# rodrigo-paganini/kalman-vae

Measured on AMD Instinct MI355X. Metric: sequences/sec (ELBO training step, 32x32xT bouncing-ball), higher is better.
Workload: dtype f32; 1 GPU; BASELINE configs[1] (configs[2] per-GPU shard): bouncing-ball 32x32, T=50, batch=256/GPU, dynamics=lstm K=3, z=4, u=4, a=2, full train step (fwd incl. sigmoid(x_logits) + loss incl. active-unit stats + bwd + clip + Adam); both the GPU leg and the cpu_baseline leg do this work; preset=c2, global_batch=256, seq_len=50, parallelism=dp1, capture=hipgraph, loss_finite=True, dist_backend=none

## Files before the change

### include/kvae_lgssm.h

```cpp
#ifndef KVAE_LGSSM_H
#define KVAE_LGSSM_H

#include <stdint.h>

#ifdef __cplusplus
extern "C" {
#endif

#define KVAE_MAX_DIM 16
#define KVAE_ABI_VERSION 12

typedef enum {
  KVAE_OK = 0,
  KVAE_ERR_DIMS = 1,
  KVAE_ERR_NULL = 2,
  KVAE_ERR_LAUNCH = 3,
  KVAE_ERR_ARG = 4
} kvae_status;

typedef struct {
  const float *ptr;
  int64_t sb, st;
} kvae_stack;

typedef struct {
  int32_t B, T, n, m, p;
  kvae_stack A;
  kvae_stack Bm;
  kvae_stack C;
  kvae_stack Q;
  const float *R;
  const float *mu0;
  int64_t mu0_sb;
  const float *Sigma0;
  int64_t Sigma0_sb;
  const float *Y;
  const float *U;
  const float *mask;
} kvae_lgssm_problem;

typedef struct {
  float *mus_filt;
  float *Sigmas_filt;
  float *mus_pred;
  float *Sigmas_pred;
  float *mus_smooth;
  float *Sigmas_smooth;
  float *aux;
} kvae_lgssm_states;
#define KVAE_AUX(n, p) ((n) * (p) + (p) * (p) + (n) * (n))

typedef struct {
  float *ptr;
  int64_t sb, st;
} kvae_gstack;

typedef struct {
  kvae_gstack gA, gB, gC, gQ;
  float *gY, *gU;
  float *g_mu0, *g_Sigma0;
} kvae_lgssm_input_grads;


int kvae_lgssm_filter_fwd(const kvae_lgssm_problem *prob, const kvae_lgssm_states *out, void *stream);

int kvae_lgssm_rts_fwd(const kvae_lgssm_problem *prob, const kvae_lgssm_states *io, void *stream);

int kvae_lgssm_smooth_fwd(const kvae_lgssm_problem *prob, const kvae_lgssm_states *out, void *stream);

int kvae_lgssm_filter_alpha_lstm(const kvae_lgssm_problem *prob, const kvae_lgssm_states *out, const float *w_ih,
                                 const float *w_hh, const float *b_ih, const float *b_hh, const float *head_w,
                                 const float *head_b, const float *A, const float *Bm, const float *C, int32_t K, int32_t H,
                                 float *record, float *alpha, float *gates, float *c_seq, float *h_seq, float *x_seq,
                                 void *stream);


int kvae_lgssm_smooth_bwd(const kvae_lgssm_problem *prob, const kvae_lgssm_states *saved,
                          const kvae_lgssm_states *up, const kvae_lgssm_input_grads *out,
                          float *ws, int with_rts, void *stream);

int kvae_lgssm_alpha_lstm_bwd(const kvae_lgssm_problem *prob, const kvae_lgssm_states *saved, const kvae_lgssm_states *up,
                              const kvae_lgssm_input_grads *out, float *ws, int with_rts, const float *w_ih,
                              const float *w_hh, const float *head_w, const float *A, const float *Bm, const float *C,
                              int32_t K, int32_t H, const float *alpha, const float *gates, const float *c_seq,
                              const float *g_record_up, const float *g_alpha_up, float *g_record, float *d_pre,
                              float *g_logit, void *stream);


int kvae_lgssm_elbo(const kvae_lgssm_problem *prob, const float *mus_smooth, const float *Sigmas_smooth,
                    const float *eps, float *terms, int32_t *chol_levels, float *ws_lz, float *g_mus,
                    float *g_Sigmas, const kvae_lgssm_input_grads *g, void *stream);


int kvae_mix_fwd(const float *alpha, const float *base, float *out, int64_t rows, int32_t K, int32_t E,
                 void *stream);

int kvae_mix_bwd(const float *alpha, const float *base, const float *g_out, float *g_alpha, float *g_base,
                 float *partials, int64_t rows, int32_t K, int32_t E, int32_t accumulate_alpha, void *stream);
int64_t kvae_mix_bwd_partials(int64_t rows);


int kvae_lstm_fwd(const float *x, const float *w_ih, const float *w_hh, const float *b_ih, const float *b_hh,
                  float *h_seq, float *gates, float *c_seq, int32_t B, int32_t T, int32_t I, int32_t H, void *stream);

int kvae_lstm_bwd(const float *g_h, const float *gates, const float *c_seq, const float *w_ih, const float *w_hh,
                  float *d_pre, float *dx, int32_t B, int32_t T, int32_t I, int32_t H, void *stream);


int kvae_regime_fwd(const float *logits, const float *init_logits, const float *gumbel, const float *P, float *y_seq,
                    float *log_q, float *log_p, int32_t B, int32_t T, int32_t K, float tau, const float *tau_dev,
                    int32_t hard, void *stream);
int kvae_regime_bwd(const float *logits, const float *init_logits, const float *gumbel, const float *P,
                    const float *y_seq, const float *g_y, const float *g_log_q, const float *g_log_p, float *g_logits,
                    float *g_init, int32_t B, int32_t T, int32_t K, float tau, const float *tau_dev, void *stream);


int kvae_bigru_fwd(const float *x, const float *const w_ih[2], const float *const w_hh[2], const float *const b_ih[2],
                   const float *const b_hh[2], float *h_seq, float *gates, int32_t B, int32_t T, int32_t I, int32_t H,
                   void *stream);
int kvae_bigru_bwd(const float *g_h, const float *gates, const float *h_seq, const float *const w_ih[2],
                   const float *const w_hh[2], float *d_pre_i, float *d_pre_h, float *dx, int32_t B, int32_t T,
                   int32_t I, int32_t H, void *stream);


int kvae_bias_shuffle_act_fwd(const float *in, const float *bias, float *out, int64_t N, int32_t C, int32_t H,
                              int32_t W, int32_t r, int32_t relu, void *stream);
int kvae_bias_shuffle_act_bwd(const float *g_out, const float *out, float *g_in, float *bias_partials, int64_t N,
                              int32_t C, int32_t H, int32_t W, int32_t r, int32_t relu, void *stream);
int64_t kvae_bias_partial_rows(int64_t N);
int kvae_colsum(const float *partials, float *out, int64_t rows, int64_t cols, void *stream);
int kvae_colsum2(const float *partials_a, float *out_a, int64_t rows_a, int64_t cols_a, const float *partials_b, float *out_b,
                 int64_t rows_b, int64_t cols_b, void *stream);


int kvae_clip_adam(float *params, const float *grads, float *exp_avg, float *exp_avg_sq, int64_t n, const int32_t *seg_of,
                   int32_t n_seg, const float *seg_active, float *seg_steps, const float *lr_dev, float lr, float beta1, float beta2,
                   float eps, float weight_decay, float clip, const float *div_dev, float *norm_out, float *ws, void *stream);


int kvae_lgssm_emission_means(const kvae_lgssm_problem *prob, const float *mus_smooth, const float *mus_filt, float *a_imputed,
                              float *a_filtered, void *stream);


typedef struct kvae_wgrad_problem {
  const float *d;
  const float *h;
  const float *x;
  float *g_wh, *g_wx, *g_b;
  int64_t d_stride, h_stride, x_stride, N;
  int32_t R, H, I, bias, T, shift;
} kvae_wgrad_problem;
int64_t kvae_rnn_wgrad_ws_floats(const kvae_wgrad_problem *probs, int32_t n);
int kvae_rnn_wgrad(const kvae_wgrad_problem *probs, int32_t n, float *ws, void *stream);

int kvae_linear_fwd(const float *x, int64_t x_stride, int64_t N, int32_t F, const float *W, const float *b, int32_t O,
                    int32_t softmax, float *y, void *stream);
int kvae_linear_bwd_input(const float *g, const float *y, int64_t N, int32_t F, const float *W, int32_t O, float *g_logit,
                          float *dx, int64_t dx_stride, void *stream);


int kvae_bce_frames_fwd(const float *logits, const float *x, float *frame_ll, int64_t frames, int32_t pixels, void *stream);
int kvae_bce_frames_bwd(const float *logits, const float *x, const float *g_frame, float *g_logits, int64_t frames,
                        int32_t pixels, void *stream);


#define KVAE_DEC_HEAD_SCRATCH_FLOATS 2304
int kvae_dec_head_fwd(const float *in, const float *W, const float *bias, float *logits, float *w_scratch, int64_t N,
                      int32_t Cin, int32_t side, void *stream);
int kvae_dec_head_bwd(const float *in, const float *W, const float *g_logits, float *g_in, float *w_partials,
                      float *b_partials, float *w_scratch, int64_t N, int32_t Cin, int32_t side, void *stream);
int kvae_enc_stem_fwd(const float *x, const float *W, const float *bias, float *out, uint32_t *relu_bits, int64_t N, int32_t Cout,
                      int32_t side, void *stream);
int kvae_enc_stem_bwd(const float *x, const float *out, const uint32_t *relu_bits, const float *g_out, float *w_partials,
                      float *b_partials, int64_t N, int32_t Cout, int32_t side, void *stream);
int64_t kvae_conv_edge_partial_rows(int64_t N);

int kvae_enc_mid_fwd(const float *in, const float *W, const float *bias, float *out, int64_t N, int32_t C, int32_t side,
                     void *stream);
int kvae_enc_mid_bwd(const float *in, const float *W, const float *out, const float *g_out, float *g_in,
                     float *w_partials, float *b_partials, int64_t N, int32_t C, int32_t side, void *stream);
int64_t kvae_enc_mid_partial_rows(int64_t N, int32_t side);

int kvae_dec_up_fwd(const float *x, const float *W, const float *bias, float *out, int64_t N, int32_t Cin, int32_t side,
                    void *stream);
int kvae_dec_up_bwd(const float *x, const float *W, const float *out, const float *g_out, float *g_x, float *w_partials,
                    float *b_partials, int64_t N, int32_t Cin, int32_t side, void *stream);
int64_t kvae_dec_up_partial_rows(int64_t N, int32_t side);
int32_t kvae_dec_up_set_workgroups(int32_t n);


int kvae_enc_head_fwd(const float *feat, const float *Wmu, const float *bmu, const float *Wvar, const float *bvar,
                      const float *eps, float *mu, float *var, float *a, int64_t N, int32_t F, int32_t A,
                      float noise_emission, void *stream);
int kvae_enc_head_bwd(const float *feat, const float *Wmu, const float *Wvar, const float *var, const float *eps,
                      const float *g_a, const float *g_mu, const float *g_var, float *g_feat, float *w_partials,
                      float *b_partials, int64_t N, int32_t F, int32_t A, float noise_emission, void *stream);
int kvae_dec_fc_fwd(const float *a, const float *W, const float *b, float *h, int64_t N, int32_t F, int32_t A, void *stream);
int kvae_dec_fc_bwd(const float *g_h, const float *a, const float *W, float *g_a, float *w_partials, float *b_partials,
                    int64_t N, int32_t F, int32_t A, void *stream);
int64_t kvae_head_partial_rows(void);
int kvae_latent_reg_fwd(const float *a, const float *mu, const float *var, float *reg, int64_t N, int32_t A, void *stream);
int kvae_latent_reg_bwd(const float *a, const float *mu, const float *var, const float *g, float *g_a, float *g_mu,
                        float *g_var, int64_t N, int32_t A, void *stream);

int kvae_loss_head_fwd(const float *lpx, const float *regf, const float *mask, const float *elbo_kf, const float *beta,
                       float scale_reconstruction, float vae_weight, float kf_weight, const float *weights_dev, float *out6,
                       float *coef3, int64_t n, void *stream);
int kvae_loss_head_bwd(const float *g_loss, const float *coef3, const float *mask, float *g_lpx, float *g_regf,
                       float *g_elbo_kf, int64_t n, void *stream);

typedef struct {
  int32_t B, S, H;
  int32_t n, m, p, K;
  int32_t kind;
  int32_t hidden;
  const float *A;
  const float *Bm;
  const float *C;
  const float *LQ;
  const float *LR;
  const float *mu;
  const float *L0;
  const float *U;
  const float *w_ih;
  const float *w_hh;
  const float *b_ih;
  const float *b_hh;
  const float *head_w;
  const float *head_b;
  const float *h0;
  const float *c0;
  const float *y0;
  const float *P;
  const float *s0;
  const float *eps0;
  const float *eps_z;
  const float *eps_a;
  const float *gumbel;
  float *a_out;
  float *z_out;
  float *w_out;
} kvae_gen_problem;
int kvae_lgssm_generate(const kvae_gen_problem *prob, void *stream);

#define KVAE_PSAMPLE_GAINS 1
#define KVAE_PSAMPLE_PATHS 2
typedef struct {
  int32_t B, S, T;
  int32_t n, p;
  int32_t stages;
  const float *mus_filt;
  const float *Sigmas_filt;
  const float *mus_pred;
  const float *Sigmas_pred;
  kvae_stack A;
  kvae_stack C;
  kvae_stack Q;
  const float *LR;
  const float *eps;
  const float *eta;
  float *z_out;
  float *a_out;
  int32_t *levels_out;
  float *ws;
} kvae_psample_problem;
int kvae_lgssm_posterior_sample(const kvae_psample_problem *prob, void *stream);
int64_t kvae_lgssm_posterior_sample_ws_floats(const kvae_psample_problem *prob);

int kvae_abi_version(void);
const char *kvae_last_error(void);
const char *kvae_build_info(void);

#ifdef __cplusplus
}
#endif
#endif
```

### kalman-vae_amd/csrc/kvae_vae.hip

```cpp
#include <hip/hip_runtime.h>

#include <stdint.h>
#include <stdio.h>
#include <stdlib.h>
#include <string.h>

#include "../../include/kvae_lgssm.h"

namespace kvae {}
using namespace kvae;

extern "C" int kvae_launch_status(const char *what);
static int launch_status(const char *what) { return kvae_launch_status(what); }

#include "vae_epilogue.h"

__device__ __forceinline__ void colsum_v4_body(const float *__restrict__ partials, float *__restrict__ out, int64_t rows, int64_t cols,
                                               unsigned block) {
  __shared__ float4 red[8][64];
  const int lane = threadIdx.x & 63, wv = threadIdx.x >> 6;
  const int64_t c = ((int64_t)block * 64 + lane) * 4;
  float4 s0 = make_float4(0.f, 0.f, 0.f, 0.f), s1 = s0, s2 = s0, s3 = s0;
  if (c < cols) {
    const float *p = partials + c;
    int64_t r = wv;
    for (; r + 24 < rows; r += 32) {
      const float4 a = *reinterpret_cast<const float4 *>(p + r * cols), b = *reinterpret_cast<const float4 *>(p + (r + 8) * cols),
                   d = *reinterpret_cast<const float4 *>(p + (r + 16) * cols), e = *reinterpret_cast<const float4 *>(p + (r + 24) * cols);
      s0.x += a.x; s0.y += a.y; s0.z += a.z; s0.w += a.w;
      s1.x += b.x; s1.y += b.y; s1.z += b.z; s1.w += b.w;
      s2.x += d.x; s2.y += d.y; s2.z += d.z; s2.w += d.w;
      s3.x += e.x; s3.y += e.y; s3.z += e.z; s3.w += e.w;
    }
    for (; r < rows; r += 8) {
      const float4 a = *reinterpret_cast<const float4 *>(p + r * cols);
      s0.x += a.x; s0.y += a.y; s0.z += a.z; s0.w += a.w;
    }
  }
  red[wv][lane] = make_float4((s0.x + s1.x) + (s2.x + s3.x), (s0.y + s1.y) + (s2.y + s3.y), (s0.z + s1.z) + (s2.z + s3.z),
                              (s0.w + s1.w) + (s2.w + s3.w));
  __syncthreads();
  if (wv == 0 && c < cols) {
    float4 t = red[0][lane];
#pragma unroll
    for (int w = 1; w < 8; ++w) { const float4 u = red[w][lane]; t.x += u.x; t.y += u.y; t.z += u.z; t.w += u.w; }
    *reinterpret_cast<float4 *>(out + c) = t;
  }
}
__global__ __launch_bounds__(512) void k_colsum_v4(const float *__restrict__ partials, float *__restrict__ out, int64_t rows,
                                                   int64_t cols) {
  colsum_v4_body(partials, out, rows, cols, blockIdx.x);
}
__global__ __launch_bounds__(512) void k_colsum_v4_pair(const float *__restrict__ pa, float *__restrict__ oa, int64_t rows_a, int64_t cols_a,
                                                        unsigned nb_a, const float *__restrict__ pb, float *__restrict__ ob,
                                                        int64_t rows_b, int64_t cols_b) {
  if (blockIdx.x < nb_a) colsum_v4_body(pa, oa, rows_a, cols_a, blockIdx.x);
  else colsum_v4_body(pb, ob, rows_b, cols_b, blockIdx.x - nb_a);
}
__global__ __launch_bounds__(256) void k_colsum(const float *__restrict__ partials, float *__restrict__ out, int64_t rows,
                                                int64_t cols) {
  __shared__ float red[256];
  const int cx = threadIdx.x & 63, ry = threadIdx.x >> 6;
  const int64_t c = (int64_t)blockIdx.x * 64 + cx;
  float s0 = 0.f, s1 = 0.f;
  if (c < cols) {
    int64_t r = ry;
    for (; r + 4 < rows; r += 8) {
      s0 += partials[r * cols + c];
      s1 += partials[(r + 4) * cols + c];
    }
    if (r < rows) s0 += partials[r * cols + c];
  }
  red[threadIdx.x] = s0 + s1;
  __syncthreads();
  if (ry == 0 && c < cols) out[c] = (red[cx] + red[64 + cx]) + (red[128 + cx] + red[192 + cx]);
}

template <int R>
__global__ __launch_bounds__(256) void k_vae_epilogue_fwd_v4(const float *__restrict__ in, const float *__restrict__ bias,
                                                             float *__restrict__ out, int C, int H, int W, int64_t quads,
                                                             int relu) {
  const int OW = W * R, OH = H * R, QW = OW / 4;
  for (int64_t qd = (int64_t)blockIdx.x * 256 + threadIdx.x; qd < quads; qd += (int64_t)gridDim.x * 256) {
    const int qw = (int)(qd % QW);
    const int64_t t1 = qd / QW;
    const int oh = (int)(t1 % OH);
    const int64_t t2 = t1 / OH;
    const int c = (int)(t2 % C);
    const int64_t n = t2 / C;
    float4 v;
    if (R == 1) {
      const float b = bias[c];
      const float4 x = *reinterpret_cast<const float4 *>(in + ((n * C + c) * H + oh) * W + 4 * qw);
      v = make_float4(x.x + b, x.y + b, x.z + b, x.w + b);
    } else {
      const int ch0 = c * 4 + (oh & 1) * 2;
      const int64_t base = ((n * (C * 4) + ch0) * H + (oh >> 1)) * W + 2 * qw;
      const float2 a = *reinterpret_cast<const float2 *>(in + base);
      const float2 d = *reinterpret_cast<const float2 *>(in + base + (int64_t)H * W);
      const float b0 = bias[ch0], b1 = bias[ch0 + 1];
      v = make_float4(a.x + b0, d.x + b1, a.y + b0, d.y + b1);
    }
    if (relu) v = make_float4(fmaxf(v.x, 0.f), fmaxf(v.y, 0.f), fmaxf(v.z, 0.f), fmaxf(v.w, 0.f));
    *reinterpret_cast<float4 *>(out + qd * 4) = v;
  }
}

__global__ __launch_bounds__(256) void k_vae_epilogue_fwd(const float *in, const float *bias, float *out, EpiShape s,
                                                          int64_t total, int relu) {
  for (int64_t o = (int64_t)blockIdx.x * 256 + threadIdx.x; o < total; o += (int64_t)gridDim.x * 256)
    epi_fwd_elem(s, in, bias, out, o, relu);
}

__global__ __launch_bounds__(256) void k_vae_epilogue_bwd_bias(const float *__restrict__ g_out, const float *__restrict__ out,
                                                               float *__restrict__ g_in, float *__restrict__ bias_partials,
                                                               EpiShape s, int n_per_chunk, int relu) {
  extern __shared__ float bins[];
  const int Cin = s.C * s.r * s.r;
  const int OW = s.W * s.r, OH = s.H * s.r;
  const int64_t vol = (int64_t)s.C * OH * OW;
  for (int i = threadIdx.x; i < Cin; i += 256) bins[i] = 0.f;
  __syncthreads();
  const int64_t pos = (int64_t)blockIdx.x * 256 + threadIdx.x;
  if (pos < vol) {
    const int ow = (int)(pos % OW);
    const int oh = (int)((pos / OW) % OH);
    const int c = (int)(pos / ((int64_t)OW * OH));
    const int ch = c * s.r * s.r + (oh % s.r) * s.r + (ow % s.r);
    const int64_t in_off = ((int64_t)ch * s.H + oh / s.r) * s.W + ow / s.r;
    const int64_t in_vol = (int64_t)Cin * s.H * s.W;
    const int64_t n0 = (int64_t)blockIdx.y * n_per_chunk;
    const int64_t n1 = n0 + n_per_chunk < s.N ? n0 + n_per_chunk : s.N;
    float acc = 0.f;
    for (int64_t n = n0; n < n1; ++n) {
      float g = g_out[n * vol + pos];
      if (relu && !(out[n * vol + pos] > 0.f)) g = 0.f;
      g_in[n * in_vol + in_off] = g;
      acc += g;
    }
    atomicAdd(&bins[ch], acc);
  }
  __syncthreads();
  for (int i = threadIdx.x; i < Cin; i += 256) {
    if (bins[i] != 0.f) atomicAdd(&bias_partials[(int64_t)blockIdx.y * Cin + i], bins[i]);
  }
}

__global__ __launch_bounds__(256) void k_vae_epilogue_bwd(const float *g_out, const float *out, float *g_in, EpiShape s,
                                                          int64_t total, int relu) {
  for (int64_t o = (int64_t)blockIdx.x * 256 + threadIdx.x; o < total; o += (int64_t)gridDim.x * 256)
    epi_bwd_elem(s, g_out, out, g_in, o, relu);
}

#define KVAE_EPI_SAMPLES_PER_CHUNK 32
extern "C" int64_t kvae_bias_partial_rows(int64_t N);
static unsigned epi_grid(int64_t total) {
  const int64_t blocks = (total + 255) / 256;
  return (unsigned)(blocks < 256 * 32 ? blocks : 256 * 32);
}

extern "C" {
int kvae_bias_shuffle_act_fwd(const float *in, const float *bias, float *out, int64_t N, int32_t C, int32_t H, int32_t W,
                              int32_t r, int32_t relu, void *stream) {
  if (!in || !bias || !out) return KVAE_ERR_NULL;
  if (N < 1 || C < 1 || H < 1 || W < 1 || r < 1) return KVAE_ERR_ARG;
  const EpiShape s{N, C, H, W, r};
  const int64_t total = N * C * H * W * r * r;
  const bool aligned = ((uintptr_t)in % 16 == 0) && ((uintptr_t)out % 16 == 0);
  if (aligned && r == 1 && W % 4 == 0)
    k_vae_epilogue_fwd_v4<1><<<dim3(epi_grid(total / 4)), dim3(256), 0, (hipStream_t)stream>>>(in, bias, out, C, H, W, total / 4, relu);
  else if (aligned && r == 2 && W % 2 == 0)
    k_vae_epilogue_fwd_v4<2><<<dim3(epi_grid(total / 4)), dim3(256), 0, (hipStream_t)stream>>>(in, bias, out, C, H, W, total / 4, relu);
  else
    k_vae_epilogue_fwd<<<dim3(epi_grid(total)), dim3(256), 0, (hipStream_t)stream>>>(in, bias, out, s, total, relu);
  return launch_status("k_vae_epilogue_fwd");
}
int kvae_bias_shuffle_act_bwd(const float *g_out, const float *out, float *g_in, float *bias_partials, int64_t N, int32_t C,
                              int32_t H, int32_t W, int32_t r, int32_t relu, void *stream) {
  if (!g_out || !g_in || (relu && !out)) return KVAE_ERR_NULL;
  if (N < 1 || C < 1 || H < 1 || W < 1 || r < 1) return KVAE_ERR_ARG;
  const EpiShape s{N, C, H, W, r};
  const int64_t total = N * C * H * W * r * r;
  hipStream_t st = (hipStream_t)stream;
  if (bias_partials) {
    const int Cin = C * r * r;
    const int64_t chunks = kvae_bias_partial_rows(N);
    if (hipMemsetAsync(bias_partials, 0, sizeof(float) * chunks * Cin, st) != hipSuccess) return launch_status("memset bias_partials");
    const int64_t vol = (int64_t)C * H * W * r * r;
    k_vae_epilogue_bwd_bias<<<dim3((unsigned)((vol + 255) / 256), (unsigned)chunks), dim3(256), sizeof(float) * Cin, st>>>(
        g_out, out, g_in, bias_partials, s, KVAE_EPI_SAMPLES_PER_CHUNK, relu);
    return launch_status("k_vae_epilogue_bwd_bias");
  }
  k_vae_epilogue_bwd<<<dim3(epi_grid(total)), dim3(256), 0, st>>>(g_out, out, g_in, s, total, relu);
  return launch_status("k_vae_epilogue_bwd");
}
int kvae_colsum(const float *partials, float *out, int64_t rows, int64_t cols, void *stream) {
  if (!partials || !out) return KVAE_ERR_NULL;
  if (rows < 1 || cols < 1) return KVAE_ERR_ARG;
  if ((cols & 3) == 0 && ((((uintptr_t)partials | (uintptr_t)out) & 15) == 0))
    k_colsum_v4<<<dim3((unsigned)((cols + 255) / 256)), dim3(512), 0, (hipStream_t)stream>>>(partials, out, rows, cols);
  else
    k_colsum<<<dim3((unsigned)((cols + 63) / 64)), dim3(256), 0, (hipStream_t)stream>>>(partials, out, rows, cols);
  return launch_status("k_colsum");
}
int kvae_colsum2(const float *pa, float *oa, int64_t rows_a, int64_t cols_a, const float *pb, float *ob, int64_t rows_b,
                 int64_t cols_b, void *stream) {
  if (!pa || !oa || !pb || !ob) return KVAE_ERR_NULL;
  if (rows_a < 1 || cols_a < 1 || rows_b < 1 || cols_b < 1) return KVAE_ERR_ARG;
  if (((cols_a | cols_b) & 3) == 0 && ((((uintptr_t)pa | (uintptr_t)oa | (uintptr_t)pb | (uintptr_t)ob) & 15) == 0)) {
    const unsigned nb_a = (unsigned)((cols_a + 255) / 256), nb_b = (unsigned)((cols_b + 255) / 256);
    k_colsum_v4_pair<<<dim3(nb_a + nb_b), dim3(512), 0, (hipStream_t)stream>>>(pa, oa, rows_a, cols_a, nb_a, pb, ob, rows_b, cols_b);
    return launch_status("k_colsum_v4_pair");
  }
  const int rc = kvae_colsum(pa, oa, rows_a, cols_a, stream);
  return rc ? rc : kvae_colsum(pb, ob, rows_b, cols_b, stream);
}
int64_t kvae_bias_partial_rows(int64_t N) { return (N + KVAE_EPI_SAMPLES_PER_CHUNK - 1) / KVAE_EPI_SAMPLES_PER_CHUNK; }
}

constexpr int CA_BLOCKS = 512;
constexpr int CA_MAX_SEG = 1024;
__global__ __launch_bounds__(256) void k_grad_sumsq(const float *__restrict__ g, int64_t n, const int32_t *__restrict__ seg_of,
                                                    int n_seg, const float *__restrict__ seg_active,
                                                    const float *__restrict__ div_dev, float *__restrict__ seg_steps,
                                                    float *__restrict__ ws) {
  __shared__ float red[256];
  const float inv = div_dev ? 1.0f / fmaxf(*div_dev, 1.0f) : 1.0f;
  const bool gated = seg_of && seg_active;
  float s = 0.f;
  for (int64_t i = (int64_t)blockIdx.x * 256 + threadIdx.x; i < n; i += (int64_t)gridDim.x * 256) {
    float v = g[i] * inv;
    if (gated && seg_active[seg_of[i]] == 0.f) v = 0.f;
    s = fmaf(v, v, s);
  }
  red[threadIdx.x] = s;
  __syncthreads();
  for (int o = 128; o > 0; o >>= 1) {
    if ((int)threadIdx.x < o) red[threadIdx.x] += red[threadIdx.x + o];
    __syncthreads();
  }
  if (threadIdx.x == 0) ws[blockIdx.x] = red[0];
  if (blockIdx.x == 0)
    for (int sg = threadIdx.x; sg < n_seg; sg += 256)
      if (!seg_active || seg_active[sg] != 0.f) seg_steps[sg] += 1.0f;
}
__global__ __launch_bounds__(256) void k_clip_adam(float *__restrict__ p, const float *__restrict__ g, float *__restrict__ m,
                                                   float *__restrict__ v, int64_t n, const int32_t *__restrict__ seg_of, int n_seg,
                                                   const float *__restrict__ seg_active, const float *__restrict__ seg_steps,
                                                   const float *__restrict__ lr_dev, float lr, float beta1, float beta2, float eps,
                                                   float wd, float clip, const float *__restrict__ div_dev,
                                                   float *__restrict__ norm_out, const float *__restrict__ ws, int nparts) {
  __shared__ float red[256];
  __shared__ float s_step_size[CA_MAX_SEG], s_bc2s[CA_MAX_SEG];
  float s = 0.f;
  for (int i = threadIdx.x; i < nparts; i += 256) s += ws[i];
  red[threadIdx.x] = s;
  const float lrv = lr_dev ? *lr_dev : lr;
  for (int sg = threadIdx.x; sg < n_seg; sg += 256) {
    const float step = seg_steps[sg];
    const bool on = !seg_active || seg_active[sg] != 0.f;
    s_step_size[sg] = on ? lrv / (1.0f - powf(beta1, step)) : -1.0f;
    s_bc2s[sg] = on ? sqrtf(1.0f - powf(beta2, step)) : 1.0f;
  }
  __syncthreads();
  for (int o = 128; o > 0; o >>= 1) {
    if ((int)threadIdx.x < o) red[threadIdx.x] += red[threadIdx.x + o];
    __syncthreads();
  }
  const float total = sqrtf(red[0]);
  if (norm_out && blockIdx.x == 0 && threadIdx.x == 0) *norm_out = total;
  const float inv = div_dev ? 1.0f / fmaxf(*div_dev, 1.0f) : 1.0f;
  const float scale = inv * (clip > 0.f ? fminf(clip / (total + 1e-6f), 1.0f) : 1.0f);
  for (int64_t i = (int64_t)blockIdx.x * 256 + threadIdx.x; i < n; i += (int64_t)gridDim.x * 256) {
    const int sg = seg_of ? seg_of[i] : 0;
    const float step_size = s_step_size[sg], bc2s = s_bc2s[sg];
    if (step_size < 0.f) continue;
    float gi = g[i] * scale;
    const float pi = p[i];
    if (wd != 0.f) gi = fmaf(wd, pi, gi);
    const float mi = m[i] + (gi - m[i]) * (1.0f - beta1);
    const float vi = beta2 * v[i] + (1.0f - beta2) * gi * gi;
    m[i] = mi, v[i] = vi;
    p[i] = pi - step_size * mi / (sqrtf(vi) / bc2s + eps);
  }
}
extern "C" int kvae_clip_adam(float *params, const float *grads, float *exp_avg, float *exp_avg_sq, int64_t n,
                              const int32_t *seg_of, int32_t n_seg, const float *seg_active, float *seg_steps, const float *lr_dev,
                              float lr, float beta1, float beta2, float eps, float weight_decay, float clip, const float *div_dev,
                              float *norm_out, float *ws, void *stream) {
  if (!params || !grads || !exp_avg || !exp_avg_sq || !seg_steps || !ws) return KVAE_ERR_NULL;
  if (n < 1 || n_seg < 1 || n_seg > CA_MAX_SEG || (!seg_of && n_seg != 1)) return KVAE_ERR_ARG;
  const int64_t want = (n + 1023) / 1024;
  const unsigned parts = (unsigned)(want < CA_BLOCKS ? want : CA_BLOCKS);
  k_grad_sumsq<<<dim3(parts), dim3(256), 0, (hipStream_t)stream>>>(grads, n, seg_of, n_seg, seg_active, div_dev, seg_steps, ws);
  int rc = launch_status("k_grad_sumsq");
  if (rc) return rc;
  const unsigned blocks = (unsigned)((n + 255) / 256 < 2048 ? (n + 255) / 256 : 2048);
  k_clip_adam<<<dim3(blocks), dim3(256), 0, (hipStream_t)stream>>>(params, grads, exp_avg, exp_avg_sq, n, seg_of, n_seg, seg_active,
                                                                   seg_steps, lr_dev, lr, beta1, beta2, eps, weight_decay, clip,
                                                                   div_dev, norm_out, ws, (int)parts);
  return launch_status("k_clip_adam");
}

#include "vae_loss.h"

__global__ __launch_bounds__(256) void k_vae_bce_fwd(const float *__restrict__ logits, const float *__restrict__ x,
                                                     float *__restrict__ frame_ll, int64_t frames, int pixels) {
  const int64_t f = (int64_t)blockIdx.x * 4 + (threadIdx.x >> 6);
  const int lane = threadIdx.x & 63;
  if (f >= frames) return;
  const float *l = logits + f * pixels, *t = x + f * pixels;
  float acc = 0.f;
  if ((pixels & 3) == 0 && (((uintptr_t)l | (uintptr_t)t) & 15) == 0) {
    for (int i = lane * 4; i < pixels; i += 256) {
      const float4 a = *reinterpret_cast<const float4 *>(l + i), b = *reinterpret_cast<const float4 *>(t + i);
      acc += bce_logit(a.x, b.x) + bce_logit(a.y, b.y) + bce_logit(a.z, b.z) + bce_logit(a.w, b.w);
    }
  } else {
    for (int i = lane; i < pixels; i += 64) acc += bce_logit(l[i], t[i]);
  }
  for (int off = 32; off > 0; off >>= 1) acc += __shfl_down(acc, off, 64);
  if (lane == 0) frame_ll[f] = -acc;
}

__global__ __launch_bounds__(256) void k_vae_bce_bwd(const float *__restrict__ logits, const float *__restrict__ x,
                                                     const float *__restrict__ g_frame, float *__restrict__ g_logits,
                                                     int64_t total, int pixels) {
  for (int64_t i = ((int64_t)blockIdx.x * 256 + threadIdx.x) * 4; i < total; i += (int64_t)gridDim.x * 1024) {
    const float g = -g_frame[i / pixels];
    const float4 a = *reinterpret_cast<const float4 *>(logits + i), b = *reinterpret_cast<const float4 *>(x + i);
    *reinterpret_cast<float4 *>(g_logits + i) = make_float4(g * (sigmoid_stable(a.x) - b.x), g * (sigmoid_stable(a.y) - b.y),
                                                            g * (sigmoid_stable(a.z) - b.z), g * (sigmoid_stable(a.w) - b.w));
  }
}
__global__ __launch_bounds__(256) void k_vae_bce_bwd_scalar(const float *logits, const float *x, const float *g_frame,
                                                            float *g_logits, int64_t total, int pixels) {
  for (int64_t i = (int64_t)blockIdx.x * 256 + threadIdx.x; i < total; i += (int64_t)gridDim.x * 256)
    g_logits[i] = -g_frame[i / pixels] * (sigmoid_stable(logits[i]) - x[i]);
}

extern "C" {
int kvae_bce_frames_fwd(const float *logits, const float *x, float *frame_ll, int64_t frames, int32_t pixels, void *stream) {
  if (!logits || !x || !frame_ll) return KVAE_ERR_NULL;
  if (frames < 1 || pixels < 1) return KVAE_ERR_ARG;
  k_vae_bce_fwd<<<dim3((unsigned)((frames + 3) / 4)), dim3(256), 0, (hipStream_t)stream>>>(logits, x, frame_ll, frames, pixels);
  return launch_status("k_vae_bce_fwd");
}
int kvae_bce_frames_bwd(const float *logits, const float *x, const float *g_frame, float *g_logits, int64_t frames,
                        int32_t pixels, void *stream) {
  if (!logits || !x || !g_frame || !g_logits) return KVAE_ERR_NULL;
  if (frames < 1 || pixels < 1) return KVAE_ERR_ARG;
  const int64_t total = frames * pixels;
  const bool v4 = (pixels & 3) == 0 && ((((uintptr_t)logits | (uintptr_t)x | (uintptr_t)g_logits) & 15) == 0);
  if (v4)
    k_vae_bce_bwd<<<dim3(epi_grid(total / 4)), dim3(256), 0, (hipStream_t)stream>>>(logits, x, g_frame, g_logits, total, pixels);
  else
    k_vae_bce_bwd_scalar<<<dim3(epi_grid(total)), dim3(256), 0, (hipStream_t)stream>>>(logits, x, g_frame, g_logits, total, pixels);
  return launch_status("k_vae_bce_bwd");
}
}

#include "vae_conv_edge.h"
extern "C" {
int64_t kvae_conv_edge_partial_rows(int64_t N) { return N < 1024 ? (N < 1 ? 1 : N) : 1024; }

int kvae_dec_head_fwd(const float *in, const float *W, const float *bias, float *logits, float *w_scratch, int64_t N,
                      int32_t Cin, int32_t side, void *stream) {
  if (!in || !W || !bias || !logits || !w_scratch) return KVAE_ERR_NULL;
  if (N < 1) return KVAE_ERR_ARG;
  if (Cin != DH_CI || side != DH_S) return KVAE_ERR_DIMS;
  k_dec_head_prep<<<dim3(1), dim3(256), 0, (hipStream_t)stream>>>(W, w_scratch);
  k_dec_head_fwd<<<dim3((unsigned)N), dim3(256), 0, (hipStream_t)stream>>>(in, w_scratch, bias, logits);
  return launch_status("k_dec_head_fwd");
}
int kvae_dec_head_bwd(const float *in, const float *W, const float *g_logits, float *g_in, float *w_partials,
                      float *b_partials, float *w_scratch, int64_t N, int32_t Cin, int32_t side, void *stream) {
  if (!in || !W || !g_logits || !w_partials || !b_partials || !w_scratch) return KVAE_ERR_NULL;
  if (N < 1) return KVAE_ERR_ARG;
  if (Cin != DH_CI || side != DH_S) return KVAE_ERR_DIMS;
  if (g_in) {
    k_dec_head_prep<<<dim3(1), dim3(256), 0, (hipStream_t)stream>>>(W, w_scratch);
    k_dec_head_bwd_data<<<dim3((unsigned)N), dim3(256), 0, (hipStream_t)stream>>>(g_logits, w_scratch, g_in);
    const int rc = launch_status("k_dec_head_bwd_data");
    if (rc) return rc;
  }
  k_dec_head_wrw<<<dim3((unsigned)kvae_conv_edge_partial_rows(N)), dim3(256), 0, (hipStream_t)stream>>>(in, g_logits, w_partials,
                                                                                                     b_partials, N);
  return launch_status("k_dec_head_wrw");
}
int kvae_enc_stem_fwd(const float *x, const float *W, const float *bias, float *out, uint32_t *relu_bits, int64_t N, int32_t Cout,
                      int32_t side, void *stream) {
  if (!x || !W || !bias || !out) return KVAE_ERR_NULL;
  if (N < 1) return KVAE_ERR_ARG;
  if (Cout != ES_CO || side != ES_IN) return KVAE_ERR_DIMS;
  k_enc_stem_fwd<<<dim3((unsigned)N), dim3(256), 0, (hipStream_t)stream>>>(x, W, bias, out, relu_bits);
  return launch_status("k_enc_stem_fwd");
}
int kvae_enc_stem_bwd(const float *x, const float *out, const uint32_t *relu_bits, const float *g_out, float *w_partials,
                      float *b_partials, int64_t N, int32_t Cout, int32_t side, void *stream) {
  if (!x || (!out && !relu_bits) || !g_out || !w_partials || !b_partials) return KVAE_ERR_NULL;
  if (N < 1) return KVAE_ERR_ARG;
  if (Cout != ES_CO || side != ES_IN) return KVAE_ERR_DIMS;
  static const int mfma = getenv("KVAE_STEM_MFMA") ? atoi(getenv("KVAE_STEM_MFMA")) : 1;
  const dim3 grid((unsigned)kvae_conv_edge_partial_rows(N));
  if (mfma == 1 && relu_bits) k_enc_stem_wrw_mfma<true><<<grid, dim3(256), 0, (hipStream_t)stream>>>(x, out, relu_bits, g_out, w_partials, b_partials, N);
  else if (!out) return KVAE_ERR_NULL;
  else if (mfma) k_enc_stem_wrw_mfma<false><<<grid, dim3(256), 0, (hipStream_t)stream>>>(x, out, relu_bits, g_out, w_partials, b_partials, N);
  else k_enc_stem_wrw<<<grid, dim3(256), 0, (hipStream_t)stream>>>(x, out, g_out, w_partials, b_partials, N);
  return launch_status("k_enc_stem_wrw");
}
}

#include "vae_conv_mid.h"
static inline int64_t enc_mid_grid(int64_t N, int32_t side) {
  const int64_t fpi = side == 16 ? 2 : 8, iters = (N + fpi - 1) / fpi;
  return iters < 256 ? (iters < 1 ? 1 : iters) : 256;
}
extern "C" {
int64_t kvae_enc_mid_partial_rows(int64_t N, int32_t side) { return enc_mid_grid(N, side); }

int kvae_enc_mid_fwd(const float *in, const float *W, const float *bias, float *out, int64_t N, int32_t C, int32_t side,
                     void *stream) {
  if (!in || !W || !bias || !out) return KVAE_ERR_NULL;
  if (N < 1 || (N + 256 * 8) * EM_C * side * side * 4 >= EM_MAX_BYTES) return KVAE_ERR_ARG;
  if (C != EM_C || (side != 16 && side != 8)) return KVAE_ERR_DIMS;
  const dim3 grid((unsigned)enc_mid_grid(N, side));
  if (side == 16) k_enc_mid_fwd<16><<<grid, dim3(256), 0, (hipStream_t)stream>>>(in, W, bias, out, N);
  else k_enc_mid_fwd<8><<<grid, dim3(256), 0, (hipStream_t)stream>>>(in, W, bias, out, N);
  return launch_status("k_enc_mid_fwd");
}
int kvae_enc_mid_bwd(const float *in, const float *W, const float *out, const float *g_out, float *g_in,
                     float *w_partials, float *b_partials, int64_t N, int32_t C, int32_t side, void *stream) {
  if (!in || !W || !out || !g_out || !w_partials || !b_partials) return KVAE_ERR_NULL;
  if (N < 1 || (N + 256 * 8) * EM_C * side * side * 4 >= EM_MAX_BYTES) return KVAE_ERR_ARG;
  if (C != EM_C || (side != 16 && side != 8)) return KVAE_ERR_DIMS;
  const dim3 grid((unsigned)enc_mid_grid(N, side));
  if (g_in) {
    if (side == 16) k_enc_mid_bwd_data<16><<<grid, dim3(256), 0, (hipStream_t)stream>>>(W, out, g_out, g_in, N);
    else k_enc_mid_bwd_data<8><<<grid, dim3(256), 0, (hipStream_t)stream>>>(W, out, g_out, g_in, N);
    const int rc = launch_status("k_enc_mid_bwd_data");
    if (rc) return rc;
  }
  if (side == 16) k_enc_mid_wrw<16><<<grid, dim3(256), 0, (hipStream_t)stream>>>(in, out, g_out, w_partials, b_partials, N);
  else k_enc_mid_wrw<8><<<grid, dim3(256), 0, (hipStream_t)stream>>>(in, out, g_out, w_partials, b_partials, N);
  return launch_status("k_enc_mid_wrw");
}
}

#include "vae_conv_up_wino.h"
static bool dec_up_wino() {
  static const int env = getenv("KVAE_WINO") ? atoi(getenv("KVAE_WINO")) : 1;
  return env != 0;
}
static int g_dec_up_wgs = 0;
static inline int64_t dec_up_cap() {
  static const int env = getenv("KVAE_UP_WGS") ? atoi(getenv("KVAE_UP_WGS")) : 0;
  const int v = env >= 1 && env <= 256 ? env : __atomic_load_n(&g_dec_up_wgs, __ATOMIC_RELAXED);
  return v >= 1 && v <= 256 ? v : 256;
}
static inline int64_t dec_up_grid(int64_t N, int32_t side) {
  const int64_t fpi = side == 8 ? 2 : 8, iters = (N + fpi - 1) / fpi, cap = dec_up_cap();
  return iters < cap ? (iters < 1 ? 1 : iters) : cap;
}
extern "C" {
int64_t kvae_dec_up_partial_rows(int64_t N, int32_t side) { return dec_up_grid(N, side); }
int32_t kvae_dec_up_set_workgroups(int32_t n) {
  const int32_t prev = (int32_t)dec_up_cap();
  __atomic_store_n(&g_dec_up_wgs, n >= 1 && n <= 256 ? n : 0, __ATOMIC_RELAXED);
  return prev;
}

int kvae_dec_up_fwd(const float *x, const float *W, const float *bias, float *out, int64_t N, int32_t Cin, int32_t side,
                    void *stream) {
  if (!x || !W || !bias || !out) return KVAE_ERR_NULL;
  if (N < 1 || (N + 256 * 8) * UP_CO * side * side * 4 >= EM_MAX_BYTES) return KVAE_ERR_ARG;
  if (Cin != UP_CI || (side != 8 && side != 4)) return KVAE_ERR_DIMS;
  const dim3 grid((unsigned)dec_up_grid(N, side));
  if (dec_up_wino()) {
    const int64_t sets = side == 8 ? N : (N + 3) / 4;
    const dim3 wgrid((unsigned)(sets < dec_up_cap() ? sets : dec_up_cap()));
    if (side == 8) k_dec_up_fwd_wino<8><<<wgrid, dim3(512), 0, (hipStream_t)stream>>>(x, W, bias, out, N);
    else k_dec_up_fwd_wino<4><<<wgrid, dim3(512), 0, (hipStream_t)stream>>>(x, W, bias, out, N);
    return launch_status("k_dec_up_fwd_wino");
  }
  if (side == 8) k_dec_up_fwd<8><<<grid, dim3(256), 0, (hipStream_t)stream>>>(x, W, bias, out, N);
  else k_dec_up_fwd<4><<<grid, dim3(256), 0, (hipStream_t)stream>>>(x, W, bias, out, N);
  return launch_status("k_dec_up_fwd");
}
int kvae_dec_up_bwd(const float *x, const float *W, const float *out, const float *g_out, float *g_x, float *w_partials,
                    float *b_partials, int64_t N, int32_t Cin, int32_t side, void *stream) {
  if (!x || !W || !out || !g_out || !w_partials || !b_partials) return KVAE_ERR_NULL;
  if (N < 1 || (N + 256 * 8) * UP_CO * side * side * 4 >= EM_MAX_BYTES) return KVAE_ERR_ARG;
  if (Cin != UP_CI || (side != 8 && side != 4)) return KVAE_ERR_DIMS;
  const dim3 grid((unsigned)dec_up_grid(N, side));
  if (g_x) {
    const int64_t sets = side == 8 ? N : (N + 3) / 4;
    const dim3 wgrid((unsigned)(sets < dec_up_cap() ? sets : dec_up_cap()));
    if (dec_up_wino() && side == 8) k_dec_up_bwd_data_wino<8><<<wgrid, dim3(512), 0, (hipStream_t)stream>>>(W, out, g_out, g_x, N);
    else if (dec_up_wino()) k_dec_up_bwd_data_wino<4><<<wgrid, dim3(512), 0, (hipStream_t)stream>>>(W, out, g_out, g_x, N);
    else if (side == 8) k_dec_up_bwd_data<8><<<grid, dim3(256), 0, (hipStream_t)stream>>>(W, out, g_out, g_x, N);
    else k_dec_up_bwd_data<4><<<grid, dim3(256), 0, (hipStream_t)stream>>>(W, out, g_out, g_x, N);
    const int rc = launch_status("k_dec_up_bwd_data");
    if (rc) return rc;
  }
  if (dec_up_wino()) {
    if (side == 8) k_dec_up_wrw_wino<8><<<grid, dim3(512), 0, (hipStream_t)stream>>>(x, out, g_out, w_partials, b_partials, N);
    else k_dec_up_wrw_wino<4><<<grid, dim3(512), 0, (hipStream_t)stream>>>(x, out, g_out, w_partials, b_partials, N);
    return launch_status("k_dec_up_wrw_wino");
  }
  if (side == 8) k_dec_up_wrw<8><<<grid, dim3(256), 0, (hipStream_t)stream>>>(x, out, g_out, w_partials, b_partials, N);
  else k_dec_up_wrw<4><<<grid, dim3(256), 0, (hipStream_t)stream>>>(x, out, g_out, w_partials, b_partials, N);
  return launch_status("k_dec_up_wrw");
}
}

#include "vae_heads.h"
extern "C" {
int64_t kvae_head_partial_rows(void) { return HD_WAVES; }

int kvae_enc_head_fwd(const float *feat, const float *Wmu, const float *bmu, const float *Wvar, const float *bvar,
                      const float *eps, float *mu, float *var, float *a, int64_t N, int32_t F, int32_t A,
                      float noise_emission, void *stream) {
  if (!feat || !Wmu || !bmu || !Wvar || !bvar || !mu || !var || !a) return KVAE_ERR_NULL;
  if (N < 1) return KVAE_ERR_ARG;
  if (F != HD_F || A != HD_A) return KVAE_ERR_DIMS;
  const unsigned grid = (unsigned)(N < 4 * 512 ? (N + 3) / 4 : 512);
  k_enc_head_fwd<<<dim3(grid), dim3(256), 0, (hipStream_t)stream>>>(feat, Wmu, bmu, Wvar, bvar, eps, noise_emission, mu, var, a, N);
  return launch_status("k_enc_head_fwd");
}
int kvae_enc_head_bwd(const float *feat, const float *Wmu, const float *Wvar, const float *var, const float *eps,
                      const float *g_a, const float *g_mu, const float *g_var, float *g_feat, float *w_partials,
                      float *b_partials, int64_t N, int32_t F, int32_t A, float noise_emission, void *stream) {
  if (!feat || !Wmu || !Wvar || !var || !g_feat || !w_partials || !b_partials) return KVAE_ERR_NULL;
  if (N < 1) return KVAE_ERR_ARG;
  if (F != HD_F || A != HD_A) return KVAE_ERR_DIMS;
  k_enc_head_bwd<<<dim3(HD_WAVES / 4), dim3(256), 0, (hipStream_t)stream>>>(feat, Wmu, Wvar, var, eps, g_a, g_mu, g_var,
                                                                             noise_emission, g_feat, w_partials, b_partials, N);
  return launch_status("k_enc_head_bwd");
}
int kvae_dec_fc_fwd(const float *a, const float *W, const float *b, float *h, int64_t N, int32_t F, int32_t A, void *stream) {
  if (!a || !W || !b || !h) return KVAE_ERR_NULL;
  if (N < 1) return KVAE_ERR_ARG;
  if (F != HD_F || A != HD_A) return KVAE_ERR_DIMS;
  k_dec_fc_fwd<<<dim3(epi_grid(N * (HD_F / 4))), dim3(256), 0, (hipStream_t)stream>>>(a, W, b, h, N * (HD_F / 4));
  return launch_status("k_dec_fc_fwd");
}
int kvae_dec_fc_bwd(const float *g_h, const float *a, const float *W, float *g_a, float *w_partials, float *b_partials,
                    int64_t N, int32_t F, int32_t A, void *stream) {
  if (!g_h || !a || !W || !g_a || !w_partials || !b_partials) return KVAE_ERR_NULL;
  if (N < 1) return KVAE_ERR_ARG;
  if (F != HD_F || A != HD_A) return KVAE_ERR_DIMS;
  k_dec_fc_bwd<<<dim3(HD_WAVES / 4), dim3(256), 0, (hipStream_t)stream>>>(g_h, a, W, g_a, w_partials, b_partials, N);
  return launch_status("k_dec_fc_bwd");
}
int kvae_latent_reg_fwd(const float *a, const float *mu, const float *var, float *reg, int64_t N, int32_t A, void *stream) {
  if (!a || !mu || !var || !reg) return KVAE_ERR_NULL;
  if (N < 1 || A < 1) return KVAE_ERR_ARG;
  k_latent_reg_fwd<<<dim3(epi_grid(N)), dim3(256), 0, (hipStream_t)stream>>>(a, mu, var, reg, N, A);
  return launch_status("k_latent_reg_fwd");
}
int kvae_latent_reg_bwd(const float *a, const float *mu, const float *var, const float *g, float *g_a, float *g_mu,
                        float *g_var, int64_t N, int32_t A, void *stream) {
  if (!a || !mu || !var || !g || !g_a || !g_mu || !g_var) return KVAE_ERR_NULL;
  if (N < 1 || A < 1) return KVAE_ERR_ARG;
  k_latent_reg_bwd<<<dim3(epi_grid(N * A)), dim3(256), 0, (hipStream_t)stream>>>(a, mu, var, g, g_a, g_mu, g_var, N, A);
  return launch_status("k_latent_reg_bwd");
}
int kvae_loss_head_fwd(const float *lpx, const float *regf, const float *mask, const float *elbo_kf, const float *beta,
                       float scale_reconstruction, float vae_weight, float kf_weight, const float *weights_dev, float *out6,
                       float *coef3, int64_t n, void *stream) {
  if (!lpx || !regf || !elbo_kf || !beta || !out6 || !coef3) return KVAE_ERR_NULL;
  if (n < 1) return KVAE_ERR_ARG;
  k_loss_head_fwd<<<dim3(1), dim3(1024), 0, (hipStream_t)stream>>>(lpx, regf, mask, elbo_kf, beta, scale_reconstruction, vae_weight,
                                                                  kf_weight, weights_dev, out6, coef3, n);
  return launch_status("k_loss_head_fwd");
}
int kvae_loss_head_bwd(const float *g_loss, const float *coef3, const float *mask, float *g_lpx, float *g_regf,
                       float *g_elbo_kf, int64_t n, void *stream) {
  if (!g_loss || !coef3 || !g_lpx || !g_regf || !g_elbo_kf) return KVAE_ERR_NULL;
  if (n < 1) return KVAE_ERR_ARG;
  k_loss_head_bwd<<<dim3(epi_grid(n)), dim3(256), 0, (hipStream_t)stream>>>(g_loss, coef3, mask, g_lpx, g_regf,
                                                                            g_elbo_kf, n);
  return launch_status("k_loss_head_bwd");
}
}
```

### kalman-vae_amd/csrc/vae_conv_edge.h

```cpp
#pragma once
#include <hip/hip_runtime.h>
#include <stdint.h>

namespace kvae {

constexpr int DH_CI = 32, DH_CO = 4, DH_S = 16, DH_TS = 18, DH_CS = 325;
constexpr int DH_W = DH_CO * DH_CI * 9;
typedef float kv_f2 __attribute__((ext_vector_type(2)));
typedef float kv_f4 __attribute__((ext_vector_type(4)));

__global__ __launch_bounds__(256) void k_dec_head_prep(const float *__restrict__ W, float *__restrict__ scratch) {
  for (int i = threadIdx.x; i < DH_W; i += 256) {
    const int co = i / (DH_CI * 9), r = i - co * DH_CI * 9, ci = r / 9, k = r - ci * 9;
    const float w = W[i];
    scratch[(ci * 9 + k) * DH_CO + co] = w;
    scratch[DH_W + (co * 9 + k) * DH_CI + ci] = w;
  }
}

__device__ __forceinline__ void dh_zero_halo(float *tile, int channels) {
  for (int i = threadIdx.x; i < channels * 68; i += 256) {
    const int c = i / 68, j = i - c * 68;
    int r, q;
    if (j < 18) { r = 0; q = j; }
    else if (j < 36) { r = 17; q = j - 18; }
    else if (j < 52) { r = j - 35; q = 0; }
    else { r = j - 51; q = 17; }
    tile[c * DH_CS + r * DH_TS + q] = 0.f;
  }
}
__device__ __forceinline__ void dh_store_interior(float *tile, int i, const float4 v) {
  const int e = i * 4, ci = e >> 8, hw = e & 255, h = hw >> 4, w = hw & 15;
  float *d = tile + ci * DH_CS + (h + 1) * DH_TS + (w + 1);
  d[0] = v.x; d[1] = v.y; d[2] = v.z; d[3] = v.w;
}

__global__ __launch_bounds__(256) void k_dec_head_fwd(const float *__restrict__ in, const float *__restrict__ scratch,
                                                      const float *__restrict__ bias, float *__restrict__ logits) {
  __shared__ float tile[DH_CI * 256];
  const int64_t n = blockIdx.x;
  const float4 *src = reinterpret_cast<const float4 *>(in + n * DH_CI * 256);
  float4 pre[8];
#pragma unroll
  for (int j = 0; j < 8; ++j) pre[j] = src[threadIdx.x + 256 * j];
#pragma unroll
  for (int j = 0; j < 8; ++j) reinterpret_cast<float4 *>(tile)[threadIdx.x + 256 * j] = pre[j];
  __syncthreads();
  const int h = threadIdx.x >> 4, w = threadIdx.x & 15;
  constexpr int OOB = 1 << 24;
  const int tb = (h - 1) * 16 + (w - 1);
  int base[9];
#pragma unroll
  for (int tap = 0; tap < 9; ++tap) {
    const int ky = tap / 3, kx = tap % 3;
    const bool z = (ky == 0 && h == 0) || (ky == 2 && h == 15) || (kx == 0 && w == 0) || (kx == 2 && w == 15);
    base[tap] = (z ? OOB : tb) + ky * 16 + kx;
  }
  kv_f2 a01 = {bias[0], bias[1]}, a23 = {bias[2], bias[3]};
  const kv_f4 *Wf = reinterpret_cast<const kv_f4 *>(scratch);
#pragma unroll 4
  for (int ci = 0; ci < DH_CI; ++ci) {
#pragma unroll
    for (int tap = 0; tap < 9; ++tap) {
      const float v = tile[base[tap] + ci * 256];
      const kv_f4 wv = Wf[ci * 9 + tap];
      a01 += wv.xy * v;
      a23 += wv.zw * v;
    }
  }
  float *o = logits + n * 1024 + (2 * h) * 32 + 2 * w;
  *reinterpret_cast<float2 *>(o) = make_float2(a01.x, a01.y);
  *reinterpret_cast<float2 *>(o + 32) = make_float2(a23.x, a23.y);
}

__global__ __launch_bounds__(256) void k_dec_head_bwd_data(const float *__restrict__ g_logits,
                                                           const float *__restrict__ scratch, float *__restrict__ g_in) {
  __shared__ float gt[DH_CO * DH_CS];
  const int64_t n = blockIdx.x;
  float gp[4];
#pragma unroll
  for (int j = 0; j < 4; ++j) gp[j] = g_logits[n * 1024 + threadIdx.x + 256 * j];
  dh_zero_halo(gt, DH_CO);
#pragma unroll
  for (int j = 0; j < 4; ++j) {
    const int i = threadIdx.x + 256 * j, oh = i >> 5, ow = i & 31, co = (oh & 1) * 2 + (ow & 1);
    gt[co * DH_CS + ((oh >> 1) + 1) * DH_TS + (ow >> 1) + 1] = gp[j];
  }
  __syncthreads();
  const int h = threadIdx.x >> 4, w = threadIdx.x & 15;
  kv_f2 acc[DH_CI / 2];
#pragma unroll
  for (int j = 0; j < DH_CI / 2; ++j) acc[j] = kv_f2{0.f, 0.f};
  const kv_f2 *Wb = reinterpret_cast<const kv_f2 *>(scratch + DH_W);
#pragma unroll
  for (int co = 0; co < DH_CO; ++co)
#pragma unroll
    for (int ky = 0; ky < 3; ++ky)
#pragma unroll
      for (int kx = 0; kx < 3; ++kx) {
        const float v = gt[co * DH_CS + (h + 2 - ky) * DH_TS + (w + 2 - kx)];
        const kv_f2 *wr = Wb + (co * 9 + ky * 3 + kx) * (DH_CI / 2);
#pragma unroll
        for (int j = 0; j < DH_CI / 2; ++j) acc[j] += wr[j] * v;
      }
  float *o = g_in + n * DH_CI * 256 + threadIdx.x;
#pragma unroll
  for (int j = 0; j < DH_CI / 2; ++j) {
    o[(2 * j) * 256] = acc[j].x;
    o[(2 * j + 1) * 256] = acc[j].y;
  }
}

__global__ __launch_bounds__(256) void k_dec_head_wrw(const float *__restrict__ in, const float *__restrict__ g_logits,
                                                      float *__restrict__ partial, float *__restrict__ partial_b, int64_t N) {
  constexpr int CS = 257, OOB = 1 << 24;
  __shared__ float lds[DH_CI * CS + DH_CO * 256];
  __shared__ float redb[8 * DH_CO];
  float *tile = lds, *gt = lds + DH_CI * CS;
  const int ci = threadIdx.x & 31, grp = threadIdx.x >> 5;
  const int tin = (((threadIdx.x & 63) >> 4) << 6) | ((threadIdx.x >> 6) << 4) | (threadIdx.x & 15);
  kv_f2 acc[DH_CO / 2][9];
  float accb[DH_CO];
#pragma unroll
  for (int c = 0; c < DH_CO / 2; ++c)
#pragma unroll
    for (int k = 0; k < 9; ++k) acc[c][k] = kv_f2{0.f, 0.f};
#pragma unroll
  for (int co = 0; co < DH_CO; ++co) accb[co] = 0.f;
  float4 pre[8];
  float gp[4];
  int64_t n = blockIdx.x;
  if (n < N) {
    const float4 *src = reinterpret_cast<const float4 *>(in + n * DH_CI * 256);
#pragma unroll
    for (int j = 0; j < 8; ++j) pre[j] = src[tin + 256 * j];
#pragma unroll
    for (int j = 0; j < 4; ++j) gp[j] = g_logits[n * 1024 + threadIdx.x + 256 * j];
  }
  for (; n < N; n += gridDim.x) {
    __syncthreads();
#pragma unroll
    for (int j = 0; j < 8; ++j) {
      const int e = (tin + 256 * j) * 4;
      float *d = tile + (e >> 8) * CS + (e & 255);
      d[0] = pre[j].x; d[1] = pre[j].y; d[2] = pre[j].z; d[3] = pre[j].w;
    }
#pragma unroll
    for (int j = 0; j < 4; ++j) {
      const int i = threadIdx.x + 256 * j, oh = i >> 5, ow = i & 31, co = (oh & 1) * 2 + (ow & 1);
      gt[co * 256 + (oh >> 1) * 16 + (ow >> 1)] = gp[j];
    }
    __syncthreads();
    const int64_t nn = n + gridDim.x;
    if (nn < N) {
      const float4 *src = reinterpret_cast<const float4 *>(in + nn * DH_CI * 256);
#pragma unroll
      for (int j = 0; j < 8; ++j) pre[j] = src[tin + 256 * j];
#pragma unroll
      for (int j = 0; j < 4; ++j) gp[j] = g_logits[nn * 1024 + threadIdx.x + 256 * j];
    }
#pragma unroll
    for (int rr = 0; rr < 2; ++rr) {
      const int h = 2 * grp + rr;
      int rb[3];
#pragma unroll
      for (int ky = 0; ky < 3; ++ky) {
        const bool off = (ky == 0 && rr == 0 && grp == 0) || (ky == 2 && rr == 1 && grp == 7);
        rb[ky] = (off ? OOB : ci * CS) + (h + ky - 1) * 16;
      }
      float c0[3] = {0.f, 0.f, 0.f}, c1[3], c2[3];
#pragma unroll
      for (int ky = 0; ky < 3; ++ky) c1[ky] = tile[rb[ky]];
#pragma unroll
      for (int w = 0; w < 16; ++w) {
#pragma unroll
        for (int ky = 0; ky < 3; ++ky) c2[ky] = w + 1 < 16 ? tile[rb[ky] + w + 1] : 0.f;
        const int hw = h * 16 + w;
        const kv_f2 g01 = {gt[hw], gt[256 + hw]}, g23 = {gt[512 + hw], gt[768 + hw]};
        accb[0] += g01.x; accb[1] += g01.y; accb[2] += g23.x; accb[3] += g23.y;
#pragma unroll
        for (int ky = 0; ky < 3; ++ky) {
          acc[0][ky * 3 + 0] += g01 * c0[ky]; acc[1][ky * 3 + 0] += g23 * c0[ky];
          acc[0][ky * 3 + 1] += g01 * c1[ky]; acc[1][ky * 3 + 1] += g23 * c1[ky];
          acc[0][ky * 3 + 2] += g01 * c2[ky]; acc[1][ky * 3 + 2] += g23 * c2[ky];
          c0[ky] = c1[ky];
          c1[ky] = c2[ky];
        }
      }
    }
  }
  __syncthreads();
  float *red = lds;
#pragma unroll
  for (int k = 0; k < 9; ++k) {
    float *r = red + (grp * 32 + ci) * 36 + k;
    r[0] = acc[0][k].x; r[9] = acc[0][k].y; r[18] = acc[1][k].x; r[27] = acc[1][k].y;
  }
  if (ci == 0) {
#pragma unroll
    for (int co = 0; co < DH_CO; ++co) redb[grp * 4 + co] = accb[co];
  }
  __syncthreads();
  for (int o = threadIdx.x; o < DH_W; o += 256) {
    const int co = o / (DH_CI * 9), r = o - co * DH_CI * 9, c2 = r / 9, k = r - c2 * 9;
    float s = 0.f;
    for (int gq = 0; gq < 8; ++gq) s += red[(gq * 32 + c2) * 36 + co * 9 + k];
    partial[(int64_t)blockIdx.x * DH_W + o] = s;
  }
  if (threadIdx.x < DH_CO) {
    float s = 0.f;
    for (int gq = 0; gq < 8; ++gq) s += redb[gq * 4 + threadIdx.x];
    partial_b[(int64_t)blockIdx.x * DH_CO + threadIdx.x] = s;
  }
}


constexpr int ES_CO = 32, ES_IN = 32, ES_OUT = 16, ES_TS = 35;

__device__ __forceinline__ void es_load_tile(float *tile, const float *__restrict__ x) {
  for (int i = threadIdx.x; i < 34 * ES_TS; i += 256) tile[i] = 0.f;
  __syncthreads();
  const float4 v = reinterpret_cast<const float4 *>(x)[threadIdx.x];
  const int e = threadIdx.x * 4, h = e >> 5, w = e & 31;
  float *d = tile + (h + 1) * ES_TS + (w + 1);
  d[0] = v.x; d[1] = v.y; d[2] = v.z; d[3] = v.w;
}

__global__ __launch_bounds__(256) void k_enc_stem_fwd(const float *__restrict__ x, const float *__restrict__ W,
                                                      const float *__restrict__ bias, float *__restrict__ out,
                                                      uint32_t *__restrict__ relu_bits) {
  __shared__ float tile[34 * ES_TS];
  const int64_t n = blockIdx.x;
  es_load_tile(tile, x + n * 1024);
  __syncthreads();
  const int oh = threadIdx.x >> 4, ow = threadIdx.x & 15;
  float v[9];
#pragma unroll
  for (int ky = 0; ky < 3; ++ky)
#pragma unroll
    for (int kx = 0; kx < 3; ++kx) v[ky * 3 + kx] = tile[(2 * oh + ky) * ES_TS + 2 * ow + kx];
  float *o = out + n * ES_CO * 256 + threadIdx.x;
  uint32_t bits = 0;
#pragma unroll 8
  for (int co = 0; co < ES_CO; ++co) {
    float acc = bias[co];
#pragma unroll
    for (int k = 0; k < 9; ++k) acc = fmaf(W[co * 9 + k], v[k], acc);
    o[co * 256] = fmaxf(acc, 0.f);
    bits |= (acc > 0.f ? 1u : 0u) << co;
  }
  if (relu_bits) relu_bits[n * 256 + threadIdx.x] = bits;
}

__global__ __launch_bounds__(256) void k_enc_stem_wrw(const float *__restrict__ x, const float *__restrict__ out,
                                                      const float *__restrict__ g_out, float *__restrict__ partial,
                                                      float *__restrict__ partial_b, int64_t N) {
  __shared__ float tile[34 * ES_TS];
  __shared__ float gt[ES_CO * 257];
  const int co = threadIdx.x & 31, grp = threadIdx.x >> 5;
  float acc[9], accb = 0.f;
#pragma unroll
  for (int k = 0; k < 9; ++k) acc[k] = 0.f;
  for (int64_t n = blockIdx.x; n < N; n += gridDim.x) {
    __syncthreads();
    es_load_tile(tile, x + n * 1024);
    const float4 *g4 = reinterpret_cast<const float4 *>(g_out + n * ES_CO * 256);
    const float4 *o4 = reinterpret_cast<const float4 *>(out + n * ES_CO * 256);
    for (int i = threadIdx.x; i < ES_CO * 64; i += 256) {
      const float4 gv = g4[i], ov = o4[i];
      const int e = i * 4, c = e >> 8, hw = e & 255;
      float *d = gt + c * 257 + hw;
      d[0] = ov.x > 0.f ? gv.x : 0.f; d[1] = ov.y > 0.f ? gv.y : 0.f;
      d[2] = ov.z > 0.f ? gv.z : 0.f; d[3] = ov.w > 0.f ? gv.w : 0.f;
    }
    __syncthreads();
    for (int i = 0; i < 32; ++i) {
      const int hw = grp * 32 + i, oh = hw >> 4, ow = hw & 15;
      const float gv = gt[co * 257 + hw];
      accb += gv;
      const float *t = tile + (2 * oh) * ES_TS + 2 * ow;
#pragma unroll
      for (int ky = 0; ky < 3; ++ky)
#pragma unroll
        for (int kx = 0; kx < 3; ++kx) acc[ky * 3 + kx] = fmaf(gv, t[ky * ES_TS + kx], acc[ky * 3 + kx]);
    }
  }
  __syncthreads();
  float *red = gt;
#pragma unroll
  for (int k = 0; k < 9; ++k) red[(grp * 32 + co) * 10 + k] = acc[k];
  red[(grp * 32 + co) * 10 + 9] = accb;
  __syncthreads();
  for (int o = threadIdx.x; o < ES_CO * 10; o += 256) {
    const int c = o / 10, k = o - c * 10;
    float s = 0.f;
    for (int gq = 0; gq < 8; ++gq) s += red[(gq * 32 + c) * 10 + k];
    if (k < 9) partial[(int64_t)blockIdx.x * (ES_CO * 9) + c * 9 + k] = s;
    else partial_b[(int64_t)blockIdx.x * ES_CO + c] = s;
  }
}

typedef float es_f4 __attribute__((ext_vector_type(4)));
template <bool BITS>
__global__ __launch_bounds__(256) void k_enc_stem_wrw_mfma(const float *__restrict__ x, const float *__restrict__ out,
                                                           const uint32_t *__restrict__ relu_bits, const float *__restrict__ g_out,
                                                           float *__restrict__ partial,
                                                           float *__restrict__ partial_b, int64_t N) {
  __shared__ float tile[34 * ES_TS];
  constexpr int GS = 260;
  __shared__ __attribute__((aligned(16))) float gt[ES_CO * GS];
  __shared__ __attribute__((aligned(16))) uint32_t mw[256];
  const int lane = threadIdx.x & 63, wv = threadIdx.x >> 6, j = lane & 15, g = lane >> 4;
  const int tap = j < 9 ? j : 8;
  const float *tb = tile + (8 * wv) * ES_TS + 2 * g + (tap / 3) * ES_TS + tap % 3;
  const float *ga = gt + j * GS + 64 * wv + g;
  es_f4 acc0 = {0.f, 0.f, 0.f, 0.f}, acc1 = acc0;
  float4 gv[8], ov[8], xv;
  uint32_t mv = 0;
  auto fetch = [&](int64_t n) {
    const bool ok = n < N;
    const float4 *g4 = reinterpret_cast<const float4 *>(g_out + (ok ? n : 0) * ES_CO * 256);
    const float4 *o4 = reinterpret_cast<const float4 *>(out + (ok ? n : 0) * ES_CO * 256);
#pragma unroll
    for (int q = 0; q < 8; ++q) {
      gv[q] = g4[threadIdx.x + 256 * q];
      if constexpr (!BITS) ov[q] = o4[threadIdx.x + 256 * q];
    }
    xv = reinterpret_cast<const float4 *>(x + (ok ? n : 0) * 1024)[threadIdx.x];
    if constexpr (BITS) mv = relu_bits[(ok ? n : 0) * 256 + threadIdx.x];
  };
  fetch(blockIdx.x);
  for (int i = threadIdx.x; i < 34 * ES_TS; i += 256) tile[i] = 0.f;
  for (int64_t n = blockIdx.x; n < N; n += gridDim.x) {
    __syncthreads();
    {
      float *d = tile + ((threadIdx.x >> 3) + 1) * ES_TS + 4 * (threadIdx.x & 7) + 1;
      d[0] = xv.x; d[1] = xv.y; d[2] = xv.z; d[3] = xv.w;
    }
    if constexpr (BITS) {
      mw[threadIdx.x] = mv;
      __syncthreads();
    }
#pragma unroll
    for (int q = 0; q < 8; ++q) {
      const int e = (threadIdx.x + 256 * q) * 4, c = e >> 8, hw = e & 255;
      float4 md;
      if constexpr (BITS) {
        const uint4 m = *reinterpret_cast<const uint4 *>(mw + hw);
        md = make_float4((m.x >> c) & 1u ? gv[q].x : 0.f, (m.y >> c) & 1u ? gv[q].y : 0.f, (m.z >> c) & 1u ? gv[q].z : 0.f,
                         (m.w >> c) & 1u ? gv[q].w : 0.f);
      } else {
        md = make_float4(ov[q].x > 0.f ? gv[q].x : 0.f, ov[q].y > 0.f ? gv[q].y : 0.f, ov[q].z > 0.f ? gv[q].z : 0.f,
                         ov[q].w > 0.f ? gv[q].w : 0.f);
      }
      *reinterpret_cast<float4 *>(gt + c * GS + hw) = md;
    }
    __syncthreads();
    fetch(n + gridDim.x);
#pragma unroll
    for (int s = 0; s < 16; ++s) {
      const float xb = tb[2 * (s >> 2) * ES_TS + 8 * (s & 3)];
      const float b = j == 9 ? 1.0f : xb;
      acc0 = __builtin_amdgcn_mfma_f32_16x16x4f32(ga[4 * s], b, acc0, 0, 0, 0);
      acc1 = __builtin_amdgcn_mfma_f32_16x16x4f32(ga[16 * GS + 4 * s], b, acc1, 0, 0, 0);
    }
  }
  __syncthreads();
  float *red = gt;
#pragma unroll
  for (int r = 0; r < 4; ++r) {
    red[(wv * 32 + 4 * g + r) * 16 + j] = acc0[r];
    red[(wv * 32 + 16 + 4 * g + r) * 16 + j] = acc1[r];
  }
  __syncthreads();
  for (int o = threadIdx.x; o < ES_CO * 10; o += 256) {
    const int c = o / 10, k = o - c * 10;
    const float s = (red[c * 16 + k] + red[(32 + c) * 16 + k]) + (red[(64 + c) * 16 + k] + red[(96 + c) * 16 + k]);
    if (k < 9) partial[(int64_t)blockIdx.x * (ES_CO * 9) + c * 9 + k] = s;
    else partial_b[(int64_t)blockIdx.x * ES_CO + c] = s;
  }
}

}
```

### kalman-vae_amd/csrc/vae_conv_mid.h

```cpp
#pragma once
#include <hip/hip_runtime.h>
#include <stdint.h>

namespace kvae {

typedef float em_f16 __attribute__((ext_vector_type(16)));
constexpr int EM_C = 32, EM_W = EM_C * EM_C * 9;

template <int S>
struct EmDims {
  static constexpr int OS = S / 2, PF = OS * OS;
  static constexpr int FPI = 128 / PF;
  static constexpr int PLANE = S * S, FRAME = EM_C * PLANE;
  static constexpr int IT_IN = FPI * FRAME;
  static constexpr int IT_OUT = FPI * EM_C * PF;
};

__device__ __forceinline__ void em_load_weights(float *Wl, const float *__restrict__ W, bool m_is_co) {
  for (int i = threadIdx.x; i < EM_W; i += 256) {
    const int tap = i >> 10, k = (i >> 5) & 31, m = i & 31;
    const int co = m_is_co ? m : k, ci = m_is_co ? k : m;
    Wl[i] = W[(co * EM_C + ci) * 9 + tap];
  }
}

constexpr int EM_OOB = 1 << 24;
constexpr int64_t EM_MAX_BYTES = (int64_t)1 << 31;

typedef unsigned int em_u4 __attribute__((ext_vector_type(4)));
__device__ __forceinline__ __amdgpu_buffer_rsrc_t em_rsrc(const void *p, int64_t bytes) {
  return __builtin_amdgcn_make_buffer_rsrc(const_cast<void *>(p), 0, (int)bytes, 0x00020000);
}
__device__ __forceinline__ float4 em_ld4(__amdgpu_buffer_rsrc_t r, uint32_t byte_off) {
  const em_u4 v = __builtin_amdgcn_raw_buffer_load_b128(r, byte_off, 0, 0);
  return make_float4(__uint_as_float(v.x), __uint_as_float(v.y), __uint_as_float(v.z), __uint_as_float(v.w));
}
__device__ __forceinline__ void em_st4(__amdgpu_buffer_rsrc_t r, uint32_t byte_off, const float4 v) {
  const em_u4 u = {__float_as_uint(v.x), __float_as_uint(v.y), __float_as_uint(v.z), __float_as_uint(v.w)};
  __builtin_amdgcn_raw_buffer_store_b128(u, r, byte_off, 0, 0);
}
__device__ __forceinline__ void em_st1(__amdgpu_buffer_rsrc_t r, uint32_t byte_off, float v) {
  __builtin_amdgcn_raw_buffer_store_b32(__float_as_uint(v), r, byte_off, 0, 0);
}
#ifdef KVAE_EM_STAMPS
__device__ unsigned long long em_stamps[4096];
#define EM_STAMP(slot, k) do { if (blockIdx.x == 0 && threadIdx.x == 0 && (slot) < 500) em_stamps[(slot) * 8 + (k)] = __builtin_amdgcn_s_memtime(); } while (0)
#else
#define EM_STAMP(slot, k) do {} while (0)
#endif
#define KV_MFMA_F32(a, b, c) __builtin_amdgcn_mfma_f32_32x32x2f32((a), (b), (c), 0, 0, 0)
#define KV_ACC_ROW(r, half) (((r) & 3) + 8 * ((r) >> 2) + 4 * (half))

template <int S>
__global__ __launch_bounds__(256) void k_enc_mid_fwd(const float *__restrict__ in, const float *__restrict__ W,
                                                     const float *__restrict__ bias, float *__restrict__ out, int64_t N) {
  using D = EmDims<S>;
  __shared__ float lds[EM_W + D::IT_IN + D::IT_OUT];
  float *Wl = lds, *fr = lds + EM_W, *ot = fr + D::IT_IN;
  const int tid = threadIdx.x, lane = tid & 63, wv = tid >> 6, q = lane & 31, half = lane >> 5;
  em_load_weights(Wl, W, true);
  const int64_t iters = (N + D::FPI - 1) / D::FPI, total = N * D::FRAME;
  const int gp = 32 * wv + q, fl = gp / D::PF, pix = gp % D::PF, oh = pix / D::OS, ow = pix % D::OS;
  const bool top = oh == 0, left = ow == 0;
  const int bbase = fl * D::FRAME + half * D::PLANE + (2 * oh - 1) * S + (2 * ow - 1);
  const int b_t = top ? EM_OOB : bbase, b_l = left ? EM_OOB : bbase, b_tl = (top || left) ? EM_OOB : bbase;
  const int abase = half * 32 + q;
  float bv[16];
#pragma unroll
  for (int r = 0; r < 16; ++r) bv[r] = bias[KV_ACC_ROW(r, half)];

  const int rot = blockIdx.x & 15;
  const __amdgpu_buffer_rsrc_t rin = em_rsrc(in, total * 4), rout = em_rsrc(out, N * EM_C * D::PF * 4);
  float4 pre[16];
  int64_t it = blockIdx.x;
  auto fetch1 = [&](int64_t i, int j) {
    pre[j] = em_ld4(rin, (uint32_t)(i * D::IT_IN + (tid + 256 * ((j + rot) & 15)) * 4) * 4u);
  };
  uint32_t done_base = 0x80000000u;
  auto flush1 = [&](int j) {
    em_st4(rout, done_base + (uint32_t)(tid + 256 * j) * 16u, reinterpret_cast<const float4 *>(ot)[tid + 256 * j]);
  };
#pragma unroll
  for (int j = 0; j < 16; ++j) fetch1(it, j);
  for (int slot = 0; it < iters; it += gridDim.x, ++slot) {
    EM_STAMP(slot, 0);
    __syncthreads();
    EM_STAMP(slot, 1);
#pragma unroll
    for (int j = 0; j < 16; ++j) reinterpret_cast<float4 *>(fr)[tid + 256 * ((j + rot) & 15)] = pre[j];
    EM_STAMP(slot, 2);
    __syncthreads();
    EM_STAMP(slot, 3);
    EM_STAMP(slot, 4);
    em_f16 acc;
#pragma unroll
    for (int r = 0; r < 16; ++r) acc[r] = 0.f;
    float av[36][4], bw[36][4];
    auto rd = [&](int g) {
#pragma unroll
      for (int u = 0; u < 4; ++u) {
        const int k = g * 4 + u, tap = k / 16, jj = k % 16, ky = tap / 3, kx = tap % 3;
        av[g][u] = Wl[abase + (tap * 32 + 2 * jj) * 32];
        bw[g][u] = fr[(ky == 0 ? (kx == 0 ? b_tl : b_t) : (kx == 0 ? b_l : bbase)) + ky * S + kx + 2 * jj * D::PLANE];
      }
    };
    rd(0);
    rd(1);
#pragma unroll
    for (int g = 0; g < 36; ++g) {
      if (g + 2 < 36) rd(g + 2);
      if (g < 4) flush1(g);
      else if (g < 20) fetch1(it + gridDim.x, g - 4);
      __builtin_amdgcn_sched_barrier(0);
#pragma unroll
      for (int u = 0; u < 4; ++u) acc = KV_MFMA_F32(av[g][u], bw[g][u], acc);
      __builtin_amdgcn_sched_barrier(0);
    }
    EM_STAMP(slot, 5);
    __syncthreads();
    EM_STAMP(slot, 6);
#pragma unroll
    for (int r = 0; r < 16; ++r) ot[(fl * EM_C + KV_ACC_ROW(r, half)) * D::PF + pix] = fmaxf(acc[r] + bv[r], 0.f);
    EM_STAMP(slot, 7);
    done_base = (uint32_t)(it * D::IT_OUT) * 4u;
  }
  __syncthreads();
#pragma unroll
  for (int j = 0; j < 4; ++j) flush1(j);
}

template <int S>
__global__ __launch_bounds__(256) void k_enc_mid_bwd_data(const float *__restrict__ W, const float *__restrict__ out,
                                                          const float *__restrict__ g_out, float *__restrict__ g_in, int64_t N) {
  using D = EmDims<S>;
  __shared__ float lds[EM_W + D::IT_OUT + D::IT_IN];
  float *Wl = lds, *gm = lds + EM_W, *ot = gm + D::IT_OUT;
  const int tid = threadIdx.x, lane = tid & 63, wv = tid >> 6, q = lane & 31, half = lane >> 5;
  em_load_weights(Wl, W, false);
  const int64_t iters = (N + D::FPI - 1) / D::FPI, total_in = N * D::FRAME, total_out = N * EM_C * D::PF;
  const int cp = 32 * wv + q, fl = cp / D::PF, idx = cp % D::PF, a_ = idx / D::OS, b_ = idx % D::OS;
  const bool bottom = a_ == D::OS - 1, right = b_ == D::OS - 1;
  const int gbase = fl * EM_C * D::PF + half * D::PF + a_ * D::OS + b_;
  const int g_b = bottom ? EM_OOB : gbase, g_r = right ? EM_OOB : gbase, g_br = (bottom || right) ? EM_OOB : gbase;
  const int abase = half * 32 + q;
  const int obase = fl * D::FRAME + (2 * a_) * S + 2 * b_;

  const int rot = blockIdx.x & 15;
  const __amdgpu_buffer_rsrc_t rg = em_rsrc(g_out, total_out * 4), ro = em_rsrc(out, total_out * 4),
                               rgi = em_rsrc(g_in, total_in * 4);
  float4 pg[4], po[4];
  int64_t it = blockIdx.x;
  auto fetch1 = [&](int64_t i, int j) {
    const uint32_t e = (uint32_t)(i * D::IT_OUT + (tid + 256 * (((j & 3) + rot) & 3)) * 4) * 4u;
    if (j < 4) pg[j] = em_ld4(rg, e);
    else po[j - 4] = em_ld4(ro, e);
  };
  uint32_t done_base = 0x80000000u;
  auto flush1 = [&](int j) {
    const int c = (j + rot) & 15;
    em_st4(rgi, done_base + (uint32_t)(tid + 256 * c) * 16u, reinterpret_cast<const float4 *>(ot)[tid + 256 * c]);
  };
#pragma unroll
  for (int j = 0; j < 8; ++j) fetch1(it, j);
  for (; it < iters; it += gridDim.x) {
    __syncthreads();
#pragma unroll
    for (int j = 0; j < 4; ++j)
      reinterpret_cast<float4 *>(gm)[tid + 256 * ((j + rot) & 3)] =
          make_float4(po[j].x > 0.f ? pg[j].x : 0.f, po[j].y > 0.f ? pg[j].y : 0.f, po[j].z > 0.f ? pg[j].z : 0.f,
                      po[j].w > 0.f ? pg[j].w : 0.f);
    __syncthreads();
    constexpr int E_CLS[9] = {3, 3, 3, 3, 1, 1, 2, 2, 0};
    constexpr int E_KY[9] = {0, 0, 2, 2, 1, 1, 0, 2, 1};
    constexpr int E_KX[9] = {0, 2, 0, 2, 0, 2, 1, 1, 1};
    float av[36][4], bw[36][4];
    auto rd = [&](int g) {
#pragma unroll
      for (int u = 0; u < 4; ++u) {
        const int en = g / 4, jj = (g % 4) * 4 + u, ph = E_CLS[en] >> 1, pw = E_CLS[en] & 1;
        const int dy = (ph == 1 && E_KY[en] == 0) ? 1 : 0, dx = (pw == 1 && E_KX[en] == 0) ? 1 : 0;
        av[g][u] = Wl[abase + ((E_KY[en] * 3 + E_KX[en]) * 32 + 2 * jj) * 32];
        bw[g][u] = gm[(dy ? (dx ? g_br : g_b) : (dx ? g_r : gbase)) + 2 * jj * D::PF + dy * D::OS + dx];
      }
    };
    rd(0);
    rd(1);
    em_f16 acc;
#pragma unroll
    for (int g = 0; g < 36; ++g) {
      const int en = g / 4, cls = E_CLS[en], ph = cls >> 1, pw = cls & 1;
      if (g % 4 == 0 && (en == 0 || E_CLS[en - 1] != cls)) {
#pragma unroll
        for (int r = 0; r < 16; ++r) acc[r] = 0.f;
      }
      if (g + 2 < 36) rd(g + 2);
      if (g < 16) flush1(g);
      else if (g < 24) fetch1(it + gridDim.x, g - 16);
      __builtin_amdgcn_sched_barrier(0);
#pragma unroll
      for (int u = 0; u < 4; ++u) acc = KV_MFMA_F32(av[g][u], bw[g][u], acc);
      __builtin_amdgcn_sched_barrier(0);
      if (g % 4 == 3 && (en == 8 || E_CLS[en + 1] != cls)) {
        if (g == 15) __syncthreads();
#pragma unroll
        for (int r = 0; r < 16; ++r) ot[obase + KV_ACC_ROW(r, half) * D::PLANE + ph * S + pw] = acc[r];
      }
    }
    done_base = (uint32_t)(it * D::IT_IN) * 4u;
  }
  __syncthreads();
#pragma unroll
  for (int j = 0; j < 16; ++j) flush1(j);
}

template <int S>
__global__ __launch_bounds__(256) void k_enc_mid_wrw(const float *__restrict__ in, const float *__restrict__ out,
                                                     const float *__restrict__ g_out, float *__restrict__ w_partials,
                                                     float *__restrict__ b_partials, int64_t N) {
  using D = EmDims<S>;
  constexpr int CSP = D::PLANE + 1, GSP = D::PF + 1;
  __shared__ float lds[D::FPI * EM_C * GSP + D::FPI * EM_C * CSP];
  float *gm = lds, *xin = lds + D::FPI * EM_C * GSP;
  const int tid = threadIdx.x, lane = tid & 63, wv = tid >> 6, q = lane & 31, half = lane >> 5;
  const int64_t iters = (N + D::FPI - 1) / D::FPI, total_in = N * D::FRAME, total_out = N * EM_C * D::PF;
  const int wframe = S == 16 ? (wv >> 1) : 2 * wv, wpix0 = S == 16 ? 32 * (wv & 1) : 0;
  const int oh0 = wpix0 / D::OS;
  const int abase = wframe * EM_C * GSP + q * GSP + wpix0 + half;
  const int bbase = wframe * EM_C * CSP + q * CSP + (2 * oh0 - 1) * S - 1 + 2 * half;
  const bool wtop = oh0 == 0, wleft = half == 0;
  const int x_t = wtop ? EM_OOB : bbase, x_l = wleft ? EM_OOB : bbase, x_tl = (wtop || wleft) ? EM_OOB : bbase;

  em_f16 acc[9];
#pragma unroll
  for (int t = 0; t < 9; ++t)
#pragma unroll
    for (int r = 0; r < 16; ++r) acc[t][r] = 0.f;
  float bsum = 0.f;

  const int rot = blockIdx.x & 15;
  const __amdgpu_buffer_rsrc_t rin = em_rsrc(in, total_in * 4), rg = em_rsrc(g_out, total_out * 4),
                               ro = em_rsrc(out, total_out * 4);
  float4 px[16], pg[4], po[4];
  int64_t it = blockIdx.x;
  const int tin = S == 16 ? ((lane >> 4) << 6) | (wv << 4) | (lane & 15) : tid;
  auto fetch1 = [&](int64_t i, int j) {
    if (j < 16) {
      px[j] = em_ld4(rin, (uint32_t)(i * D::IT_IN + (tin + 256 * ((j + rot) & 15)) * 4) * 4u);
    } else {
      const uint32_t e = (uint32_t)(i * D::IT_OUT + (tid + 256 * (((j & 3) + rot) & 3)) * 4) * 4u;
      if (j < 20) pg[j - 16] = em_ld4(rg, e);
      else po[j - 20] = em_ld4(ro, e);
    }
  };
#pragma unroll
  for (int j = 0; j < 24; ++j) fetch1(it, j);
  for (; it < iters; it += gridDim.x) {
    __syncthreads();
#pragma unroll
    for (int j = 0; j < 16; ++j) {
      const int e = (tin + 256 * ((j + rot) & 15)) * 4, f = e / D::FRAME, c = (e % D::FRAME) / D::PLANE, p = e % D::PLANE;
      float *d = xin + (f * EM_C + c) * CSP + p;
      d[0] = px[j].x; d[1] = px[j].y; d[2] = px[j].z; d[3] = px[j].w;
    }
#pragma unroll
    for (int j = 0; j < 4; ++j) {
      const int e = (tid + 256 * ((j + rot) & 3)) * 4, f = e / (EM_C * D::PF), c = (e / D::PF) % EM_C, p = e % D::PF;
      float *d = gm + (f * EM_C + c) * GSP + p;
      d[0] = po[j].x > 0.f ? pg[j].x : 0.f; d[1] = po[j].y > 0.f ? pg[j].y : 0.f;
      d[2] = po[j].z > 0.f ? pg[j].z : 0.f; d[3] = po[j].w > 0.f ? pg[j].w : 0.f;
    }
    __syncthreads();
    float av[16], bw[16][9];
    auto rd = [&](int i) {
      const int fi = S == 16 ? 0 : i / 8, p = S == 16 ? 2 * i : 2 * (i % 8);
      const int ohr = p / D::OS, owr = p % D::OS;
      av[i] = gm[abase + fi * EM_C * GSP + p];
#pragma unroll
      for (int tap = 0; tap < 9; ++tap) {
        const bool zt = tap / 3 == 0 && ohr == 0, zl = tap % 3 == 0 && owr == 0;
        bw[i][tap] = xin[(zt ? (zl ? x_tl : x_t) : (zl ? x_l : bbase)) + fi * EM_C * CSP + (2 * ohr + tap / 3) * S + 2 * owr + tap % 3];
      }
    };
    rd(0);
#pragma unroll
    for (int i = 0; i < 16; ++i) {
      if (i + 1 < 16) rd(i + 1);
      if (i < 12) {
        fetch1(it + gridDim.x, 2 * i);
        fetch1(it + gridDim.x, 2 * i + 1);
      }
      __builtin_amdgcn_sched_barrier(0);
      bsum += av[i];
#pragma unroll
      for (int tap = 0; tap < 9; ++tap) acc[tap] = KV_MFMA_F32(av[i], bw[i][tap], acc[tap]);
      __builtin_amdgcn_sched_barrier(0);
    }
  }
  float *red = lds, *redb = lds + EM_W;
  for (int w = 0; w < 4; ++w) {
    __syncthreads();
    if (wv == w) {
#pragma unroll
      for (int tap = 0; tap < 9; ++tap)
#pragma unroll
        for (int r = 0; r < 16; ++r) {
          float *d = red + (KV_ACC_ROW(r, half) * EM_C + q) * 9 + tap;
          *d = w == 0 ? acc[tap][r] : *d + acc[tap][r];
        }
      float *db = redb + half * EM_C + q;
      *db = w == 0 ? bsum : *db + bsum;
    }
  }
  __syncthreads();
  for (int i = tid; i < EM_W; i += 256) w_partials[(int64_t)blockIdx.x * EM_W + i] = red[i];
  if (tid < EM_C) b_partials[(int64_t)blockIdx.x * EM_C + tid] = redb[tid] + redb[EM_C + tid];
}

}
```

### kalman-vae_amd/csrc/vae_loss.h

```cpp
#pragma once
#include "lgssm_vm.h"

namespace kvae {

KV_DEV float bce_logit(float l, float x) { return fmaxf(l, 0.f) - l * x + log1pf(expf(-fabsf(l))); }
KV_DEV float sigmoid_stable(float l) {
  const float e = expf(-fabsf(l));
  return l >= 0.f ? 1.0f / (1.0f + e) : e / (1.0f + e);
}

}
```

### kalman-vae_amd/kvae/_native.py

```python
import ctypes as C
import os
from pathlib import Path

import torch

_HERE = Path(__file__).resolve().parent
LIB_PATH = _HERE / "lib" / "libkvae_lgssm.so"

KVAE_MAX_DIM = 16
KVAE_MAX_K = 16
LSTM_MAX_H, LSTM_MAX_I = 52, 16
ABI_VERSION = 12

_STATUS = {1: "KVAE_ERR_DIMS (n, m, p must be in [1,16]; B, T >= 1)", 2: "KVAE_ERR_NULL", 3: "KVAE_ERR_LAUNCH",
           4: "KVAE_ERR_ARG"}


class Stack(C.Structure):
    _fields_ = [("ptr", C.c_void_p), ("sb", C.c_int64), ("st", C.c_int64)]


class Problem(C.Structure):
    _fields_ = [("B", C.c_int32), ("T", C.c_int32), ("n", C.c_int32), ("m", C.c_int32), ("p", C.c_int32),
                ("A", Stack), ("Bm", Stack), ("C", Stack), ("Q", Stack),
                ("R", C.c_void_p), ("mu0", C.c_void_p), ("mu0_sb", C.c_int64),
                ("Sigma0", C.c_void_p), ("Sigma0_sb", C.c_int64),
                ("Y", C.c_void_p), ("U", C.c_void_p), ("mask", C.c_void_p)]


class States(C.Structure):
    _fields_ = [(k, C.c_void_p) for k in ("mus_filt", "Sigmas_filt", "mus_pred", "Sigmas_pred",
                                          "mus_smooth", "Sigmas_smooth", "aux")]


class WgradProblem(C.Structure):
    _fields_ = [("d", C.c_void_p), ("h", C.c_void_p), ("x", C.c_void_p), ("g_wh", C.c_void_p), ("g_wx", C.c_void_p),
                ("g_b", C.c_void_p), ("d_stride", C.c_int64), ("h_stride", C.c_int64), ("x_stride", C.c_int64), ("N", C.c_int64),
                ("R", C.c_int32), ("H", C.c_int32), ("I", C.c_int32), ("bias", C.c_int32), ("T", C.c_int32), ("shift", C.c_int32)]


class GenProblem(C.Structure):
    _fields_ = ([(k, C.c_int32) for k in ("B", "S", "H", "n", "m", "p", "K", "kind", "hidden")]
                + [(k, C.c_void_p) for k in ("A", "Bm", "C", "LQ", "LR", "mu", "L0", "U", "w_ih", "w_hh", "b_ih", "b_hh",
                                             "head_w", "head_b", "h0", "c0", "y0", "P", "s0", "eps0", "eps_z", "eps_a",
                                             "gumbel", "a_out", "z_out", "w_out")])


class PsampleProblem(C.Structure):
    _fields_ = ([(k, C.c_int32) for k in ("B", "S", "T", "n", "p", "stages")]
                + [(k, C.c_void_p) for k in ("mus_filt", "Sigmas_filt", "mus_pred", "Sigmas_pred")]
                + [("A", Stack), ("C", Stack), ("Q", Stack)]
                + [(k, C.c_void_p) for k in ("LR", "eps", "eta", "z_out", "a_out", "levels_out", "ws")])


class InputGrads(C.Structure):
    _fields_ = [("gA", Stack), ("gB", Stack), ("gC", Stack), ("gQ", Stack),
                ("gY", C.c_void_p), ("gU", C.c_void_p), ("g_mu0", C.c_void_p), ("g_Sigma0", C.c_void_p)]


SYMBOLS = ("kvae_lgssm_filter_alpha_lstm", "kvae_lgssm_alpha_lstm_bwd", "kvae_lgssm_filter_fwd", "kvae_lgssm_rts_fwd", "kvae_lgssm_smooth_fwd", "kvae_lgssm_smooth_bwd",
           "kvae_lgssm_elbo", "kvae_mix_fwd", "kvae_mix_bwd", "kvae_mix_bwd_partials", "kvae_lstm_fwd",
           "kvae_lstm_bwd", "kvae_bias_shuffle_act_fwd", "kvae_bias_shuffle_act_bwd", "kvae_bias_partial_rows", "kvae_colsum", "kvae_colsum2", "kvae_clip_adam", "kvae_regime_fwd", "kvae_regime_bwd", "kvae_bigru_fwd", "kvae_bigru_bwd", "kvae_bce_frames_fwd", "kvae_bce_frames_bwd",
           "kvae_dec_head_fwd", "kvae_dec_head_bwd", "kvae_enc_stem_fwd", "kvae_enc_stem_bwd", "kvae_conv_edge_partial_rows",
           "kvae_enc_mid_fwd", "kvae_enc_mid_bwd", "kvae_enc_mid_partial_rows",
           "kvae_dec_up_fwd", "kvae_dec_up_bwd", "kvae_dec_up_partial_rows", "kvae_dec_up_set_workgroups",
           "kvae_enc_head_fwd", "kvae_enc_head_bwd", "kvae_dec_fc_fwd", "kvae_dec_fc_bwd", "kvae_head_partial_rows",
           "kvae_latent_reg_fwd", "kvae_latent_reg_bwd", "kvae_loss_head_fwd", "kvae_loss_head_bwd",
           "kvae_lgssm_emission_means", "kvae_lgssm_generate", "kvae_lgssm_posterior_sample", "kvae_lgssm_posterior_sample_ws_floats", "kvae_rnn_wgrad", "kvae_rnn_wgrad_ws_floats", "kvae_linear_fwd", "kvae_linear_bwd_input",
           "kvae_abi_version",
           "kvae_last_error", "kvae_build_info")


class LgssmLib:

    def __init__(self, path):
        self.path = str(path)
        self.dll = C.CDLL(self.path)
        missing = [s for s in SYMBOLS if not hasattr(self.dll, s)]
        if missing:
            raise OSError(f"{self.path} does not export {missing}")
        d = self.dll
        P, S, G, vp = C.POINTER(Problem), C.POINTER(States), C.POINTER(InputGrads), C.c_void_p
        for name in ("kvae_lgssm_filter_fwd", "kvae_lgssm_rts_fwd", "kvae_lgssm_smooth_fwd"):
            getattr(d, name).argtypes = [P, S, vp]
            getattr(d, name).restype = C.c_int
        d.kvae_lgssm_filter_alpha_lstm.argtypes = [P, S] + [vp] * 9 + [C.c_int32, C.c_int32] + [vp] * 7
        d.kvae_lgssm_filter_alpha_lstm.restype = C.c_int
        d.kvae_lgssm_alpha_lstm_bwd.argtypes = [P, S, S, G, vp, C.c_int] + [vp] * 6 + [C.c_int32, C.c_int32] + [vp] * 9
        d.kvae_lgssm_alpha_lstm_bwd.restype = C.c_int
        d.kvae_lgssm_generate.argtypes = [C.POINTER(GenProblem), vp]
        d.kvae_lgssm_generate.restype = C.c_int
        d.kvae_lgssm_posterior_sample.argtypes = [C.POINTER(PsampleProblem), vp]
        d.kvae_lgssm_posterior_sample.restype = C.c_int
        d.kvae_lgssm_posterior_sample_ws_floats.argtypes = [C.POINTER(PsampleProblem)]
        d.kvae_lgssm_posterior_sample_ws_floats.restype = C.c_int64
        d.kvae_lgssm_smooth_bwd.argtypes = [P, S, S, G, vp, C.c_int, vp]
        d.kvae_lgssm_smooth_bwd.restype = C.c_int
        d.kvae_lgssm_elbo.argtypes = [P, vp, vp, vp, vp, vp, vp, vp, vp, G, vp]
        d.kvae_lgssm_elbo.restype = C.c_int
        d.kvae_mix_fwd.argtypes = [vp, vp, vp, C.c_int64, C.c_int32, C.c_int32, vp]
        d.kvae_mix_fwd.restype = C.c_int
        d.kvae_mix_bwd.argtypes = [vp, vp, vp, vp, vp, vp, C.c_int64, C.c_int32, C.c_int32, C.c_int32, vp]
        d.kvae_mix_bwd.restype = C.c_int
        d.kvae_mix_bwd_partials.argtypes = [C.c_int64]
        d.kvae_mix_bwd_partials.restype = C.c_int64
        d.kvae_lstm_fwd.argtypes = [vp] * 8 + [C.c_int32] * 4 + [vp]
        d.kvae_lstm_fwd.restype = C.c_int
        d.kvae_lstm_bwd.argtypes = [vp] * 7 + [C.c_int32] * 4 + [vp]
        d.kvae_lstm_bwd.restype = C.c_int
        d.kvae_bias_shuffle_act_fwd.argtypes = [vp, vp, vp, C.c_int64] + [C.c_int32] * 5 + [vp]
        d.kvae_bias_shuffle_act_fwd.restype = C.c_int
        d.kvae_bias_shuffle_act_bwd.argtypes = [vp, vp, vp, vp, C.c_int64] + [C.c_int32] * 5 + [vp]
        d.kvae_bias_shuffle_act_bwd.restype = C.c_int
        d.kvae_regime_fwd.argtypes = [vp] * 7 + [C.c_int32] * 3 + [C.c_float, vp, C.c_int32, vp]
        d.kvae_regime_fwd.restype = C.c_int
        d.kvae_regime_bwd.argtypes = [vp] * 10 + [C.c_int32] * 3 + [C.c_float, vp, vp]
        d.kvae_regime_bwd.restype = C.c_int
        d.kvae_bigru_fwd.argtypes = [vp] * 7 + [C.c_int32] * 4 + [vp]
        d.kvae_bigru_fwd.restype = C.c_int
        d.kvae_bigru_bwd.argtypes = [vp] * 8 + [C.c_int32] * 4 + [vp]
        d.kvae_bigru_bwd.restype = C.c_int
        d.kvae_bce_frames_fwd.argtypes = [vp, vp, vp, C.c_int64, C.c_int32, vp]
        d.kvae_bce_frames_fwd.restype = C.c_int
        d.kvae_bce_frames_bwd.argtypes = [vp, vp, vp, vp, C.c_int64, C.c_int32, vp]
        d.kvae_bce_frames_bwd.restype = C.c_int
        d.kvae_dec_head_fwd.argtypes = [vp, vp, vp, vp, vp, C.c_int64, C.c_int32, C.c_int32, vp]
        d.kvae_dec_head_fwd.restype = C.c_int
        d.kvae_dec_head_bwd.argtypes = [vp] * 7 + [C.c_int64, C.c_int32, C.c_int32, vp]
        d.kvae_dec_head_bwd.restype = C.c_int
        d.kvae_enc_stem_fwd.argtypes = [vp, vp, vp, vp, vp, C.c_int64, C.c_int32, C.c_int32, vp]
        d.kvae_enc_stem_fwd.restype = C.c_int
        d.kvae_enc_stem_bwd.argtypes = [vp] * 6 + [C.c_int64, C.c_int32, C.c_int32, vp]
        d.kvae_enc_stem_bwd.restype = C.c_int
        d.kvae_enc_mid_fwd.argtypes = [vp, vp, vp, vp, C.c_int64, C.c_int32, C.c_int32, vp]
        d.kvae_enc_mid_fwd.restype = C.c_int
        d.kvae_enc_mid_bwd.argtypes = [vp] * 7 + [C.c_int64, C.c_int32, C.c_int32, vp]
        d.kvae_enc_mid_bwd.restype = C.c_int
        d.kvae_enc_mid_partial_rows.argtypes = [C.c_int64, C.c_int32]
        d.kvae_dec_up_fwd.argtypes = [vp, vp, vp, vp, C.c_int64, C.c_int32, C.c_int32, vp]
        d.kvae_dec_up_fwd.restype = C.c_int
        d.kvae_dec_up_bwd.argtypes = [vp] * 7 + [C.c_int64, C.c_int32, C.c_int32, vp]
        d.kvae_dec_up_bwd.restype = C.c_int
        d.kvae_dec_up_partial_rows.argtypes = [C.c_int64, C.c_int32]
        d.kvae_enc_head_fwd.argtypes = [vp] * 9 + [C.c_int64, C.c_int32, C.c_int32, C.c_float, vp]
        d.kvae_enc_head_fwd.restype = C.c_int
        d.kvae_enc_head_bwd.argtypes = [vp] * 11 + [C.c_int64, C.c_int32, C.c_int32, C.c_float, vp]
        d.kvae_enc_head_bwd.restype = C.c_int
        d.kvae_dec_fc_fwd.argtypes = [vp] * 4 + [C.c_int64, C.c_int32, C.c_int32, vp]
        d.kvae_dec_fc_fwd.restype = C.c_int
        d.kvae_dec_fc_bwd.argtypes = [vp] * 6 + [C.c_int64, C.c_int32, C.c_int32, vp]
        d.kvae_dec_fc_bwd.restype = C.c_int
        d.kvae_head_partial_rows.argtypes = []
        d.kvae_head_partial_rows.restype = C.c_int64
        d.kvae_latent_reg_fwd.argtypes = [vp] * 4 + [C.c_int64, C.c_int32, vp]
        d.kvae_latent_reg_fwd.restype = C.c_int
        d.kvae_latent_reg_bwd.argtypes = [vp] * 7 + [C.c_int64, C.c_int32, vp]
        d.kvae_latent_reg_bwd.restype = C.c_int
        d.kvae_loss_head_fwd.argtypes = [vp] * 5 + [C.c_float] * 3 + [vp, vp, vp, C.c_int64, vp]
        d.kvae_loss_head_fwd.restype = C.c_int
        d.kvae_loss_head_bwd.argtypes = [vp, vp, vp, vp, vp, vp, C.c_int64, vp]
        d.kvae_loss_head_bwd.restype = C.c_int
        d.kvae_dec_up_partial_rows.restype = C.c_int64
        d.kvae_dec_up_set_workgroups.argtypes = [C.c_int32]
        d.kvae_dec_up_set_workgroups.restype = C.c_int32
        d.kvae_enc_mid_partial_rows.restype = C.c_int64
        d.kvae_conv_edge_partial_rows.argtypes = [C.c_int64]
        d.kvae_conv_edge_partial_rows.restype = C.c_int64
        d.kvae_colsum.argtypes = [vp, vp, C.c_int64, C.c_int64, vp]
        d.kvae_colsum.restype = C.c_int
        d.kvae_colsum2.argtypes = [vp, vp, C.c_int64, C.c_int64, vp, vp, C.c_int64, C.c_int64, vp]
        d.kvae_colsum2.restype = C.c_int
        d.kvae_lgssm_emission_means.argtypes = [P, vp, vp, vp, vp, vp]
        d.kvae_lgssm_emission_means.restype = C.c_int
        d.kvae_rnn_wgrad_ws_floats.argtypes = [C.POINTER(WgradProblem), C.c_int32]
        d.kvae_rnn_wgrad_ws_floats.restype = C.c_int64
        d.kvae_rnn_wgrad.argtypes = [C.POINTER(WgradProblem), C.c_int32, vp, vp]
        d.kvae_rnn_wgrad.restype = C.c_int
        d.kvae_linear_fwd.argtypes = [vp, C.c_int64, C.c_int64, C.c_int32, vp, vp, C.c_int32, C.c_int32, vp, vp]
        d.kvae_linear_fwd.restype = C.c_int
        d.kvae_linear_bwd_input.argtypes = [vp, vp, C.c_int64, C.c_int32, vp, C.c_int32, vp, vp, C.c_int64, vp]
        d.kvae_linear_bwd_input.restype = C.c_int
        d.kvae_clip_adam.argtypes = [vp, vp, vp, vp, C.c_int64, vp, C.c_int32, vp, vp, vp, C.c_float, C.c_float, C.c_float, C.c_float,
                                     C.c_float, C.c_float, vp, vp, vp, vp]
        d.kvae_clip_adam.restype = C.c_int
        d.kvae_bias_partial_rows.argtypes = [C.c_int64]
        d.kvae_bias_partial_rows.restype = C.c_int64
        d.kvae_abi_version.restype = C.c_int
        d.kvae_last_error.restype = C.c_char_p
        d.kvae_build_info.restype = C.c_char_p
        if d.kvae_abi_version() != ABI_VERSION:
            raise OSError(f"{self.path}: ABI {d.kvae_abi_version()} != expected {ABI_VERSION}")

    def check(self, rc, what):
        if rc != 0:
            detail = self.dll.kvae_last_error().decode() if rc == 3 else ""
            raise RuntimeError(f"{what} failed: {_STATUS.get(rc, rc)} {detail}")

    @property
    def build_info(self):
        return self.dll.kvae_build_info().decode()


_hip_lib = None
_test_backend = None


def hip_lib():
    global _hip_lib
    if _hip_lib is None:
        if not LIB_PATH.exists():
            raise RuntimeError(
                f"HIP library {LIB_PATH} is missing. Build it with `python __graft_entry__.py build` "
                "(hipcc --offload-arch=gfx950). There is no CPU fallback for the LGSSM path.")
        _hip_lib = LgssmLib(LIB_PATH)
    return _hip_lib


def _set_test_backend(lib):
    global _test_backend
    _test_backend = lib


def fused_ok(t: torch.Tensor) -> bool:
    return t.is_cuda or _test_backend is not None


def lib_for(t: torch.Tensor):
    if t.is_cuda:
        return hip_lib()
    if _test_backend is not None:
        return _test_backend
    raise RuntimeError(
        "kvae LGSSM ops run only on a HIP device (MI355X): got a CPU tensor and there is no CPU fallback. "
        "Move the model and inputs to 'cuda'.")


def stream_for(t: torch.Tensor):
    if t.is_cuda:
        return C.c_void_p(torch.cuda.current_stream(t.device).cuda_stream)
    return C.c_void_p(0)


def ptr(t):
    return C.c_void_p(t.data_ptr()) if t is not None else C.c_void_p(0)


_prof = None


def profile_start():
    global _prof
    _prof = {}


def profile_stop():
    global _prof
    rec, _prof = _prof, None
    torch.cuda.synchronize()
    return {k: [s.elapsed_time(e) for s, e in v] for k, v in (rec or {}).items()}


def timed(name, t, thunk):
    if _prof is None or not t.is_cuda:
        return thunk()
    s, e = torch.cuda.Event(enable_timing=True), torch.cuda.Event(enable_timing=True)
    s.record()
    rc = thunk()
    e.record()
    _prof.setdefault(name, []).append((s, e))
    return rc


def _colsum_raw(p2):
    import torch
    out = torch.empty(p2.shape[1], device=p2.device, dtype=torch.float32)
    lib = lib_for(p2)
    lib.check(lib.dll.kvae_colsum(ptr(p2), ptr(out), p2.shape[0], p2.shape[1], stream_for(p2)), "kvae_colsum")
    return out


def colsum_pair(a, b):
    import torch
    a2, b2 = a.reshape(a.shape[0], -1).contiguous(), b.reshape(b.shape[0], -1).contiguous()
    tall = [p.shape[0] >= 1024 and p.shape[1] < 4096 for p in (a2, b2)]
    if a2.device != b2.device or tall[0] != tall[1] or (tall[0] and (a2.shape[0] != b2.shape[0] or a2.shape[0] % 64)):
        return colsum(a), colsum(b)

    def pair(x, y):
        ox = torch.empty(x.shape[1], device=x.device, dtype=torch.float32)
        oy = torch.empty(y.shape[1], device=y.device, dtype=torch.float32)
        lib = lib_for(x)
        lib.check(lib.dll.kvae_colsum2(ptr(x), ptr(ox), x.shape[0], x.shape[1], ptr(y), ptr(oy), y.shape[0], y.shape[1],
                                       stream_for(x)), "kvae_colsum2")
        return ox, oy

    if tall[0]:
        rows = a2.shape[0]
        fa, fb = pair(a2.view(64, (rows // 64) * a2.shape[1]), b2.view(64, (rows // 64) * b2.shape[1]))
        a2, b2 = fa.view(rows // 64, a2.shape[1]), fb.view(rows // 64, b2.shape[1])
    oa, ob = pair(a2, b2)
    return oa.view(a.shape[1:]), ob.view(b.shape[1:])


def colsum(partials):
    p2 = partials.reshape(partials.shape[0], -1).contiguous()
    rows, cols = p2.shape
    if rows >= 1024 and cols < 4096:
        r1 = 64
        while r1 > 1 and rows % r1:
            r1 //= 2
        if r1 > 1:
            p2 = _colsum_raw(p2.view(r1, (rows // r1) * cols)).view(rows // r1, cols)
    return _colsum_raw(p2).view(partials.shape[1:])
```

### kalman-vae_amd/kvae/model/model.py

```python
import os

import torch
from torch import nn

from kvae import _native, noise
from kvae.kalman import dyn_param as base_dyn_param
from kvae.kalman import lgssm_ops, switch_dyn_param
from kvae.kalman.kalman_filter import KalmanFilter
from kvae.noise import take as _take_noise
from kvae.vae.losses import LinearScheduler, count_active_units, vae_loss
from kvae.vae.vae import Decoder, Encoder


_FAST_PATH_NOTES = {
    "lgssm_specialised": "(z,u,a) is neither (4,4,2) nor (16,16,2): the LGSSM runs the run-time-dimension kernels",
    "lstm_registers": "alpha-net shape is not (hidden 50, a_dim 2): the LSTM runs the run-time-shape kernel",
    "bigru_registers": "regime posterior shape is not (hidden 50, a_dim 2): the bi-GRU runs on nn.GRU (MIOpen), "
                       "which cannot be captured into a hipGraph",
    "vae_default_shapes": "frame VAE is not the reference's default (32x32x1, channels [32,32,32], a_dim 2): "
                          "convolutions run on MIOpen with fused epilogues",
}


class _SideGradJoin(torch.autograd.Function):

    @staticmethod
    def forward(ctx, a, holder):
        ctx.holder = holder
        return a.view_as(a)

    @staticmethod
    def backward(ctx, g):
        h = ctx.holder
        torch.cuda.current_stream().wait_stream(h["side"])
        ga = h["a_side"].grad
        if ga is None:
            raise RuntimeError("KVAE.early_kf_backward is on but the LGSSM branch has no gradient yet: call "
                               "compute_loss() (which runs that branch's backward) before loss.backward(), or clear the flag")
        return g + ga, None


_LOSS_HEAD = os.environ.get("KVAE_LOSS_HEAD")


class KVAE(nn.Module):
    early_kf_backward = False
    lgssm_stream = None
    kf_value_only = False

    def __init__(self, config):
        super().__init__()
        if hasattr(config, "validate"):
            config.validate()
            slow = [k for k, v in config.fast_path().items() if not v and k in _FAST_PATH_NOTES]
            if slow:
                import warnings
                warnings.warn("KVAE: " + "; ".join(_FAST_PATH_NOTES[k] for k in slow), stacklevel=2)
        self.config = config
        self.encoder = Encoder(config)
        self.decoder = Decoder(config)
        self.scheduler = LinearScheduler(config)
        self.beta = self.scheduler.get_beta(0) if config.scheduled_beta else 1.0
        self.K, self.z_dim, self.a_dim, self.u_dim = config.num_modes, config.z_dim, config.a_dim, config.u_dim

        A0 = torch.eye(self.z_dim).repeat(self.K, 1, 1)
        B0 = torch.randn(self.K, self.z_dim, self.u_dim) * config.init_kf_matrices
        C0 = torch.randn(self.K, self.a_dim, self.z_dim) * config.init_kf_matrices
        kind = config.dynamics_model.lower()
        if kind == "switching":
            prior = switch_dyn_param.StickyRegimePrior(self.K, p_stay=config.sticky_p_stay)
            posterior = switch_dyn_param.MarkovVariationalRegimePosterior(
                self.K, input_dim=self.a_dim, hidden_size=config.dynamics_hidden_dim)
            Q0 = torch.eye(self.z_dim).repeat(self.K, 1, 1) * config.noise_transition
            dynamics = switch_dyn_param.SwitchingDynamicsParameter(
                A0, B0, C0, Q=Q0, prior=prior, hidden_lstm=config.dynamics_hidden_dim,
                markov_regime_posterior=posterior)
            dynamics.tau = config.tau_init
        elif kind == "lstm":
            dynamics = base_dyn_param.DynamicsParameter(A0, B0, C0, hidden_lstm=config.dynamics_hidden_dim)
        else:
            raise ValueError(f"Unknown dynamics model: {config.dynamics_model}")
        self.kalman_filter = KalmanFilter(config.noise_transition ** 0.5, config.noise_emission ** 0.5,
                                          torch.zeros(self.z_dim), torch.eye(self.z_dim) * config.init_cov, dynamics)

    def reparameterize(self, mu, var):
        std = torch.sqrt(var + 1e-6)
        eps = noise.take("eps_a")
        eps = torch.randn_like(std) if eps is None else eps.to(device=std.device, dtype=std.dtype).reshape(std.shape)
        return mu + eps * std

    def encode_sequence(self, x):
        lead = x.shape[:2]
        feat = self.encoder.features(x.flatten(0, 1))
        eps = noise.take("eps_a")
        if eps is None:
            eps = torch.randn(feat.shape[0], self.config.a_dim, device=feat.device, dtype=feat.dtype)
        else:
            eps = eps.to(device=feat.device, dtype=feat.dtype).reshape(feat.shape[0], self.config.a_dim)
        a, mu, var = self.encoder.heads(feat, eps)
        return a.unflatten(0, lead), mu.unflatten(0, lead), var.unflatten(0, lead)

    def decode_sequence(self, a):
        return self.decoder(a.flatten(0, 1)).unflatten(0, a.shape[:2])

    def _to_pixels(self, logits):
        return torch.sigmoid(logits) if self.config.out_distr.lower() == "bernoulli" else logits

    def forward(self, x, u=None, mask=None, with_recon=True):
        a_samples, a_mu, a_var = self.encode_sequence(x)
        if u is None:
            u = torch.zeros(x.shape[0], x.shape[1], self.u_dim, device=x.device, dtype=x.dtype)
        self.kalman_filter.dyn_params.reset_state()
        side = self.lgssm_stream if (self.training and a_samples.is_cuda) else None
        a_side = None
        value_only = self.kf_value_only and self.training
        if side is not None:
            side.wait_stream(torch.cuda.current_stream())
            a_lgssm = a_samples.detach() if value_only else a_samples
            if self.early_kf_backward and not value_only and torch.is_grad_enabled() and a_samples.requires_grad:
                a_side = a_lgssm = a_samples.detach().requires_grad_(True)
                a_samples = _SideGradJoin.apply(a_samples, {"a_side": a_side, "side": side})
            with torch.cuda.stream(side), torch.set_grad_enabled(torch.is_grad_enabled() and not value_only):
                smoothed = self.kalman_filter.smooth(a_lgssm, u, mask=mask)
        elif value_only:
            with torch.no_grad():
                smoothed = self.kalman_filter.smooth(a_samples.detach(), u, mask=mask)
        else:
            smoothed = self.kalman_filter.smooth(a_samples, u, mask=mask)
        (mus_smooth, Sigmas_smooth, mus_filt, Sigmas_filt, mus_pred, Sigmas_pred, A_list, B_list, C_list) = smoothed
        x_logits = self.decode_sequence(a_samples)
        return {
            "x_recon": self._to_pixels(x_logits) if with_recon else None, "x_logits": x_logits,
            "a_samples": a_samples, "a_mu": a_mu, "a_var": a_var, "a_side": a_side,
            "mus_smooth": mus_smooth, "Sigmas_smooth": Sigmas_smooth,
            "mus_filt": mus_filt, "Sigmas_filt": Sigmas_filt,
            "mus_pred": mus_pred, "Sigmas_pred": Sigmas_pred,
            "ABC": (A_list, B_list, C_list), "u": u,
            "state_probs": self.kalman_filter.dyn_params.state_seq,
        }

    def compute_loss(self, x, outputs, kf_weight=1.0, vae_weight=1.0, mask=None, with_metrics=True, weights_dev=None):
        if weights_dev is not None:
            vae_weight, kf_weight = weights_dev[0], weights_dev[1]
        B, T = x.shape[:2]
        a, a_mu, a_var = outputs["a_samples"], outputs["a_mu"], outputs["a_var"]
        A_list, B_list, C_list = outputs["ABC"]
        u = outputs.get("u")
        if u is None:
            u = torch.zeros(B, T, self.u_dim, device=x.device, dtype=x.dtype)
        x_mu = outputs["x_logits"] if outputs.get("x_logits") is not None else outputs["x_recon"]
        side = self.lgssm_stream if (self.training and a.is_cuda) else None

        a_side = outputs.get("a_side")
        stats = None
        if with_metrics == "device":
            variances = a_mu.detach().reshape(-1, a_mu.shape[-1]).var(dim=0)
            stats = ((variances > 1e-2).sum(), variances)

        def kf_elbo():
            if self.kf_value_only and self.training:
                with torch.no_grad():
                    if side is None:
                        return self.kalman_filter.elbo(outputs["mus_smooth"], outputs["Sigmas_smooth"], a.detach(), u, A_list,
                                                       B_list, C_list, mask=mask)
                    with torch.cuda.stream(side):
                        v = self.kalman_filter.elbo(outputs["mus_smooth"], outputs["Sigmas_smooth"], a.detach(), u, A_list,
                                                    B_list, C_list, mask=mask)
                    torch.cuda.current_stream().wait_stream(side)
                    return v
            if a_side is not None:
                with torch.cuda.stream(side):
                    v = self.kalman_filter.elbo(outputs["mus_smooth"], outputs["Sigmas_smooth"], a_side, u, A_list, B_list,
                                                C_list, mask=mask)
                    done = torch.cuda.Event()
                    done.record(side)
                    v.backward((-kf_weight).reshape(v.shape) if torch.is_tensor(kf_weight) else torch.full_like(v, -float(kf_weight)))
                torch.cuda.current_stream().wait_event(done)
                return v.detach()
            if side is None:
                return self.kalman_filter.elbo(outputs["mus_smooth"], outputs["Sigmas_smooth"], a, u, A_list, B_list, C_list,
                                               mask=mask)
            with torch.cuda.stream(side):
                v = self.kalman_filter.elbo(outputs["mus_smooth"], outputs["Sigmas_smooth"], a, u, A_list, B_list, C_list,
                                            mask=mask)
            torch.cuda.current_stream().wait_stream(side)
            return v

        head = _LOSS_HEAD
        if head is None and (a_side is not None or (self.kf_value_only and self.training and side is not None)):
            head = "2"
        if ((head in ("1", "2") or (head is None and side is None)) and self.config.out_distr.lower() == "bernoulli"
                and _native.fused_ok(x_mu) and x_mu.dtype == torch.float32
                and x.dtype == torch.float32 and a.dtype == torch.float32 and not x.requires_grad):
            from kvae.vae.fused import BernoulliFrameLogLik, LatentReg, LossHead
            lpx = BernoulliFrameLogLik.apply(x_mu, x)
            regf = LatentReg.apply(a, a_mu, a_var)
            mk = None if mask is None else mask.to(device=x.device, dtype=torch.float32).reshape(B, T)
            if head == "2":
                z = getattr(self, "_zero_kf", None)
                if z is None or z.device != x.device:
                    z = self._zero_kf = torch.zeros(1, device=x.device, dtype=torch.float32)
                wd = weights_dev
                vae_loss_w, _, _, vae_elbo, recon, reg = LossHead.apply(
                    lpx, regf, z, mk, self.beta, self.config.scale_reconstruction, 0.0 if wd is not None else vae_weight, 0.0, wd)
                elbo_kf = kf_elbo()
                loss = vae_loss_w - kf_weight * elbo_kf
                out = {"loss": loss, "elbo_total": -loss.detach(), "elbo_kf": elbo_kf, "elbo_vae_total": vae_elbo,
                       "recon": recon, "kl": reg}
            else:
                elbo_kf = kf_elbo()
                loss, elbo_total, elbo_kf_v, vae_elbo, recon, reg = LossHead.apply(
                    lpx, regf, elbo_kf, mk, self.beta, self.config.scale_reconstruction,
                    0.0 if weights_dev is not None else vae_weight, 0.0 if weights_dev is not None else kf_weight, weights_dev)
                out = {"loss": loss, "elbo_total": elbo_total, "elbo_kf": elbo_kf_v, "elbo_vae_total": vae_elbo,
                       "recon": recon, "kl": reg}
        else:
            x_var = torch.tensor(self.config.noise_pixel_var, device=x.device, dtype=x_mu.dtype) \
                if self.config.out_distr.lower() != "bernoulli" else None
            vae_elbo, recon, reg = vae_loss(x, x_mu, x_var, a, a_mu, a_var,
                                            scale_reconstruction=self.config.scale_reconstruction, mask=mask,
                                            out_distr=self.config.out_distr, beta=self.beta)
            elbo_kf = kf_elbo()
            elbo_total = vae_weight * vae_elbo + kf_weight * elbo_kf
            out = {"loss": -elbo_total, "elbo_total": elbo_total, "elbo_kf": elbo_kf, "elbo_vae_total": vae_elbo,
                   "recon": recon, "kl": reg}
        if with_metrics == "device":
            out.update(active_units=stats[0], latent_variances=stats[1])
        elif with_metrics:
            active, variances = count_active_units(a_mu)
            out.update(active_units=active, latent_var_0=variances[0].item(), latent_var_1=variances[1].item())
        return out

    @torch.no_grad()
    def impute(self, x, mask, u=None):
        self.eval()
        mask = mask.to(device=x.device, dtype=x.dtype)
        out = self.forward(x, u=u, mask=mask)
        _, _, C_list = out["ABC"]
        a_imputed, a_filtered = self.kalman_filter.emission_means(out["mus_smooth"], out["mus_filt"], C_list)
        x2 = self._to_pixels(self.decode_sequence(torch.cat([a_imputed, a_filtered], 0)))
        x_imputed, x_filtered = x2.chunk(2, 0)
        return {"x_recon": out["x_recon"], "x_imputed": x_imputed, "x_filtered": x_filtered,
                "a_vae": out["a_samples"], "a_imputed": a_imputed, "a_filtered": a_filtered,
                "state_probs": out["state_probs"]}

    @torch.no_grad()
    def sample_imputations(self, x, mask, num_samples=1, u=None, noise=True, emission_noise=False, decode=True):
        num_samples = int(num_samples)
        if num_samples < 1:
            raise ValueError(f"sample_imputations: num_samples must be >= 1, got {num_samples}")
        Bsz, T = x.shape[:2]
        if mask is None or tuple(mask.shape) != (Bsz, T):
            raise ValueError(f"sample_imputations: mask must be [B, T] = [{Bsz}, {T}], got "
                             f"{None if mask is None else list(mask.shape)}")
        if u is not None and (u.dim() != 3 or u.shape[0] != Bsz or u.shape[1] != T or u.shape[2] != self.u_dim):
            raise ValueError(f"sample_imputations: u must be [B, T, m] = [{Bsz}, {T}, {self.u_dim}], got {list(u.shape)}")
        was_training = self.training
        self.eval()
        try:
            a_vae, _, _ = self.encode_sequence(x)
            dev, dt = a_vae.device, a_vae.dtype
            u = torch.zeros(Bsz, T, self.u_dim, device=dev, dtype=dt) if u is None else u.to(device=dev, dtype=dt)
            self.kalman_filter.dyn_params.reset_state()
            post = self.kalman_filter.sample_posterior(a_vae, u, mask.to(device=dev, dtype=dt), num_samples, noise=noise,
                                                       emission_noise=emission_noise)
            a = post["a"]
            x_s = None
            if decode:
                x_s = self._to_pixels(self.decode_sequence(a.reshape(Bsz, num_samples * T, self.a_dim).to(dt))).unflatten(
                    1, (num_samples, T))
            return {"x": x_s, "a": a, "z": post["z"], "a_vae": a_vae, "state_probs": post["state_probs"],
                    "levels": post["levels"]}
        finally:
            self.train(was_training)

    @torch.no_grad()
    def generate(self, x, horizon, num_samples=1, u=None, mask=None, noise=True, decode=True):
        horizon, num_samples = int(horizon), int(num_samples)
        if horizon < 1:
            raise ValueError(f"generate: horizon must be >= 1, got {horizon}")
        if num_samples < 1:
            raise ValueError(f"generate: num_samples must be >= 1, got {num_samples}")
        Bsz, T0 = x.shape[:2]
        H, S = horizon, num_samples
        if u is not None and (u.dim() != 3 or u.shape[0] != Bsz or u.shape[1] != T0 + H or u.shape[2] != self.u_dim):
            raise ValueError(f"generate: u must be [B, T0+H, m] = [{Bsz}, {T0 + H}, {self.u_dim}], got {list(u.shape)}")
        was_training = self.training
        self.eval()
        try:
            kf, dyn = self.kalman_filter, self.kalman_filter.dyn_params
            a_vae, _, _ = self.encode_sequence(x)
            dev, dt = a_vae.device, a_vae.dtype
            if u is None:
                u_cond, u_fut = torch.zeros(Bsz, T0, self.u_dim, device=dev, dtype=dt), None
            else:
                u = u.to(device=dev, dtype=dt)
                u_cond, u_fut = u[:, :T0], u[:, T0:]
            hand = kf.condition(a_vae, u_cond, mask)
            n, p, K = self.z_dim, self.a_dim, self.K
            switching = dyn.is_switching_dynamics
            draws = dict(eps0=None, eps_z=None, eps_a=None, gumbel=None)
            L0 = LQ = LR = None
            if noise:
                def draw(slot, *shape):
                    v = _take_noise(slot)
                    return torch.randn(*shape, device=dev, dtype=dt) if v is None else v.to(device=dev, dtype=dt).reshape(shape)
                draws.update(eps0=draw("gen_z0", Bsz, S, n), eps_z=draw("gen_z", Bsz, S, H, n), eps_a=draw("gen_a", Bsz, S, H, p))
                if switching:
                    g = _take_noise("gen_gumbel")
                    draws["gumbel"] = (-torch.empty(Bsz, S, H, K, device=dev, dtype=dt).exponential_().log() if g is None
                                       else g.to(device=dev, dtype=dt).reshape(Bsz, S, H, K))
                L0 = lgssm_ops.safe_cholesky(hand["Sigma"])
                LQ = lgssm_ops.safe_cholesky(dyn.Q.detach() if switching else kf.Q)
                LR = lgssm_ops.safe_cholesky(kf.R)
            if switching:
                kind, extra = "switching", dict(P=dyn._prior_matrix(dev, dt), s0=hand["s"])
            elif K > 1:
                lstm = dyn.lstm
                kind, extra = "lstm", dict(lstm=tuple(t.detach() for t in (lstm.weight_ih_l0, lstm.weight_hh_l0, lstm.bias_ih_l0,
                                                                         lstm.bias_hh_l0, dyn.head_w.weight, dyn.head_w.bias)),
                                           h0=hand["h"], c0=hand["c"], y0=hand["y"])
            else:
                kind, extra = "lstm", {}
            a, z, w = lgssm_ops.rollout(kind, dyn.A.detach(), dyn.B.detach(), dyn.C.detach(), hand["mu"], L0, u_fut, LQ, LR, S, H,
                                        **extra, **draws)
            x_gen = None
            if decode:
                x_gen = self._to_pixels(self.decode_sequence(a.reshape(Bsz, S * H, p).to(dt))).unflatten(1, (S, H))
            return {"a": a, "z": z, "weights": w, "x": x_gen, "a_vae": a_vae}
        finally:
            self.train(was_training)
```

### kalman-vae_amd/kvae/vae/fused.py

```python
import torch

from .. import _native as N


colsum = N.colsum
colsum_pair = N.colsum_pair


def _chunks(n, size):
    return [(a, min(a + size, n)) for a in range(0, n, size)]


def _acc(total, part):
    return part if total is None else total + part


class BiasShuffleAct(torch.autograd.Function):

    @staticmethod
    def forward(ctx, x, bias, r, relu):
        x = x.contiguous()
        bias = bias.contiguous()
        Nb, Crr, H, W = x.shape
        C = Crr // (r * r)
        out = torch.empty(Nb, C, H * r, W * r, device=x.device, dtype=torch.float32)
        lib = N.lib_for(x)
        lib.check(lib.dll.kvae_bias_shuffle_act_fwd(N.ptr(x), N.ptr(bias), N.ptr(out), Nb, C, H, W, r, int(relu),
                                                    N.stream_for(x)), "kvae_bias_shuffle_act_fwd")
        ctx.r, ctx.relu, ctx.shape = r, relu, (Nb, C, H, W)
        ctx.save_for_backward(out if relu else None)
        return out

    @staticmethod
    def backward(ctx, g):
        (out,) = ctx.saved_tensors
        Nb, C, H, W = ctx.shape
        g = g.contiguous()
        g_in = torch.empty(Nb, C * ctx.r * ctx.r, H, W, device=g.device, dtype=torch.float32)
        lib = N.lib_for(g)
        partials = torch.empty(lib.dll.kvae_bias_partial_rows(Nb), C * ctx.r * ctx.r, device=g.device, dtype=torch.float32)
        lib.check(lib.dll.kvae_bias_shuffle_act_bwd(N.ptr(g), N.ptr(out), N.ptr(g_in), N.ptr(partials), Nb, C, H, W, ctx.r,
                                                    int(ctx.relu), N.stream_for(g)), "kvae_bias_shuffle_act_bwd")
        return g_in, colsum(partials), None, None


def conv_block(x, conv, r=1, relu=True):
    y = torch.nn.functional.conv2d(x, conv.weight, None, conv.stride, conv.padding, conv.dilation, conv.groups)
    return BiasShuffleAct.apply(y, conv.bias, r, relu)


class DecoderHead(torch.autograd.Function):

    SCRATCH = 2304

    @staticmethod
    def supported(h, conv):
        return (h.dim() == 4 and tuple(h.shape[1:]) == (32, 16, 16) and tuple(conv.weight.shape) == (4, 32, 3, 3)
                and conv.stride == (1, 1) and conv.padding == (1, 1) and conv.dilation == (1, 1) and conv.groups == 1
                and conv.bias is not None)

    @staticmethod
    def forward(ctx, h, weight, bias):
        h, weight, bias = h.contiguous(), weight.contiguous(), bias.contiguous()
        Nb, Cin, s, _ = h.shape
        logits = torch.empty(Nb, 1, 2 * s, 2 * s, device=h.device, dtype=torch.float32)
        scratch = torch.empty(DecoderHead.SCRATCH, device=h.device, dtype=torch.float32)
        lib = N.lib_for(h)
        lib.check(lib.dll.kvae_dec_head_fwd(N.ptr(h), N.ptr(weight), N.ptr(bias), N.ptr(logits), N.ptr(scratch), Nb, Cin, s,
                                            N.stream_for(h)), "kvae_dec_head_fwd")
        ctx.save_for_backward(h, weight)
        return logits

    @staticmethod
    def backward(ctx, g):
        h, weight = ctx.saved_tensors
        g = g.contiguous()
        Nb, Cin, s, _ = h.shape
        lib = N.lib_for(h)
        rows = lib.dll.kvae_conv_edge_partial_rows(Nb)
        g_h = torch.empty_like(h) if ctx.needs_input_grad[0] else None
        wp = torch.empty(rows, weight.numel(), device=h.device, dtype=torch.float32)
        bp = torch.empty(rows, 4, device=h.device, dtype=torch.float32)
        scratch = torch.empty(DecoderHead.SCRATCH, device=h.device, dtype=torch.float32)
        lib.check(lib.dll.kvae_dec_head_bwd(N.ptr(h), N.ptr(weight), N.ptr(g), N.ptr(g_h) if g_h is not None else None,
                                            N.ptr(wp), N.ptr(bp), N.ptr(scratch), Nb, Cin, s, N.stream_for(h)),
                  "kvae_dec_head_bwd")
        gw, gb = colsum_pair(wp, bp)
        return g_h, gw.view_as(weight), gb


class EncoderStem(torch.autograd.Function):

    @staticmethod
    def supported(x, conv):
        return (x.dim() == 4 and tuple(x.shape[1:]) == (1, 32, 32) and tuple(conv.weight.shape) == (32, 1, 3, 3)
                and conv.stride == (2, 2) and conv.padding == (1, 1) and conv.dilation == (1, 1) and conv.groups == 1
                and conv.bias is not None and not x.requires_grad)

    @staticmethod
    def forward(ctx, x, weight, bias):
        x, weight, bias = x.contiguous(), weight.contiguous(), bias.contiguous()
        Nb, _, s, _ = x.shape
        Cout = weight.shape[0]
        out = torch.empty(Nb, Cout, s // 2, s // 2, device=x.device, dtype=torch.float32)
        lib = N.lib_for(x)
        bits = torch.empty(Nb, (s // 2) ** 2, device=x.device, dtype=torch.int32) if (x.is_cuda and Cout == 32) else None
        lib.check(lib.dll.kvae_enc_stem_fwd(N.ptr(x), N.ptr(weight), N.ptr(bias), N.ptr(out), N.ptr(bits) if bits is not None else None,
                                            Nb, Cout, s, N.stream_for(x)), "kvae_enc_stem_fwd")
        ctx.save_for_backward(x, out, bits)
        ctx.wshape = weight.shape
        return out

    @staticmethod
    def backward(ctx, g):
        x, out, bits = ctx.saved_tensors
        g = g.contiguous()
        Nb, Cout = out.shape[:2]
        lib = N.lib_for(x)
        rows = lib.dll.kvae_conv_edge_partial_rows(Nb)
        wp = torch.empty(rows, Cout * 9, device=x.device, dtype=torch.float32)
        bp = torch.empty(rows, Cout, device=x.device, dtype=torch.float32)
        lib.check(lib.dll.kvae_enc_stem_bwd(N.ptr(x), N.ptr(out), N.ptr(bits) if bits is not None else None, N.ptr(g), N.ptr(wp),
                                            N.ptr(bp), Nb, Cout, x.shape[2], N.stream_for(x)), "kvae_enc_stem_bwd")
        gw, gb = colsum_pair(wp, bp)
        return None, gw.view(ctx.wshape), gb


class EncoderMid(torch.autograd.Function):

    @staticmethod
    def supported(x, conv):
        return (x.dim() == 4 and x.shape[1] == 32 and x.shape[2] == x.shape[3] and x.shape[2] in (16, 8)
                and tuple(conv.weight.shape) == (32, 32, 3, 3) and conv.stride == (2, 2) and conv.padding == (1, 1)
                and conv.dilation == (1, 1) and conv.groups == 1 and conv.bias is not None)

    CHUNK = 16384

    @staticmethod
    def forward(ctx, x, weight, bias):
        x, weight, bias = x.contiguous(), weight.contiguous(), bias.contiguous()
        Nb, Cc, s, _ = x.shape
        out = torch.empty(Nb, Cc, s // 2, s // 2, device=x.device, dtype=torch.float32)
        lib = N.lib_for(x)
        for a, b in _chunks(Nb, EncoderMid.CHUNK):
            lib.check(N.timed(f"enc_mid_fwd_s{s}", x, lambda: lib.dll.kvae_enc_mid_fwd(
                N.ptr(x[a:b]), N.ptr(weight), N.ptr(bias), N.ptr(out[a:b]), b - a, Cc, s, N.stream_for(x))), "kvae_enc_mid_fwd")
        ctx.save_for_backward(x, weight, out)
        return out

    @staticmethod
    def backward(ctx, g):
        x, weight, out = ctx.saved_tensors
        g = g.contiguous()
        Nb, Cc, s, _ = x.shape
        lib = N.lib_for(x)
        g_x = torch.empty_like(x) if ctx.needs_input_grad[0] else None
        gw = gb = None
        for a, b in _chunks(Nb, EncoderMid.CHUNK):
            rows = lib.dll.kvae_enc_mid_partial_rows(b - a, s)
            wp = torch.empty(rows, weight.numel(), device=x.device, dtype=torch.float32)
            bp = torch.empty(rows, Cc, device=x.device, dtype=torch.float32)
            lib.check(lib.dll.kvae_enc_mid_bwd(N.ptr(x[a:b]), N.ptr(weight), N.ptr(out[a:b]), N.ptr(g[a:b]),
                                               N.ptr(g_x[a:b]) if g_x is not None else None, N.ptr(wp), N.ptr(bp), b - a, Cc, s,
                                               N.stream_for(x)), "kvae_enc_mid_bwd")
            cw, cb = colsum_pair(wp, bp)
            gw, gb = _acc(gw, cw), _acc(gb, cb)
        return g_x, gw.view_as(weight), gb


class DecoderUp(torch.autograd.Function):

    CHUNK = 16384

    @staticmethod
    def supported(x, conv):
        return (x.dim() == 4 and x.shape[1] == 32 and x.shape[2] == x.shape[3] and x.shape[2] in (8, 4)
                and tuple(conv.weight.shape) == (128, 32, 3, 3) and conv.stride == (1, 1) and conv.padding == (1, 1)
                and conv.dilation == (1, 1) and conv.groups == 1 and conv.bias is not None)

    @staticmethod
    def forward(ctx, x, weight, bias):
        x, weight, bias = x.contiguous(), weight.contiguous(), bias.contiguous()
        Nb, Cin, s, _ = x.shape
        out = torch.empty(Nb, 32, 2 * s, 2 * s, device=x.device, dtype=torch.float32)
        lib = N.lib_for(x)
        for a, b in _chunks(Nb, DecoderUp.CHUNK):
            lib.check(N.timed(f"dec_up_fwd_s{s}", x, lambda: lib.dll.kvae_dec_up_fwd(
                N.ptr(x[a:b]), N.ptr(weight), N.ptr(bias), N.ptr(out[a:b]), b - a, Cin, s, N.stream_for(x))), "kvae_dec_up_fwd")
        ctx.save_for_backward(x, weight, out)
        return out

    @staticmethod
    def backward(ctx, g):
        x, weight, out = ctx.saved_tensors
        g = g.contiguous()
        Nb, Cin, s, _ = x.shape
        lib = N.lib_for(x)
        g_x = torch.empty_like(x) if ctx.needs_input_grad[0] else None
        gw = gb = None
        for a, b in _chunks(Nb, DecoderUp.CHUNK):
            rows = lib.dll.kvae_dec_up_partial_rows(b - a, s)
            wp = torch.empty(rows, weight.numel(), device=x.device, dtype=torch.float32)
            bp = torch.empty(rows, 128, device=x.device, dtype=torch.float32)
            lib.check(N.timed(f"dec_up_bwd_s{s}", x, lambda: lib.dll.kvae_dec_up_bwd(
                N.ptr(x[a:b]), N.ptr(weight), N.ptr(out[a:b]), N.ptr(g[a:b]), N.ptr(g_x[a:b]) if g_x is not None else None, N.ptr(wp),
                N.ptr(bp), b - a, Cin, s, N.stream_for(x))), "kvae_dec_up_bwd")
            cw, cb = colsum_pair(wp, bp)
            gw, gb = _acc(gw, cw), _acc(gb, cb)
        return g_x, gw.view_as(weight), gb


def _optr(t):
    return N.ptr(t) if t is not None else None


class EncoderHead(torch.autograd.Function):

    @staticmethod
    def supported(feat, fc_mu, fc_var_lin):
        return (feat.dim() == 2 and feat.shape[1] == 512 and tuple(fc_mu.weight.shape) == (2, 512)
                and tuple(fc_var_lin.weight.shape) == (2, 512) and fc_mu.bias is not None and fc_var_lin.bias is not None)

    @staticmethod
    def forward(ctx, feat, w_mu, b_mu, w_var, b_var, eps, ne):
        feat, w_mu, b_mu, w_var, b_var = (t.contiguous() for t in (feat, w_mu, b_mu, w_var, b_var))
        eps = eps.contiguous() if eps is not None else None
        Nb = feat.shape[0]
        mu, var, a = (torch.empty(Nb, 2, device=feat.device, dtype=torch.float32) for _ in range(3))
        lib = N.lib_for(feat)
        lib.check(lib.dll.kvae_enc_head_fwd(N.ptr(feat), N.ptr(w_mu), N.ptr(b_mu), N.ptr(w_var), N.ptr(b_var), _optr(eps),
                                            N.ptr(mu), N.ptr(var), N.ptr(a), Nb, 512, 2, float(ne), N.stream_for(feat)),
                  "kvae_enc_head_fwd")
        ctx.save_for_backward(feat, w_mu, w_var, var, eps)
        ctx.ne = float(ne)
        return a, mu, var

    @staticmethod
    def backward(ctx, g_a, g_mu, g_var):
        feat, w_mu, w_var, var, eps = ctx.saved_tensors
        g_a, g_mu, g_var = (t.contiguous() if t is not None else None for t in (g_a, g_mu, g_var))
        Nb = feat.shape[0]
        lib = N.lib_for(feat)
        rows = lib.dll.kvae_head_partial_rows()
        g_feat = torch.empty_like(feat)
        wp = torch.empty(rows, 4 * 512, device=feat.device, dtype=torch.float32)
        bp = torch.empty(rows, 4, device=feat.device, dtype=torch.float32)
        lib.check(lib.dll.kvae_enc_head_bwd(N.ptr(feat), N.ptr(w_mu), N.ptr(w_var), N.ptr(var), _optr(eps), _optr(g_a), _optr(g_mu),
                                            _optr(g_var), N.ptr(g_feat), N.ptr(wp), N.ptr(bp), Nb, 512, 2, ctx.ne,
                                            N.stream_for(feat)), "kvae_enc_head_bwd")
        gw, gb = colsum_pair(wp, bp)
        gw, gb = gw.view(2, 2, 512), gb.view(2, 2)
        return g_feat, gw[0], gb[0], gw[1], gb[1], None, None


class DecoderFc(torch.autograd.Function):

    @staticmethod
    def supported(a, fc):
        return a.dim() == 2 and a.shape[1] == 2 and tuple(fc.weight.shape) == (512, 2) and fc.bias is not None

    @staticmethod
    def forward(ctx, a, weight, bias):
        a, weight, bias = a.contiguous(), weight.contiguous(), bias.contiguous()
        Nb = a.shape[0]
        h = torch.empty(Nb, 512, device=a.device, dtype=torch.float32)
        lib = N.lib_for(a)
        lib.check(lib.dll.kvae_dec_fc_fwd(N.ptr(a), N.ptr(weight), N.ptr(bias), N.ptr(h), Nb, 512, 2, N.stream_for(a)),
                  "kvae_dec_fc_fwd")
        ctx.save_for_backward(a, weight)
        return h

    @staticmethod
    def backward(ctx, g):
        a, weight = ctx.saved_tensors
        g = g.contiguous()
        Nb = a.shape[0]
        lib = N.lib_for(a)
        rows = lib.dll.kvae_head_partial_rows()
        g_a = torch.empty_like(a)
        wp = torch.empty(rows, 1024, device=a.device, dtype=torch.float32)
        bp = torch.empty(rows, 512, device=a.device, dtype=torch.float32)
        lib.check(lib.dll.kvae_dec_fc_bwd(N.ptr(g), N.ptr(a), N.ptr(weight), N.ptr(g_a), N.ptr(wp), N.ptr(bp), Nb, 512, 2,
                                          N.stream_for(a)), "kvae_dec_fc_bwd")
        gw, gb = colsum_pair(wp, bp)
        return g_a, gw.view(512, 2), gb


class LatentReg(torch.autograd.Function):

    @staticmethod
    def forward(ctx, a, mu, var):
        a, mu, var = a.contiguous(), mu.contiguous(), var.contiguous()
        A = a.shape[-1]
        Nb = a.numel() // A
        reg = torch.empty(a.shape[:-1], device=a.device, dtype=torch.float32)
        lib = N.lib_for(a)
        lib.check(lib.dll.kvae_latent_reg_fwd(N.ptr(a), N.ptr(mu), N.ptr(var), N.ptr(reg), Nb, A, N.stream_for(a)),
                  "kvae_latent_reg_fwd")
        ctx.save_for_backward(a, mu, var)
        return reg

    @staticmethod
    def backward(ctx, g):
        a, mu, var = ctx.saved_tensors
        g = g.contiguous()
        A = a.shape[-1]
        g_a, g_mu, g_var = torch.empty_like(a), torch.empty_like(a), torch.empty_like(a)
        lib = N.lib_for(a)
        lib.check(lib.dll.kvae_latent_reg_bwd(N.ptr(a), N.ptr(mu), N.ptr(var), N.ptr(g), N.ptr(g_a), N.ptr(g_mu), N.ptr(g_var),
                                              a.numel() // A, A, N.stream_for(a)), "kvae_latent_reg_bwd")
        return g_a, g_mu, g_var


class LossHead(torch.autograd.Function):

    @staticmethod
    def forward(ctx, lpx, regf, elbo_kf, mask, beta, scale, vae_w, kf_w, weights=None):
        lpx, regf = lpx.contiguous(), regf.contiguous()
        mask = mask.contiguous() if mask is not None else None
        kf = elbo_kf.reshape(1).contiguous()
        b = beta.reshape(1).to(device=lpx.device, dtype=torch.float32).contiguous() if torch.is_tensor(beta) else \
            torch.full((1,), float(beta), device=lpx.device, dtype=torch.float32)
        out, coef = torch.empty(6, device=lpx.device, dtype=torch.float32), torch.empty(3, device=lpx.device, dtype=torch.float32)
        lib = N.lib_for(lpx)
        lib.check(lib.dll.kvae_loss_head_fwd(N.ptr(lpx), N.ptr(regf), _optr(mask), N.ptr(kf), N.ptr(b), float(scale), float(vae_w),
                                             float(kf_w), _optr(weights), N.ptr(out), N.ptr(coef), lpx.numel(), N.stream_for(lpx)),
                  "kvae_loss_head_fwd")
        ctx.save_for_backward(coef, mask)
        ctx.set_materialize_grads(False)
        ctx.shape, ctx.kf_shape = lpx.shape, elbo_kf.shape
        vals = out.unbind(0)
        ctx.mark_non_differentiable(*vals[1:])
        return vals

    @staticmethod
    def backward(ctx, g_loss, *_unused):
        if g_loss is None:
            return (None,) * 9
        coef, mask = ctx.saved_tensors
        g = g_loss.reshape(1).contiguous()
        g_lpx = torch.empty(ctx.shape, device=g.device, dtype=torch.float32)
        g_reg = torch.empty(ctx.shape, device=g.device, dtype=torch.float32)
        g_kf = torch.empty(1, device=g.device, dtype=torch.float32)
        lib = N.lib_for(g)
        lib.check(lib.dll.kvae_loss_head_bwd(N.ptr(g), N.ptr(coef), _optr(mask), N.ptr(g_lpx), N.ptr(g_reg), N.ptr(g_kf),
                                             g_lpx.numel(), N.stream_for(g)), "kvae_loss_head_bwd")
        return g_lpx, g_reg, g_kf.reshape(ctx.kf_shape), None, None, None, None, None, None


class BernoulliFrameLogLik(torch.autograd.Function):

    @staticmethod
    def forward(ctx, x_logits, x):
        lg, xx = x_logits.contiguous(), x.contiguous()
        lead = lg.shape[:2]
        frames = lead[0] * lead[1]
        pixels = lg.numel() // frames
        out = torch.empty(lead, device=lg.device, dtype=torch.float32)
        lib = N.lib_for(lg)
        lib.check(lib.dll.kvae_bce_frames_fwd(N.ptr(lg), N.ptr(xx), N.ptr(out), frames, pixels, N.stream_for(lg)),
                  "kvae_bce_frames_fwd")
        ctx.save_for_backward(lg, xx)
        return out

    @staticmethod
    def backward(ctx, g):
        lg, xx = ctx.saved_tensors
        g = g.contiguous()
        frames = g.numel()
        g_logits = torch.empty_like(lg)
        lib = N.lib_for(lg)
        lib.check(lib.dll.kvae_bce_frames_bwd(N.ptr(lg), N.ptr(xx), N.ptr(g), N.ptr(g_logits), frames, lg.numel() // frames,
                                              N.stream_for(lg)), "kvae_bce_frames_bwd")
        return g_logits, None
```

### kalman-vae_amd/kvae/vae/losses.py

```python
import math

import torch
import torch.nn.functional as F

from kvae.utils.config import KVAEConfig

_HALF_LOG_2PI = 0.5 * math.log(2.0 * math.pi)


def log_gaussian(x, mean, var):
    return -_HALF_LOG_2PI - 0.5 * torch.log(var) - (x - mean) ** 2 / (2 * var)


def _frame_mask(mask, x):
    B, T = x.shape[:2]
    if mask is None:
        return torch.ones(B, T, device=x.device, dtype=x.dtype)
    return mask.to(device=x.device, dtype=x.dtype).reshape(B, T)


def log_likelihood(x, x_mu, x_var, a, a_mu, a_var, mask=None):
    mk = _frame_mask(mask, x)
    lpx = log_gaussian(x, x_mu, x_var).sum(dim=(2, 3, 4))
    lqa = log_gaussian(a, a_mu, a_var).sum(dim=-1)
    return (lpx * mk).sum(), (lqa * mk).sum()


def vae_loss(x, x_mu, x_var, a, a_mu, a_var, scale_reconstruction: float = 0.3, beta: float = 1.0,
             mask=None, out_distr: str = "gaussian"):
    mk = _frame_mask(mask, x)
    denom = mk.sum().clamp(min=1.0)
    from kvae import _native
    if out_distr.lower() == "bernoulli" and _native.fused_ok(a) and a.dtype == torch.float32 and a_var.dim() == a.dim():
        from kvae.vae.fused import BernoulliFrameLogLik, LatentReg
        if x_mu.dtype == torch.float32 and x.dtype == torch.float32 and not x.requires_grad:
            lpx = BernoulliFrameLogLik.apply(x_mu, x)
        else:
            lpx = -F.binary_cross_entropy_with_logits(x_mu, x, reduction="none").sum(dim=(2, 3, 4))
        recon = (lpx * mk).sum() / denom
        reg = (LatentReg.apply(a, a_mu, a_var) * mk).sum() / denom
        return scale_reconstruction * recon + beta * reg, recon, reg
    if out_distr.lower() == "bernoulli":
        if _native.fused_ok(x_mu) and x_mu.dtype == torch.float32 and x.dtype == torch.float32 and not x.requires_grad:
            from kvae.vae.fused import BernoulliFrameLogLik
            lpx = BernoulliFrameLogLik.apply(x_mu, x)
        else:
            lpx = -F.binary_cross_entropy_with_logits(x_mu, x, reduction="none").sum(dim=(2, 3, 4))
        log_px = (lpx * mk).sum()
        log_qa = (log_gaussian(a, a_mu, a_var).sum(-1) * mk).sum()
    else:
        log_px, log_qa = log_likelihood(x, x_mu, x_var, a, a_mu, a_var, mask=mask)
    log_pa = ((-_HALF_LOG_2PI - 0.5 * a ** 2).sum(-1) * mk).sum()
    recon = log_px / denom
    reg = (log_pa - log_qa) / denom
    return scale_reconstruction * recon + beta * reg, recon, reg


class LinearScheduler:

    def __init__(self, config: KVAEConfig):
        self.start_epoch, self.end_epoch = config.start_epoch, config.end_epoch
        self.start_val, self.end_val = config.start_val, config.end_val

    def get_beta(self, current_epoch: int) -> float:
        if current_epoch < self.start_epoch:
            return self.start_val
        if current_epoch >= self.end_epoch:
            return self.end_val
        frac = (current_epoch - self.start_epoch) / (self.end_epoch - self.start_epoch)
        return self.start_val + frac * (self.end_val - self.start_val)


def count_active_units(mu_tensor, threshold=1e-2):
    mu = mu_tensor.reshape(-1, mu_tensor.shape[-1]) if mu_tensor.dim() == 3 else mu_tensor
    variances = mu.var(dim=0)
    return int((variances > threshold).sum().item()), variances
```

### kalman-vae_amd/kvae/vae/vae.py

```python
import os
from typing import Tuple

import torch
import torch.nn as nn

from kvae import _native
from kvae.utils.config import KVAEConfig
from kvae.vae.fused import DecoderFc, DecoderHead, DecoderUp, EncoderHead, EncoderMid, EncoderStem, conv_block


def _conv_out(size, k, s, p):
    return (size + 2 * p - k) // s + 1


class Encoder(nn.Module):

    def __init__(self, config: KVAEConfig):
        super().__init__()
        self.config = config
        blocks, c_in, side = [], config.img_channels, config.img_size
        for c_out in config.encoder_channels:
            blocks += [nn.Conv2d(c_in, c_out, config.encoder_kernel_size, config.encoder_stride,
                                 config.encoder_padding), nn.ReLU()]
            side = _conv_out(side, config.encoder_kernel_size, config.encoder_stride, config.encoder_padding)
            c_in = c_out
        self.conv_layers = nn.Sequential(*blocks)
        self.flat_size = c_in * side * side
        self.fc_mu = nn.Linear(self.flat_size, config.a_dim)
        self.fc_var = nn.Sequential(nn.Linear(self.flat_size, config.a_dim), nn.Sigmoid())

    def features(self, x: torch.Tensor) -> torch.Tensor:
        if _native.fused_ok(x) and x.dtype == torch.float32:
            h = x
            for i, layer in enumerate(self.conv_layers):
                if isinstance(layer, nn.Conv2d):
                    if i == 0 and EncoderStem.supported(h, layer):
                        h = EncoderStem.apply(h, layer.weight, layer.bias)
                    elif EncoderMid.supported(h, layer):
                        h = EncoderMid.apply(h, layer.weight, layer.bias)
                    else:
                        h = conv_block(h, layer, r=1, relu=True)
            return h.flatten(1)
        return self.conv_layers(x).flatten(1)

    def heads(self, feat: torch.Tensor, eps=None):
        if _native.fused_ok(feat) and feat.dtype == torch.float32 and EncoderHead.supported(feat, self.fc_mu, self.fc_var[0]):
            return EncoderHead.apply(feat, self.fc_mu.weight, self.fc_mu.bias, self.fc_var[0].weight, self.fc_var[0].bias,
                                     eps, self.config.noise_emission)
        mu, var = self.fc_mu(feat), self.config.noise_emission * self.fc_var(feat)
        return (mu if eps is None else mu + eps * torch.sqrt(var + 1e-6)), mu, var

    def forward(self, x: torch.Tensor) -> Tuple[torch.Tensor, torch.Tensor]:
        _, mu, var = self.heads(self.features(x))
        return mu, var


class Decoder(nn.Module):

    def __init__(self, config: KVAEConfig):
        super().__init__()
        self.config = config
        chans = list(config.decoder_channels)
        self.init_size = config.img_size // (2 ** len(chans))
        self.init_channels = chans[0]
        self.fc = nn.Linear(config.a_dim, self.init_channels * self.init_size ** 2)
        up = []
        for c_in, c_out in zip(chans[:-1], chans[1:]):
            up += [nn.Conv2d(c_in, 4 * c_out, kernel_size=3, padding=1), nn.PixelShuffle(2), nn.ReLU()]
        up += [nn.Conv2d(chans[-1], 4 * config.img_channels, kernel_size=3, padding=1), nn.PixelShuffle(2)]
        self.deconv_layers = nn.Sequential(*up)

    def forward(self, a: torch.Tensor) -> torch.Tensor:
        fused = _native.fused_ok(a) and a.dtype == torch.float32
        h = DecoderFc.apply(a, self.fc.weight, self.fc.bias) if fused and DecoderFc.supported(a, self.fc) else self.fc(a)
        h = h.unflatten(1, (self.init_channels, self.init_size, self.init_size))
        if not fused:
            return self.deconv_layers(h)
        layers = list(self.deconv_layers)
        for i, layer in enumerate(layers):
            if isinstance(layer, nn.Conv2d):
                relu = i + 2 < len(layers) and isinstance(layers[i + 2], nn.ReLU)
                if not relu and DecoderHead.supported(h, layer):
                    h = DecoderHead.apply(h, layer.weight, layer.bias)
                elif relu and DecoderUp.supported(h, layer):
                    h = DecoderUp.apply(h, layer.weight, layer.bias)
                else:
                    h = conv_block(h, layer, r=2, relu=relu)
        return h


class VAE(nn.Module):

    def __init__(self, config: KVAEConfig):
        super().__init__()
        self.config = config
        self.encoder = Encoder(config)
        self.decoder = Decoder(config)

    def encode(self, x):
        return self.encoder(x)

    def decode(self, a):
        return self.decoder(a)

    def reparameterize(self, mu, var):
        return mu + torch.randn_like(var) * var.sqrt()

    def forward(self, x: torch.Tensor) -> dict:
        lead = x.shape[:2]
        mu, var = self.encode(x.flatten(0, 1))
        a = self.reparameterize(mu, var)
        x_mu = self.decode(a)
        x_rec = torch.sigmoid(x_mu) if self.config.out_distr.lower() == "bernoulli" else x_mu
        back = lambda t: t.unflatten(0, lead)
        return {"x_recon": back(x_rec), "x_recon_mu": back(x_mu),
                "x_recon_var": torch.tensor(self.config.noise_pixel_var, device=x.device, dtype=x_mu.dtype),
                "a_vae": back(a), "a_mu": back(mu), "a_var": back(var)}

    def sample_from_prior(self, n: int = 1, device=None) -> torch.Tensor:
        device = device or next(self.parameters()).device
        return self.decode(torch.randn(n, self.config.a_dim, device=device))

    @classmethod
    def load_from_checkpoint(cls, checkpoint_path: str, config: KVAEConfig = None, device: str = "cpu"):
        if not os.path.exists(checkpoint_path):
            raise FileNotFoundError(checkpoint_path)
        vae = cls(config or KVAEConfig())
        payload = torch.load(checkpoint_path, map_location=device, weights_only=True)
        for key in ("state_dict", "model_state"):
            if isinstance(payload, dict) and key in payload:
                payload = payload[key]
        for part in ("encoder", "decoder"):
            sub = {k.split(part + ".", 1)[1]: v for k, v in payload.items() if (part + ".") in k}
            if sub:
                getattr(vae, part).load_state_dict(sub)
        return vae.to(device)
```

Baseline: 91880 sequences/s.

## Fuse decoder head with BCE loss, add ReLU bitmasks to enc mid, GPU active units

Adds a fused decoder-head kernel that computes the logits and, in the same pass, the sigmoid reconstruction, the unscaled gradient (x - sigmoid) and per-frame BCE log-likelihood. The backward pass scales that stored gradient by the per-frame upstream gradient inside the data and weight-gradient kernels, which removes the separate BCE forward and backward kernels and their extra passes over the 32x32 logits. It also adds encoder-mid conv variants that save packed ReLU bitmasks instead of the full float output for backward, and a single-block GPU kernel for the active-unit statistics. The changes add more code paths and gated Python branches, and the active-unit kernel runs in one workgroup.

Result: faster. 93360 sequences/s, median of 6 (+1.6%).

```diff
diff --git a/include/kvae_lgssm.h b/include/kvae_lgssm.h
--- a/include/kvae_lgssm.h
+++ b/include/kvae_lgssm.h
@@ -8,7 +8,7 @@
 #endif
 
 #define KVAE_MAX_DIM 16
-#define KVAE_ABI_VERSION 12
+#define KVAE_ABI_VERSION 13
 
 typedef enum {
   KVAE_OK = 0,
@@ -169,6 +169,12 @@
                       int32_t Cin, int32_t side, void *stream);
 int kvae_dec_head_bwd(const float *in, const float *W, const float *g_logits, float *g_in, float *w_partials,
                       float *b_partials, float *w_scratch, int64_t N, int32_t Cin, int32_t side, void *stream);
+int kvae_dec_head_fwd_loss(const float *in, const float *W, const float *bias, const float *x, float *logits, float *x_recon,
+                           float *g_unscaled, float *frame_ll, float *w_scratch, int64_t N, int32_t Cin, int32_t side,
+                           void *stream);
+int kvae_dec_head_bwd_loss(const float *in, const float *W, const float *g_unscaled, const float *g_frame, float *g_in,
+                           float *w_partials, float *b_partials, float *w_scratch, int64_t N, int32_t Cin, int32_t side,
+                           void *stream);
 int kvae_enc_stem_fwd(const float *x, const float *W, const float *bias, float *out, uint32_t *relu_bits, int64_t N, int32_t Cout,
                       int32_t side, void *stream);
 int kvae_enc_stem_bwd(const float *x, const float *out, const uint32_t *relu_bits, const float *g_out, float *w_partials,
@@ -180,6 +186,12 @@
 int kvae_enc_mid_bwd(const float *in, const float *W, const float *out, const float *g_out, float *g_in,
                      float *w_partials, float *b_partials, int64_t N, int32_t C, int32_t side, void *stream);
 int64_t kvae_enc_mid_partial_rows(int64_t N, int32_t side);
+int kvae_enc_mid_fwd_bits(const float *in, const float *W, const float *bias, float *out, uint32_t *relu_bits, int64_t N, int32_t C,
+                          int32_t side, void *stream);
+int kvae_enc_mid_bwd_bits(const float *in, const float *W, const uint32_t *relu_bits, const float *g_out, float *g_in,
+                          float *w_partials, float *b_partials, int64_t N, int32_t C, int32_t side, void *stream);
+
+int kvae_active_units(const float *mu, int64_t N, int32_t A, float threshold, float *variances, int64_t *count, void *stream);
 
 int kvae_dec_up_fwd(const float *x, const float *W, const float *bias, float *out, int64_t N, int32_t Cin, int32_t side,
                     void *stream);
diff --git a/kalman-vae_amd/csrc/kvae_vae.hip b/kalman-vae_amd/csrc/kvae_vae.hip
--- a/kalman-vae_amd/csrc/kvae_vae.hip
+++ b/kalman-vae_amd/csrc/kvae_vae.hip
@@ -388,6 +388,32 @@
                                                                                                      b_partials, N);
   return launch_status("k_dec_head_wrw");
 }
+int kvae_dec_head_fwd_loss(const float *in, const float *W, const float *bias, const float *x, float *logits, float *x_recon,
+                           float *g_unscaled, float *frame_ll, float *w_scratch, int64_t N, int32_t Cin, int32_t side,
+                           void *stream) {
+  if (!in || !W || !bias || !x || !logits || !g_unscaled || !frame_ll || !w_scratch) return KVAE_ERR_NULL;
+  if (N < 1) return KVAE_ERR_ARG;
+  if (Cin != DH_CI || side != DH_S) return KVAE_ERR_DIMS;
+  k_dec_head_prep<<<dim3(1), dim3(256), 0, (hipStream_t)stream>>>(W, w_scratch);
+  k_dec_head_fwd_loss<<<dim3((unsigned)N), dim3(256), 0, (hipStream_t)stream>>>(in, w_scratch, bias, x, logits, x_recon, g_unscaled,
+                                                                                frame_ll);
+  return launch_status("k_dec_head_fwd_loss");
+}
+int kvae_dec_head_bwd_loss(const float *in, const float *W, const float *g_unscaled, const float *g_frame, float *g_in,
+                           float *w_partials, float *b_partials, float *w_scratch, int64_t N, int32_t Cin, int32_t side,
+                           void *stream) {
+  if (!in || !g_unscaled || !g_frame || !w_partials || !b_partials || !w_scratch) return KVAE_ERR_NULL;
+  if (N < 1) return KVAE_ERR_ARG;
+  if (Cin != DH_CI || side != DH_S) return KVAE_ERR_DIMS;
+  if (g_in) {
+    k_dec_head_bwd_data_scaled<<<dim3((unsigned)N), dim3(256), 0, (hipStream_t)stream>>>(g_unscaled, g_frame, w_scratch, g_in);
+    const int rc = launch_status("k_dec_head_bwd_data_scaled");
+    if (rc) return rc;
+  }
+  k_dec_head_wrw_scaled<<<dim3((unsigned)kvae_conv_edge_partial_rows(N)), dim3(256), 0, (hipStream_t)stream>>>(
+      in, g_unscaled, g_frame, w_partials, b_partials, N);
+  return launch_status("k_dec_head_wrw_scaled");
+}
 int kvae_enc_stem_fwd(const float *x, const float *W, const float *bias, float *out, uint32_t *relu_bits, int64_t N, int32_t Cout,
                       int32_t side, void *stream) {
   if (!x || !W || !bias || !out) return KVAE_ERR_NULL;
@@ -444,6 +470,32 @@
   if (side == 16) k_enc_mid_wrw<16><<<grid, dim3(256), 0, (hipStream_t)stream>>>(in, out, g_out, w_partials, b_partials, N);
   else k_enc_mid_wrw<8><<<grid, dim3(256), 0, (hipStream_t)stream>>>(in, out, g_out, w_partials, b_partials, N);
   return launch_status("k_enc_mid_wrw");
+}
+int kvae_enc_mid_fwd_bits(const float *in, const float *W, const float *bias, float *out, uint32_t *relu_bits, int64_t N, int32_t C,
+                          int32_t side, void *stream) {
+  if (!in || !W || !bias || !out || !relu_bits) return KVAE_ERR_NULL;
+  if (N < 1 || (N + 256 * 8) * EM_C * side * side * 4 >= EM_MAX_BYTES) return KVAE_ERR_ARG;
+  if (C != EM_C || (side != 16 && side != 8)) return KVAE_ERR_DIMS;
+  const dim3 grid((unsigned)enc_mid_grid(N, side));
+  if (side == 16) k_enc_mid_fwd_bits<16><<<grid, dim3(256), 0, (hipStream_t)stream>>>(in, W, bias, out, relu_bits, N);
+  else k_enc_mid_fwd_bits<8><<<grid, dim3(256), 0, (hipStream_t)stream>>>(in, W, bias, out, relu_bits, N);
+  return launch_status("k_enc_mid_fwd_bits");
+}
+int kvae_enc_mid_bwd_bits(const float *in, const float *W, const uint32_t *relu_bits, const float *g_out, float *g_in,
+                          float *w_partials, float *b_partials, int64_t N, int32_t C, int32_t side, void *stream) {
+  if (!in || !W || !relu_bits || !g_out || !w_partials || !b_partials) return KVAE_ERR_NULL;
+  if (N < 1 || (N + 256 * 8) * EM_C * side * side * 4 >= EM_MAX_BYTES) return KVAE_ERR_ARG;
+  if (C != EM_C || (side != 16 && side != 8)) return KVAE_ERR_DIMS;
+  const dim3 grid((unsigned)enc_mid_grid(N, side));
+  if (g_in) {
+    if (side == 16) k_enc_mid_bwd_data_bits<16><<<grid, dim3(256), 0, (hipStream_t)stream>>>(W, relu_bits, g_out, g_in, N);
+    else k_enc_mid_bwd_data_bits<8><<<grid, dim3(256), 0, (hipStream_t)stream>>>(W, relu_bits, g_out, g_in, N);
+    const int rc = launch_status("k_enc_mid_bwd_data_bits");
+    if (rc) return rc;
+  }
+  if (side == 16) k_enc_mid_wrw_bits<16><<<grid, dim3(256), 0, (hipStream_t)stream>>>(in, relu_bits, g_out, w_partials, b_partials, N);
+  else k_enc_mid_wrw_bits<8><<<grid, dim3(256), 0, (hipStream_t)stream>>>(in, relu_bits, g_out, w_partials, b_partials, N);
+  return launch_status("k_enc_mid_wrw_bits");
 }
 }
 
@@ -515,8 +567,16 @@
 }
 
 #include "vae_heads.h"
+#include "vae_stats.h"
 extern "C" {
 int64_t kvae_head_partial_rows(void) { return HD_WAVES; }
+
+int kvae_active_units(const float *mu, int64_t N, int32_t A, float threshold, float *variances, int64_t *count, void *stream) {
+  if (!mu || !variances || !count) return KVAE_ERR_NULL;
+  if (N < 1 || N > AU_MAX_ROWS || A < 1) return KVAE_ERR_ARG;
+  k_active_units<<<dim3(1), dim3(AU_THREADS), 0, (hipStream_t)stream>>>(mu, N, A, threshold, variances, count);
+  return launch_status("k_active_units");
+}
 
 int kvae_enc_head_fwd(const float *feat, const float *Wmu, const float *bmu, const float *Wvar, const float *bvar,
                       const float *eps, float *mu, float *var, float *a, int64_t N, int32_t F, int32_t A,
diff --git a/kalman-vae_amd/csrc/vae_conv_edge.h b/kalman-vae_amd/csrc/vae_conv_edge.h
--- a/kalman-vae_amd/csrc/vae_conv_edge.h
+++ b/kalman-vae_amd/csrc/vae_conv_edge.h
@@ -1,6 +1,8 @@
 #pragma once
 #include <hip/hip_runtime.h>
 #include <stdint.h>
+
+#include "vae_loss.h"
 
 namespace kvae {
 
@@ -35,8 +37,11 @@
   d[0] = v.x; d[1] = v.y; d[2] = v.z; d[3] = v.w;
 }
 
-__global__ __launch_bounds__(256) void k_dec_head_fwd(const float *__restrict__ in, const float *__restrict__ scratch,
-                                                      const float *__restrict__ bias, float *__restrict__ logits) {
+template <bool LOSS>
+__device__ __forceinline__ void dh_fwd_body(const float *__restrict__ in, const float *__restrict__ scratch,
+                                            const float *__restrict__ bias, float *__restrict__ logits,
+                                            const float *__restrict__ x, float *__restrict__ x_recon,
+                                            float *__restrict__ g_unscaled, float *__restrict__ frame_ll) {
   __shared__ float tile[DH_CI * 256];
   const int64_t n = blockIdx.x;
   const float4 *src = reinterpret_cast<const float4 *>(in + n * DH_CI * 256);
@@ -68,18 +73,64 @@
       a23 += wv.zw * v;
     }
   }
-  float *o = logits + n * 1024 + (2 * h) * 32 + 2 * w;
+  const int64_t po = n * 1024 + (2 * h) * 32 + 2 * w;
+  float2 x0, x1;
+  if constexpr (LOSS) {
+    x0 = *reinterpret_cast<const float2 *>(x + po);
+    x1 = *reinterpret_cast<const float2 *>(x + po + 32);
+  }
+  float *o = logits + po;
   *reinterpret_cast<float2 *>(o) = make_float2(a01.x, a01.y);
   *reinterpret_cast<float2 *>(o + 32) = make_float2(a23.x, a23.y);
-}
-
-__global__ __launch_bounds__(256) void k_dec_head_bwd_data(const float *__restrict__ g_logits,
-                                                           const float *__restrict__ scratch, float *__restrict__ g_in) {
+  if constexpr (LOSS) {
+    const float s00 = sigmoid_stable(a01.x), s01 = sigmoid_stable(a01.y), s10 = sigmoid_stable(a23.x), s11 = sigmoid_stable(a23.y);
+    if (x_recon) {
+      *reinterpret_cast<float2 *>(x_recon + po) = make_float2(s00, s01);
+      *reinterpret_cast<float2 *>(x_recon + po + 32) = make_float2(s10, s11);
+    }
+    *reinterpret_cast<float2 *>(g_unscaled + po) = make_float2(x0.x - s00, x0.y - s01);
+    *reinterpret_cast<float2 *>(g_unscaled + po + 32) = make_float2(x1.x - s10, x1.y - s11);
+    const float b00 = bce_logit(a01.x, x0.x), b01 = bce_logit(a01.y, x0.y), b10 = bce_logit(a23.x, x1.x), b11 = bce_logit(a23.y, x1.y);
+    const float n00 = __shfl_down(b00, 1, 64), n01 = __shfl_down(b01, 1, 64), n10 = __shfl_down(b10, 1, 64), n11 = __shfl_down(b11, 1, 64);
+    __syncthreads();
+    if ((w & 1) == 0) {
+      tile[(2 * h) * 8 + (w >> 1)] = b00 + b01 + n00 + n01;
+      tile[(2 * h + 1) * 8 + (w >> 1)] = b10 + b11 + n10 + n11;
+    }
+    __syncthreads();
+    if (threadIdx.x < 64) {
+      float acc = 0.f;
+#pragma unroll
+      for (int k = 0; k < 4; ++k) acc += tile[threadIdx.x + 64 * k];
+      for (int off = 32; off > 0; off >>= 1) acc += __shfl_down(acc, off, 64);
+      if (threadIdx.x == 0) frame_ll[n] = -acc;
+    }
+  }
+}
+__global__ __launch_bounds__(256) void k_dec_head_fwd(const float *__restrict__ in, const float *__restrict__ scratch,
+                                                      const float *__restrict__ bias, float *__restrict__ logits) {
+  dh_fwd_body<false>(in, scratch, bias, logits, nullptr, nullptr, nullptr, nullptr);
+}
+__global__ __launch_bounds__(256) void k_dec_head_fwd_loss(const float *__restrict__ in, const float *__restrict__ scratch,
+                                                           const float *__restrict__ bias, const float *__restrict__ x,
+                                                           float *__restrict__ logits, float *__restrict__ x_recon,
+                                                           float *__restrict__ g_unscaled, float *__restrict__ frame_ll) {
+  dh_fwd_body<true>(in, scratch, bias, logits, x, x_recon, g_unscaled, frame_ll);
+}
+
+template <bool SCALED>
+__device__ __forceinline__ void dh_bwd_data_body(const float *__restrict__ g_logits, const float *__restrict__ g_frame,
+                                                 const float *__restrict__ scratch, float *__restrict__ g_in) {
   __shared__ float gt[DH_CO * DH_CS];
   const int64_t n = blockIdx.x;
   float gp[4];
 #pragma unroll
   for (int j = 0; j < 4; ++j) gp[j] = g_logits[n * 1024 + threadIdx.x + 256 * j];
+  if constexpr (SCALED) {
+    const float gf = g_frame[n];
+#pragma unroll
+    for (int j = 0; j < 4; ++j) gp[j] = gf * gp[j];
+  }
   dh_zero_halo(gt, DH_CO);
 #pragma unroll
   for (int j = 0; j < 4; ++j) {
@@ -110,9 +161,20 @@
     o[(2 * j + 1) * 256] = acc[j].y;
   }
 }
-
-__global__ __launch_bounds__(256) void k_dec_head_wrw(const float *__restrict__ in, const float *__restrict__ g_logits,
-                                                      float *__restrict__ partial, float *__restrict__ partial_b, int64_t N) {
+__global__ __launch_bounds__(256) void k_dec_head_bwd_data(const float *__restrict__ g_logits,
+                                                           const float *__restrict__ scratch, float *__restrict__ g_in) {
+  dh_bwd_data_body<false>(g_logits, nullptr, scratch, g_in);
+}
+__global__ __launch_bounds__(256) void k_dec_head_bwd_data_scaled(const float *__restrict__ g_unscaled,
+                                                                  const float *__restrict__ g_frame,
+                                                                  const float *__restrict__ scratch, float *__restrict__ g_in) {
+  dh_bwd_data_body<true>(g_unscaled, g_frame, scratch, g_in);
+}
+
+template <bool SCALED>
+__device__ __forceinline__ void dh_wrw_body(const float *__restrict__ in, const float *__restrict__ g_logits,
+                                            const float *__restrict__ g_frame, float *__restrict__ partial,
+                                            float *__restrict__ partial_b, int64_t N) {
   constexpr int CS = 257, OOB = 1 << 24;
   __shared__ float lds[DH_CI * CS + DH_CO * 256];
   __shared__ float redb[8 * DH_CO];
@@ -128,7 +190,7 @@
 #pragma unroll
   for (int co = 0; co < DH_CO; ++co) accb[co] = 0.f;
   float4 pre[8];
-  float gp[4];
+  float gp[4], gf = 1.f;
   int64_t n = blockIdx.x;
   if (n < N) {
     const float4 *src = reinterpret_cast<const float4 *>(in + n * DH_CI * 256);
@@ -136,6 +198,7 @@
     for (int j = 0; j < 8; ++j) pre[j] = src[tin + 256 * j];
 #pragma unroll
     for (int j = 0; j < 4; ++j) gp[j] = g_logits[n * 1024 + threadIdx.x + 256 * j];
+    if constexpr (SCALED) gf = g_frame[n];
   }
   for (; n < N; n += gridDim.x) {
     __syncthreads();
@@ -148,7 +211,7 @@
 #pragma unroll
     for (int j = 0; j < 4; ++j) {
       const int i = threadIdx.x + 256 * j, oh = i >> 5, ow = i & 31, co = (oh & 1) * 2 + (ow & 1);
-      gt[co * 256 + (oh >> 1) * 16 + (ow >> 1)] = gp[j];
+      gt[co * 256 + (oh >> 1) * 16 + (ow >> 1)] = SCALED ? gf * gp[j] : gp[j];
     }
     __syncthreads();
     const int64_t nn = n + gridDim.x;
@@ -158,6 +221,7 @@
       for (int j = 0; j < 8; ++j) pre[j] = src[tin + 256 * j];
 #pragma unroll
       for (int j = 0; j < 4; ++j) gp[j] = g_logits[nn * 1024 + threadIdx.x + 256 * j];
+      if constexpr (SCALED) gf = g_frame[nn];
     }
 #pragma unroll
     for (int rr = 0; rr < 2; ++rr) {
@@ -212,6 +276,15 @@
     for (int gq = 0; gq < 8; ++gq) s += redb[gq * 4 + threadIdx.x];
     partial_b[(int64_t)blockIdx.x * DH_CO + threadIdx.x] = s;
   }
+}
+__global__ __launch_bounds__(256) void k_dec_head_wrw(const float *__restrict__ in, const float *__restrict__ g_logits,
+                                                      float *__restrict__ partial, float *__restrict__ partial_b, int64_t N) {
+  dh_wrw_body<false>(in, g_logits, nullptr, partial, partial_b, N);
+}
+__global__ __launch_bounds__(256) void k_dec_head_wrw_scaled(const float *__restrict__ in, const float *__restrict__ g_unscaled,
+                                                             const float *__restrict__ g_frame, float *__restrict__ partial,
+                                                             float *__restrict__ partial_b, int64_t N) {
+  dh_wrw_body<true>(in, g_unscaled, g_frame, partial, partial_b, N);
 }
 
 
diff --git a/kalman-vae_amd/csrc/vae_conv_mid.h b/kalman-vae_amd/csrc/vae_conv_mid.h
--- a/kalman-vae_amd/csrc/vae_conv_mid.h
+++ b/kalman-vae_amd/csrc/vae_conv_mid.h
@@ -38,6 +38,16 @@
 __device__ __forceinline__ void em_st4(__amdgpu_buffer_rsrc_t r, uint32_t byte_off, const float4 v) {
   const em_u4 u = {__float_as_uint(v.x), __float_as_uint(v.y), __float_as_uint(v.z), __float_as_uint(v.w)};
   __builtin_amdgcn_raw_buffer_store_b128(u, r, byte_off, 0, 0);
+}
+__device__ __forceinline__ uint32_t em_ld1u(__amdgpu_buffer_rsrc_t r, uint32_t byte_off) {
+  return __builtin_amdgcn_raw_buffer_load_b32(r, byte_off, 0, 0);
+}
+__device__ __forceinline__ void em_st1u(__amdgpu_buffer_rsrc_t r, uint32_t byte_off, uint32_t v) {
+  __builtin_amdgcn_raw_buffer_store_b32(v, r, byte_off, 0, 0);
+}
+__device__ __forceinline__ float4 em_mask4(const float4 g, const uint4 m, int c) {
+  return make_float4((m.x >> c) & 1u ? g.x : 0.f, (m.y >> c) & 1u ? g.y : 0.f, (m.z >> c) & 1u ? g.z : 0.f,
+                     (m.w >> c) & 1u ? g.w : 0.f);
 }
 __device__ __forceinline__ void em_st1(__amdgpu_buffer_rsrc_t r, uint32_t byte_off, float v) {
   __builtin_amdgcn_raw_buffer_store_b32(__float_as_uint(v), r, byte_off, 0, 0);
@@ -51,9 +61,10 @@
 #define KV_MFMA_F32(a, b, c) __builtin_amdgcn_mfma_f32_32x32x2f32((a), (b), (c), 0, 0, 0)
 #define KV_ACC_ROW(r, half) (((r) & 3) + 8 * ((r) >> 2) + 4 * (half))
 
-template <int S>
-__global__ __launch_bounds__(256) void k_enc_mid_fwd(const float *__restrict__ in, const float *__restrict__ W,
-                                                     const float *__restrict__ bias, float *__restrict__ out, int64_t N) {
+template <int S, bool BITS>
+__device__ __forceinline__ void em_fwd_body(const float *__restrict__ in, const float *__restrict__ W,
+                                            const float *__restrict__ bias, float *__restrict__ out,
+                                            uint32_t *__restrict__ bits, int64_t N) {
   using D = EmDims<S>;
   __shared__ float lds[EM_W + D::IT_IN + D::IT_OUT];
   float *Wl = lds, *fr = lds + EM_W, *ot = fr + D::IT_IN;
@@ -70,7 +81,9 @@
   for (int r = 0; r < 16; ++r) bv[r] = bias[KV_ACC_ROW(r, half)];
 
   const int rot = blockIdx.x & 15;
-  const __amdgpu_buffer_rsrc_t rin = em_rsrc(in, total * 4), rout = em_rsrc(out, N * EM_C * D::PF * 4);
+  const __amdgpu_buffer_rsrc_t rin = em_rsrc(in, total * 4), rout = em_rsrc(out, N * EM_C * D::PF * 4),
+                               rbits = em_rsrc(bits, BITS ? N * D::PF * 4 : 0);
+  uint32_t word = 0, word_off = 0x80000000u;
   float4 pre[16];
   int64_t it = blockIdx.x;
   auto fetch1 = [&](int64_t i, int j) {
@@ -111,6 +124,7 @@
       if (g + 2 < 36) rd(g + 2);
       if (g < 4) flush1(g);
       else if (g < 20) fetch1(it + gridDim.x, g - 4);
+      else if (BITS && g == 20) em_st1u(rbits, word_off, word);
       __builtin_amdgcn_sched_barrier(0);
 #pragma unroll
       for (int u = 0; u < 4; ++u) acc = KV_MFMA_F32(av[g][u], bw[g][u], acc);
@@ -119,22 +133,45 @@
     EM_STAMP(slot, 5);
     __syncthreads();
     EM_STAMP(slot, 6);
-#pragma unroll
-    for (int r = 0; r < 16; ++r) ot[(fl * EM_C + KV_ACC_ROW(r, half)) * D::PF + pix] = fmaxf(acc[r] + bv[r], 0.f);
+    uint32_t wbits = 0;
+#pragma unroll
+    for (int r = 0; r < 16; ++r) {
+      const float v = acc[r] + bv[r];
+      ot[(fl * EM_C + KV_ACC_ROW(r, half)) * D::PF + pix] = fmaxf(v, 0.f);
+      if constexpr (BITS) wbits |= (v > 0.f ? 1u : 0u) << KV_ACC_ROW(r, half);
+    }
     EM_STAMP(slot, 7);
     done_base = (uint32_t)(it * D::IT_OUT) * 4u;
+    if constexpr (BITS) {
+      word = wbits | __shfl_xor(wbits, 32, 64);
+      word_off = half == 0 ? (uint32_t)(it * 128 + gp) * 4u : 0x80000000u;
+    }
   }
   __syncthreads();
 #pragma unroll
   for (int j = 0; j < 4; ++j) flush1(j);
-}
-
-template <int S>
-__global__ __launch_bounds__(256) void k_enc_mid_bwd_data(const float *__restrict__ W, const float *__restrict__ out,
-                                                          const float *__restrict__ g_out, float *__restrict__ g_in, int64_t N) {
+  if constexpr (BITS) em_st1u(rbits, word_off, word);
+}
+template <int S>
+__global__ __launch_bounds__(256) void k_enc_mid_fwd(const float *__restrict__ in, const float *__restrict__ W,
+                                                     const float *__restrict__ bias, float *__restrict__ out, int64_t N) {
+  em_fwd_body<S, false>(in, W, bias, out, nullptr, N);
+}
+template <int S>
+__global__ __launch_bounds__(256) void k_enc_mid_fwd_bits(const float *__restrict__ in, const float *__restrict__ W,
+                                                          const float *__restrict__ bias, float *__restrict__ out,
+                                                          uint32_t *__restrict__ bits, int64_t N) {
+  em_fwd_body<S, true>(in, W, bias, out, bits, N);
+}
+
+template <int S, bool BITS>
+__device__ __forceinline__ void em_bwd_data_body(const float *__restrict__ W, const float *__restrict__ out,
+                                                 const uint32_t *__restrict__ bits, const float *__restrict__ g_out,
+                                                 float *__restrict__ g_in, int64_t N) {
   using D = EmDims<S>;
-  __shared__ float lds[EM_W + D::IT_OUT + D::IT_IN];
+  __shared__ __attribute__((aligned(16))) float lds[EM_W + D::IT_OUT + D::IT_IN + (BITS ? 128 : 0)];
   float *Wl = lds, *gm = lds + EM_W, *ot = gm + D::IT_OUT;
+  uint32_t *mw = reinterpret_cast<uint32_t *>(ot + D::IT_IN);
   const int tid = threadIdx.x, lane = tid & 63, wv = tid >> 6, q = lane & 31, half = lane >> 5;
   em_load_weights(Wl, W, false);
   const int64_t iters = (N + D::FPI - 1) / D::FPI, total_in = N * D::FRAME, total_out = N * EM_C * D::PF;
@@ -146,14 +183,16 @@
   const int obase = fl * D::FRAME + (2 * a_) * S + 2 * b_;
 
   const int rot = blockIdx.x & 15;
-  const __amdgpu_buffer_rsrc_t rg = em_rsrc(g_out, total_out * 4), ro = em_rsrc(out, total_out * 4),
-                               rgi = em_rsrc(g_in, total_in * 4);
+  const __amdgpu_buffer_rsrc_t rg = em_rsrc(g_out, total_out * 4), ro = em_rsrc(BITS ? nullptr : out, BITS ? 0 : total_out * 4),
+                               rb = em_rsrc(bits, BITS ? N * D::PF * 4 : 0), rgi = em_rsrc(g_in, total_in * 4);
   float4 pg[4], po[4];
+  uint32_t pm = 0;
   int64_t it = blockIdx.x;
   auto fetch1 = [&](int64_t i, int j) {
     const uint32_t e = (uint32_t)(i * D::IT_OUT + (tid + 256 * (((j & 3) + rot) & 3)) * 4) * 4u;
     if (j < 4) pg[j] = em_ld4(rg, e);
-    else po[j - 4] = em_ld4(ro, e);
+    else if constexpr (!BITS) po[j - 4] = em_ld4(ro, e);
+    else if (j == 4) pm = em_ld1u(rb, tid < 128 ? (uint32_t)(i * 128 + tid) * 4u : 0x80000000u);
   };
   uint32_t done_base = 0x80000000u;
   auto flush1 = [&](int j) {
@@ -163,12 +202,22 @@
 #pragma unroll
   for (int j = 0; j < 8; ++j) fetch1(it, j);
   for (; it < iters; it += gridDim.x) {
-    __syncthreads();
-#pragma unroll
-    for (int j = 0; j < 4; ++j)
-      reinterpret_cast<float4 *>(gm)[tid + 256 * ((j + rot) & 3)] =
-          make_float4(po[j].x > 0.f ? pg[j].x : 0.f, po[j].y > 0.f ? pg[j].y : 0.f, po[j].z > 0.f ? pg[j].z : 0.f,
-                      po[j].w > 0.f ? pg[j].w : 0.f);
+    if constexpr (BITS) {
+      if (tid < 128) mw[tid] = pm;
+    }
+    __syncthreads();
+#pragma unroll
+    for (int j = 0; j < 4; ++j) {
+      if constexpr (BITS) {
+        const int e = (tid + 256 * ((j + rot) & 3)) * 4, f = e / (EM_C * D::PF), c = (e / D::PF) % EM_C, p = e % D::PF;
+        reinterpret_cast<float4 *>(gm)[tid + 256 * ((j + rot) & 3)] =
+            em_mask4(pg[j], *reinterpret_cast<const uint4 *>(mw + f * D::PF + p), c);
+      } else {
+        reinterpret_cast<float4 *>(gm)[tid + 256 * ((j + rot) & 3)] =
+            make_float4(po[j].x > 0.f ? pg[j].x : 0.f, po[j].y > 0.f ? pg[j].y : 0.f, po[j].z > 0.f ? pg[j].z : 0.f,
+                        po[j].w > 0.f ? pg[j].w : 0.f);
+      }
+    }
     __syncthreads();
     constexpr int E_CLS[9] = {3, 3, 3, 3, 1, 1, 2, 2, 0};
     constexpr int E_KY[9] = {0, 0, 2, 2, 1, 1, 0, 2, 1};
@@ -212,15 +261,27 @@
 #pragma unroll
   for (int j = 0; j < 16; ++j) flush1(j);
 }
-
-template <int S>
-__global__ __launch_bounds__(256) void k_enc_mid_wrw(const float *__restrict__ in, const float *__restrict__ out,
-                                                     const float *__restrict__ g_out, float *__restrict__ w_partials,
-                                                     float *__restrict__ b_partials, int64_t N) {
+template <int S>
+__global__ __launch_bounds__(256) void k_enc_mid_bwd_data(const float *__restrict__ W, const float *__restrict__ out,
+                                                          const float *__restrict__ g_out, float *__restrict__ g_in, int64_t N) {
+  em_bwd_data_body<S, false>(W, out, nullptr, g_out, g_in, N);
+}
+template <int S>
+__global__ __launch_bounds__(256) void k_enc_mid_bwd_data_bits(const float *__restrict__ W, const uint32_t *__restrict__ bits,
+                                                               const float *__restrict__ g_out, float *__restrict__ g_in,
+                                                               int64_t N) {
+  em_bwd_data_body<S, true>(W, nullptr, bits, g_out, g_in, N);
+}
+
+template <int S, bool BITS>
+__device__ __forceinline__ void em_wrw_body(const float *__restrict__ in, const float *__restrict__ out,
+                                            const uint32_t *__restrict__ bits, const float *__restrict__ g_out,
+                                            float *__restrict__ w_partials, float *__restrict__ b_partials, int64_t N) {
   using D = EmDims<S>;
   constexpr int CSP = D::PLANE + 1, GSP = D::PF + 1;
-  __shared__ float lds[D::FPI * EM_C * GSP + D::FPI * EM_C * CSP];
+  __shared__ __attribute__((aligned(16))) float lds[D::FPI * EM_C * GSP + D::FPI * EM_C * CSP + (BITS ? 128 : 0)];
   float *gm = lds, *xin = lds + D::FPI * EM_C * GSP;
+  uint32_t *mw = reinterpret_cast<uint32_t *>(xin + D::FPI * EM_C * CSP);
   const int tid = threadIdx.x, lane = tid & 63, wv = tid >> 6, q = lane & 31, half = lane >> 5;
   const int64_t iters = (N + D::FPI - 1) / D::FPI, total_in = N * D::FRAME, total_out = N * EM_C * D::PF;
   const int wframe = S == 16 ? (wv >> 1) : 2 * wv, wpix0 = S == 16 ? 32 * (wv & 1) : 0;
@@ -239,8 +300,10 @@
 
   const int rot = blockIdx.x & 15;
   const __amdgpu_buffer_rsrc_t rin = em_rsrc(in, total_in * 4), rg = em_rsrc(g_out, total_out * 4),
-                               ro = em_rsrc(out, total_out * 4);
+                               ro = em_rsrc(BITS ? nullptr : out, BITS ? 0 : total_out * 4),
+                               rb = em_rsrc(bits, BITS ? N * D::PF * 4 : 0);
   float4 px[16], pg[4], po[4];
+  uint32_t pm = 0;
   int64_t it = blockIdx.x;
   const int tin = S == 16 ? ((lane >> 4) << 6) | (wv << 4) | (lane & 15) : tid;
   auto fetch1 = [&](int64_t i, int j) {
@@ -249,12 +312,16 @@
     } else {
       const uint32_t e = (uint32_t)(i * D::IT_OUT + (tid + 256 * (((j & 3) + rot) & 3)) * 4) * 4u;
       if (j < 20) pg[j - 16] = em_ld4(rg, e);
-      else po[j - 20] = em_ld4(ro, e);
+      else if constexpr (!BITS) po[j - 20] = em_ld4(ro, e);
+      else if (j == 20) pm = em_ld1u(rb, tid < 128 ? (uint32_t)(i * 128 + tid) * 4u : 0x80000000u);
     }
   };
 #pragma unroll
   for (int j = 0; j < 24; ++j) fetch1(it, j);
   for (; it < iters; it += gridDim.x) {
+    if constexpr (BITS) {
+      if (tid < 128) mw[tid] = pm;
+    }
     __syncthreads();
 #pragma unroll
     for (int j = 0; j < 16; ++j) {
@@ -266,8 +333,13 @@
     for (int j = 0; j < 4; ++j) {
       const int e = (tid + 256 * ((j + rot) & 3)) * 4, f = e / (EM_C * D::PF), c = (e / D::PF) % EM_C, p = e % D::PF;
       float *d = gm + (f * EM_C + c) * GSP + p;
-      d[0] = po[j].x > 0.f ? pg[j].x : 0.f; d[1] = po[j].y > 0.f ? pg[j].y : 0.f;
-      d[2] = po[j].z > 0.f ? pg[j].z : 0.f; d[3] = po[j].w > 0.f ? pg[j].w : 0.f;
+      if constexpr (BITS) {
+        const float4 md = em_mask4(pg[j], *reinterpret_cast<const uint4 *>(mw + f * D::PF + p), c);
+        d[0] = md.x; d[1] = md.y; d[2] = md.z; d[3] = md.w;
+      } else {
+        d[0] = po[j].x > 0.f ? pg[j].x : 0.f; d[1] = po[j].y > 0.f ? pg[j].y : 0.f;
+        d[2] = po[j].z > 0.f ? pg[j].z : 0.f; d[3] = po[j].w > 0.f ? pg[j].w : 0.f;
+      }
     }
     __syncthreads();
     float av[16], bw[16][9];
@@ -315,5 +387,17 @@
   for (int i = tid; i < EM_W; i += 256) w_partials[(int64_t)blockIdx.x * EM_W + i] = red[i];
   if (tid < EM_C) b_partials[(int64_t)blockIdx.x * EM_C + tid] = redb[tid] + redb[EM_C + tid];
 }
-
-}
+template <int S>
+__global__ __launch_bounds__(256) void k_enc_mid_wrw(const float *__restrict__ in, const float *__restrict__ out,
+                                                     const float *__restrict__ g_out, float *__restrict__ w_partials,
+                                                     float *__restrict__ b_partials, int64_t N) {
+  em_wrw_body<S, false>(in, out, nullptr, g_out, w_partials, b_partials, N);
+}
+template <int S>
+__global__ __launch_bounds__(256) void k_enc_mid_wrw_bits(const float *__restrict__ in, const uint32_t *__restrict__ bits,
+                                                          const float *__restrict__ g_out, float *__restrict__ w_partials,
+                                                          float *__restrict__ b_partials, int64_t N) {
+  em_wrw_body<S, true>(in, nullptr, bits, g_out, w_partials, b_partials, N);
+}
+
+}
diff --git a/kalman-vae_amd/csrc/vae_host_twins.h b/kalman-vae_amd/csrc/vae_host_twins.h
--- /dev/null
+++ b/kalman-vae_amd/csrc/vae_host_twins.h
@@ -0,0 +1,88 @@
+#pragma once
+#include <stdint.h>
+
+#include <vector>
+
+#include "../../include/kvae_lgssm.h"
+
+extern "C" {
+int kvae_enc_mid_fwd_bits(const float *in, const float *W, const float *bias, float *out, uint32_t *relu_bits, int64_t N, int32_t C,
+                          int32_t side, void *stream) {
+  if (!in || !W || !bias || !out || !relu_bits) return KVAE_ERR_NULL;
+  const int rc = kvae_enc_mid_fwd(in, W, bias, out, N, C, side, stream);
+  if (rc != KVAE_OK) return rc;
+  const int64_t PF = (int64_t)(side / 2) * (side / 2);
+  for (int64_t n = 0; n < N; ++n)
+    for (int64_t p = 0; p < PF; ++p) {
+      uint32_t w = 0;
+      for (int co = 0; co < C; ++co) w |= (out[(n * C + co) * PF + p] > 0.f ? 1u : 0u) << co;
+      relu_bits[n * PF + p] = w;
+    }
+  return KVAE_OK;
+}
+int kvae_enc_mid_bwd_bits(const float *in, const float *W, const uint32_t *relu_bits, const float *g_out, float *g_in,
+                          float *w_partials, float *b_partials, int64_t N, int32_t C, int32_t side, void *stream) {
+  if (!in || !W || !relu_bits || !g_out || !w_partials || !b_partials) return KVAE_ERR_NULL;
+  if (N < 1) return KVAE_ERR_ARG;
+  if (C != 32 || (side != 16 && side != 8)) return KVAE_ERR_DIMS;
+  const int64_t PF = (int64_t)(side / 2) * (side / 2);
+  std::vector<float> sign((size_t)(N * C * PF));
+  for (int64_t n = 0; n < N; ++n)
+    for (int co = 0; co < C; ++co)
+      for (int64_t p = 0; p < PF; ++p) sign[(n * C + co) * PF + p] = (relu_bits[n * PF + p] >> co) & 1u ? 1.0f : 0.0f;
+  return kvae_enc_mid_bwd(in, W, sign.data(), g_out, g_in, w_partials, b_partials, N, C, side, stream);
+}
+
+int kvae_dec_head_fwd_loss(const float *in, const float *W, const float *bias, const float *x, float *logits, float *x_recon,
+                           float *g_unscaled, float *frame_ll, float *w_scratch, int64_t N, int32_t Cin, int32_t side,
+                           void *stream) {
+  if (!x || !g_unscaled || !frame_ll) return KVAE_ERR_NULL;
+  int rc = kvae_dec_head_fwd(in, W, bias, logits, w_scratch, N, Cin, side, stream);
+  if (rc != KVAE_OK) return rc;
+  const int32_t pixels = 4 * side * side;
+  rc = kvae_bce_frames_fwd(logits, x, frame_ll, N, pixels, stream);
+  if (rc != KVAE_OK) return rc;
+  for (int64_t i = 0; i < N * pixels; ++i) {
+    const float s = kvae::sigmoid_stable(logits[i]);
+    if (x_recon) x_recon[i] = s;
+    g_unscaled[i] = x[i] - s;
+  }
+  return KVAE_OK;
+}
+int kvae_dec_head_bwd_loss(const float *in, const float *W, const float *g_unscaled, const float *g_frame, float *g_in,
+                           float *w_partials, float *b_partials, float *w_scratch, int64_t N, int32_t Cin, int32_t side,
+                           void *stream) {
+  if (!g_unscaled || !g_frame) return KVAE_ERR_NULL;
+  if (N < 1) return KVAE_ERR_ARG;
+  if (Cin != 32 || side != 16) return KVAE_ERR_DIMS;
+  const int64_t pixels = 4 * (int64_t)side * side;
+  std::vector<float> g((size_t)(N * pixels));
+  for (int64_t i = 0; i < N * pixels; ++i) g[i] = g_frame[i / pixels] * g_unscaled[i];
+  return kvae_dec_head_bwd(in, W, g.data(), g_in, w_partials, b_partials, w_scratch, N, Cin, side, stream);
+}
+}
+
+#include "vae_stats.h"
+extern "C" int kvae_active_units(const float *mu, int64_t N, int32_t A, float threshold, float *variances, int64_t *count,
+                                 void *) {
+  if (!mu || !variances || !count) return KVAE_ERR_NULL;
+  if (N < 1 || N > kvae::AU_MAX_ROWS || A < 1) return KVAE_ERR_ARG;
+  int64_t active = 0;
+  std::vector<kvae::ChanStat> s(kvae::AU_THREADS);
+  for (int c = 0; c < A; ++c) {
+    for (int t = 0; t < kvae::AU_THREADS; ++t) {
+      s[t] = kvae::ChanStat{0.0, 0.0, 0.0};
+      for (int64_t r = t; r < N; r += kvae::AU_THREADS) kvae::chan_push(s[t], mu[r * A + c]);
+    }
+    for (int w = 0; w < kvae::AU_WAVES; ++w)
+      for (int off = 32; off > 0; off >>= 1)
+        for (int l = 0; l < off; ++l) s[64 * w + l] = kvae::chan_merge(s[64 * w + l], s[64 * w + l + off]);
+    for (int w = kvae::AU_WAVES / 2; w > 0; w >>= 1)
+      for (int i = 0; i < w; ++i) s[64 * i] = kvae::chan_merge(s[64 * i], s[64 * (i + w)]);
+    const float v = (float)(s[0].m2 / (s[0].n - 1.0));
+    variances[c] = v;
+    active += v > threshold ? 1 : 0;
+  }
+  *count = active;
+  return KVAE_OK;
+}
diff --git a/kalman-vae_amd/csrc/vae_loss.h b/kalman-vae_amd/csrc/vae_loss.h
--- a/kalman-vae_amd/csrc/vae_loss.h
+++ b/kalman-vae_amd/csrc/vae_loss.h
@@ -10,3 +10,7 @@
 }
 
 }
+
+#if defined(KVAE_HOSTSIM)
+#include "vae_host_twins.h"
+#endif
diff --git a/kalman-vae_amd/csrc/vae_stats.h b/kalman-vae_amd/csrc/vae_stats.h
--- /dev/null
+++ b/kalman-vae_amd/csrc/vae_stats.h
@@ -0,0 +1,57 @@
+#pragma once
+#include "lgssm_vm.h"
+
+namespace kvae {
+
+struct ChanStat { double n, mean, m2; };
+
+KV_DEV void chan_push(ChanStat &s, double x) {
+  s.n += 1.0;
+  const double d = x - s.mean;
+  s.mean += d / s.n;
+  s.m2 += d * (x - s.mean);
+}
+KV_DEV ChanStat chan_merge(const ChanStat a, const ChanStat b) {
+  const double n = a.n + b.n;
+  if (n == 0.0) return a;
+  const double d = b.mean - a.mean, f = b.n / n;
+  return ChanStat{n, a.mean + d * f, a.m2 + b.m2 + d * d * a.n * f};
+}
+
+constexpr int AU_THREADS = 1024, AU_WAVES = AU_THREADS / 64;
+constexpr int64_t AU_MAX_ROWS = (int64_t)1 << 24;
+
+#if !defined(KVAE_HOSTSIM)
+__global__ __launch_bounds__(AU_THREADS) void k_active_units(const float *__restrict__ mu, int64_t N, int A, float threshold,
+                                                             float *__restrict__ variances, int64_t *__restrict__ count) {
+  __shared__ ChanStat part[AU_WAVES];
+  const int lane = threadIdx.x & 63, wv = threadIdx.x >> 6;
+  int64_t active = 0;
+  for (int c = 0; c < A; ++c) {
+    ChanStat s{0.0, 0.0, 0.0};
+    for (int64_t r = threadIdx.x; r < N; r += AU_THREADS) chan_push(s, mu[r * A + c]);
+    for (int off = 32; off > 0; off >>= 1) {
+      const ChanStat o{__shfl_down(s.n, off, 64), __shfl_down(s.mean, off, 64), __shfl_down(s.m2, off, 64)};
+      s = chan_merge(s, o);
+    }
+    if (lane == 0) part[wv] = s;
+    __syncthreads();
+    if (threadIdx.x == 0) {
+      ChanStat t[AU_WAVES];
+#pragma unroll
+      for (int w = 0; w < AU_WAVES; ++w) t[w] = part[w];
+#pragma unroll
+      for (int w = AU_WAVES / 2; w > 0; w >>= 1)
+#pragma unroll
+        for (int i = 0; i < w; ++i) t[i] = chan_merge(t[i], t[i + w]);
+      const float v = (float)(t[0].m2 / (t[0].n - 1.0));
+      variances[c] = v;
+      active += v > threshold ? 1 : 0;
+    }
+    __syncthreads();
+  }
+  if (threadIdx.x == 0) *count = active;
+}
+#endif
+
+}
diff --git a/kalman-vae_amd/kvae/_native.py b/kalman-vae_amd/kvae/_native.py
--- a/kalman-vae_amd/kvae/_native.py
+++ b/kalman-vae_amd/kvae/_native.py
@@ -10,7 +10,7 @@
 KVAE_MAX_DIM = 16
 KVAE_MAX_K = 16
 LSTM_MAX_H, LSTM_MAX_I = 52, 16
-ABI_VERSION = 12
+ABI_VERSION = 13
 
 _STATUS = {1: "KVAE_ERR_DIMS (n, m, p must be in [1,16]; B, T >= 1)", 2: "KVAE_ERR_NULL", 3: "KVAE_ERR_LAUNCH",
            4: "KVAE_ERR_ARG"}
@@ -61,8 +61,9 @@
 SYMBOLS = ("kvae_lgssm_filter_alpha_lstm", "kvae_lgssm_alpha_lstm_bwd", "kvae_lgssm_filter_fwd", "kvae_lgssm_rts_fwd", "kvae_lgssm_smooth_fwd", "kvae_lgssm_smooth_bwd",
            "kvae_lgssm_elbo", "kvae_mix_fwd", "kvae_mix_bwd", "kvae_mix_bwd_partials", "kvae_lstm_fwd",
            "kvae_lstm_bwd", "kvae_bias_shuffle_act_fwd", "kvae_bias_shuffle_act_bwd", "kvae_bias_partial_rows", "kvae_colsum", "kvae_colsum2", "kvae_clip_adam", "kvae_regime_fwd", "kvae_regime_bwd", "kvae_bigru_fwd", "kvae_bigru_bwd", "kvae_bce_frames_fwd", "kvae_bce_frames_bwd",
-           "kvae_dec_head_fwd", "kvae_dec_head_bwd", "kvae_enc_stem_fwd", "kvae_enc_stem_bwd", "kvae_conv_edge_partial_rows",
-           "kvae_enc_mid_fwd", "kvae_enc_mid_bwd", "kvae_enc_mid_partial_rows",
+           "kvae_dec_head_fwd", "kvae_dec_head_bwd", "kvae_dec_head_fwd_loss", "kvae_dec_head_bwd_loss", "kvae_active_units",
+           "kvae_enc_stem_fwd", "kvae_enc_stem_bwd", "kvae_conv_edge_partial_rows",
+           "kvae_enc_mid_fwd", "kvae_enc_mid_bwd", "kvae_enc_mid_partial_rows", "kvae_enc_mid_fwd_bits", "kvae_enc_mid_bwd_bits",
            "kvae_dec_up_fwd", "kvae_dec_up_bwd", "kvae_dec_up_partial_rows", "kvae_dec_up_set_workgroups",
            "kvae_enc_head_fwd", "kvae_enc_head_bwd", "kvae_dec_fc_fwd", "kvae_dec_fc_bwd", "kvae_head_partial_rows",
            "kvae_latent_reg_fwd", "kvae_latent_reg_bwd", "kvae_loss_head_fwd", "kvae_loss_head_bwd",
@@ -128,6 +129,12 @@
         d.kvae_dec_head_fwd.restype = C.c_int
         d.kvae_dec_head_bwd.argtypes = [vp] * 7 + [C.c_int64, C.c_int32, C.c_int32, vp]
         d.kvae_dec_head_bwd.restype = C.c_int
+        d.kvae_dec_head_fwd_loss.argtypes = [vp] * 9 + [C.c_int64, C.c_int32, C.c_int32, vp]
+        d.kvae_dec_head_fwd_loss.restype = C.c_int
+        d.kvae_dec_head_bwd_loss.argtypes = [vp] * 8 + [C.c_int64, C.c_int32, C.c_int32, vp]
+        d.kvae_dec_head_bwd_loss.restype = C.c_int
+        d.kvae_active_units.argtypes = [vp, C.c_int64, C.c_int32, C.c_float, vp, vp, vp]
+        d.kvae_active_units.restype = C.c_int
         d.kvae_enc_stem_fwd.argtypes = [vp, vp, vp, vp, vp, C.c_int64, C.c_int32, C.c_int32, vp]
         d.kvae_enc_stem_fwd.restype = C.c_int
         d.kvae_enc_stem_bwd.argtypes = [vp] * 6 + [C.c_int64, C.c_int32, C.c_int32, vp]
@@ -137,6 +144,10 @@
         d.kvae_enc_mid_bwd.argtypes = [vp] * 7 + [C.c_int64, C.c_int32, C.c_int32, vp]
         d.kvae_enc_mid_bwd.restype = C.c_int
         d.kvae_enc_mid_partial_rows.argtypes = [C.c_int64, C.c_int32]
+        d.kvae_enc_mid_fwd_bits.argtypes = [vp, vp, vp, vp, vp, C.c_int64, C.c_int32, C.c_int32, vp]
+        d.kvae_enc_mid_fwd_bits.restype = C.c_int
+        d.kvae_enc_mid_bwd_bits.argtypes = [vp] * 7 + [C.c_int64, C.c_int32, C.c_int32, vp]
+        d.kvae_enc_mid_bwd_bits.restype = C.c_int
         d.kvae_dec_up_fwd.argtypes = [vp, vp, vp, vp, C.c_int64, C.c_int32, C.c_int32, vp]
         d.kvae_dec_up_fwd.restype = C.c_int
         d.kvae_dec_up_bwd.argtypes = [vp] * 7 + [C.c_int64, C.c_int32, C.c_int32, vp]
diff --git a/kalman-vae_amd/kvae/model/model.py b/kalman-vae_amd/kvae/model/model.py
--- a/kalman-vae_amd/kvae/model/model.py
+++ b/kalman-vae_amd/kvae/model/model.py
@@ -100,8 +100,13 @@
         a, mu, var = self.encoder.heads(feat, eps)
         return a.unflatten(0, lead), mu.unflatten(0, lead), var.unflatten(0, lead)
 
-    def decode_sequence(self, a):
-        return self.decoder(a.flatten(0, 1)).unflatten(0, a.shape[:2])
+    def decode_sequence(self, a, frames=None, want_recon=True):
+        if frames is None:
+            return self.decoder(a.flatten(0, 1)).unflatten(0, a.shape[:2])
+        dec = self.decoder(a.flatten(0, 1), frames=frames.flatten(0, 1), want_recon=want_recon)
+        if isinstance(dec, tuple):
+            return tuple(t.unflatten(0, a.shape[:2]) if t is not None else None for t in dec)
+        return dec.unflatten(0, a.shape[:2])
 
     def _to_pixels(self, logits):
         return torch.sigmoid(logits) if self.config.out_distr.lower() == "bernoulli" else logits
@@ -128,9 +133,17 @@
         else:
             smoothed = self.kalman_filter.smooth(a_samples, u, mask=mask)
         (mus_smooth, Sigmas_smooth, mus_filt, Sigmas_filt, mus_pred, Sigmas_pred, A_list, B_list, C_list) = smoothed
-        x_logits = self.decode_sequence(a_samples)
+        frame_ll = x_recon = None
+        if (self.training and torch.is_grad_enabled() and self.config.out_distr.lower() == "bernoulli"
+                and x.dtype == torch.float32 and not x.requires_grad):
+            dec = self.decode_sequence(a_samples, frames=x, want_recon=with_recon)
+            x_logits, x_recon, frame_ll = dec if isinstance(dec, tuple) else (dec, None, None)
+        else:
+            x_logits = self.decode_sequence(a_samples)
+        if with_recon and x_recon is None:
+            x_recon = self._to_pixels(x_logits)
         return {
-            "x_recon": self._to_pixels(x_logits) if with_recon else None, "x_logits": x_logits,
+            "x_recon": x_recon, "x_logits": x_logits, "frame_ll": frame_ll,
             "a_samples": a_samples, "a_mu": a_mu, "a_var": a_var, "a_side": a_side,
             "mus_smooth": mus_smooth, "Sigmas_smooth": Sigmas_smooth,
             "mus_filt": mus_filt, "Sigmas_filt": Sigmas_filt,
@@ -154,8 +167,13 @@
         a_side = outputs.get("a_side")
         stats = None
         if with_metrics == "device":
-            variances = a_mu.detach().reshape(-1, a_mu.shape[-1]).var(dim=0)
-            stats = ((variances > 1e-2).sum(), variances)
+            from kvae.vae import fused
+            mu2 = a_mu.detach().reshape(-1, a_mu.shape[-1])
+            if fused._FUSED_TAIL and _native.fused_ok(mu2) and mu2.dtype == torch.float32 and 1 <= mu2.shape[0] <= 1 << 24:
+                stats = fused.active_units(mu2, 1e-2)
+            else:
+                variances = mu2.var(dim=0)
+                stats = ((variances > 1e-2).sum(), variances)
 
         def kf_elbo():
             if self.kf_value_only and self.training:
@@ -193,7 +211,9 @@
                 and _native.fused_ok(x_mu) and x_mu.dtype == torch.float32
                 and x.dtype == torch.float32 and a.dtype == torch.float32 and not x.requires_grad):
             from kvae.vae.fused import BernoulliFrameLogLik, LatentReg, LossHead
-            lpx = BernoulliFrameLogLik.apply(x_mu, x)
+            lpx = outputs.get("frame_ll")
+            if lpx is None:
+                lpx = BernoulliFrameLogLik.apply(x_mu, x)
             regf = LatentReg.apply(a, a_mu, a_var)
             mk = None if mask is None else mask.to(device=x.device, dtype=torch.float32).reshape(B, T)
             if head == "2":
@@ -219,7 +239,7 @@
                 if self.config.out_distr.lower() != "bernoulli" else None
             vae_elbo, recon, reg = vae_loss(x, x_mu, x_var, a, a_mu, a_var,
                                             scale_reconstruction=self.config.scale_reconstruction, mask=mask,
-                                            out_distr=self.config.out_distr, beta=self.beta)
+                                            out_distr=self.config.out_distr, beta=self.beta, frame_ll=outputs.get("frame_ll"))
             elbo_kf = kf_elbo()
             elbo_total = vae_weight * vae_elbo + kf_weight * elbo_kf
             out = {"loss": -elbo_total, "elbo_total": elbo_total, "elbo_kf": elbo_kf, "elbo_vae_total": vae_elbo,
diff --git a/kalman-vae_amd/kvae/vae/fused.py b/kalman-vae_amd/kvae/vae/fused.py
--- a/kalman-vae_amd/kvae/vae/fused.py
+++ b/kalman-vae_amd/kvae/vae/fused.py
@@ -1,10 +1,19 @@
+import os
+
 import torch
 
 from .. import _native as N
+
+_RELU_BITS = os.environ.get("KVAE_RELU_BITS", "1") != "0"
+_FUSED_TAIL = os.environ.get("KVAE_FUSED_TAIL", "1") != "0"
 
 
 colsum = N.colsum
 colsum_pair = N.colsum_pair
+
+
+def _optr(t):
+    return N.ptr(t) if t is not None else None
 
 
 def _chunks(n, size):
@@ -89,6 +98,65 @@
         return g_h, gw.view_as(weight), gb
 
 
+class DecoderHeadLoss(torch.autograd.Function):
+
+    @staticmethod
+    def forward(ctx, h, weight, bias, x, want_recon):
+        h, weight, bias, x = h.contiguous(), weight.contiguous(), bias.contiguous(), x.contiguous()
+        Nb, Cin, s, _ = h.shape
+        logits = torch.empty(Nb, 1, 2 * s, 2 * s, device=h.device, dtype=torch.float32)
+        recon = torch.empty_like(logits) if want_recon else None
+        gdiff = torch.empty_like(logits)
+        ll = torch.empty(Nb, device=h.device, dtype=torch.float32)
+        scratch = torch.empty(DecoderHead.SCRATCH, device=h.device, dtype=torch.float32)
+        lib = N.lib_for(h)
+        lib.check(lib.dll.kvae_dec_head_fwd_loss(N.ptr(h), N.ptr(weight), N.ptr(bias), N.ptr(x), N.ptr(logits), _optr(recon),
+                                                 N.ptr(gdiff), N.ptr(ll), N.ptr(scratch), Nb, Cin, s, N.stream_for(h)),
+                  "kvae_dec_head_fwd_loss")
+        ctx.save_for_backward(h, weight, gdiff, scratch, logits)
+        ctx.set_materialize_grads(False)
+        if recon is None:
+            return logits, None, ll
+        return logits, recon, ll
+
+    @staticmethod
+    def backward(ctx, g_logits, g_recon, g_ll):
+        h, weight, gdiff, scratch, logits = ctx.saved_tensors
+        Nb, Cin, s, _ = h.shape
+        lib = N.lib_for(h)
+        rows = lib.dll.kvae_conv_edge_partial_rows(Nb)
+        g_h = torch.empty_like(h) if ctx.needs_input_grad[0] else None
+        wp = torch.empty(rows, weight.numel(), device=h.device, dtype=torch.float32)
+        bp = torch.empty(rows, 4, device=h.device, dtype=torch.float32)
+        if g_logits is None and g_recon is None:
+            g_ll = g_ll.contiguous() if g_ll is not None else torch.zeros(Nb, device=h.device, dtype=torch.float32)
+            lib.check(lib.dll.kvae_dec_head_bwd_loss(N.ptr(h), N.ptr(weight), N.ptr(gdiff), N.ptr(g_ll), _optr(g_h), N.ptr(wp),
+                                                     N.ptr(bp), N.ptr(scratch), Nb, Cin, s, N.stream_for(h)),
+                      "kvae_dec_head_bwd_loss")
+        else:
+            g = torch.zeros_like(logits) if g_ll is None else g_ll.view(Nb, 1, 1, 1) * gdiff
+            if g_logits is not None:
+                g = g + g_logits
+            if g_recon is not None:
+                sg = torch.sigmoid(logits)
+                g = g + g_recon * sg * (1 - sg)
+            lib.check(lib.dll.kvae_dec_head_bwd(N.ptr(h), N.ptr(weight), N.ptr(g.contiguous()), _optr(g_h), N.ptr(wp), N.ptr(bp),
+                                                N.ptr(scratch), Nb, Cin, s, N.stream_for(h)), "kvae_dec_head_bwd")
+        gw, gb = colsum_pair(wp, bp)
+        return g_h, gw.view_as(weight), gb, None, None
+
+
+def active_units(mu, threshold=1e-2):
+    mu = mu.contiguous()
+    Nb, A = mu.shape
+    variances = torch.empty(A, device=mu.device, dtype=torch.float32)
+    count = torch.empty((), device=mu.device, dtype=torch.int64)
+    lib = N.lib_for(mu)
+    lib.check(lib.dll.kvae_active_units(N.ptr(mu), Nb, A, float(threshold), N.ptr(variances), N.ptr(count), N.stream_for(mu)),
+              "kvae_active_units")
+    return count, variances
+
+
 class EncoderStem(torch.autograd.Function):
 
     @staticmethod
@@ -141,16 +209,23 @@
         x, weight, bias = x.contiguous(), weight.contiguous(), bias.contiguous()
         Nb, Cc, s, _ = x.shape
         out = torch.empty(Nb, Cc, s // 2, s // 2, device=x.device, dtype=torch.float32)
+        need_bits = _RELU_BITS and any(ctx.needs_input_grad)
+        bits = torch.empty(Nb, (s // 2) ** 2, device=x.device, dtype=torch.int32) if need_bits else None
         lib = N.lib_for(x)
         for a, b in _chunks(Nb, EncoderMid.CHUNK):
-            lib.check(N.timed(f"enc_mid_fwd_s{s}", x, lambda: lib.dll.kvae_enc_mid_fwd(
-                N.ptr(x[a:b]), N.ptr(weight), N.ptr(bias), N.ptr(out[a:b]), b - a, Cc, s, N.stream_for(x))), "kvae_enc_mid_fwd")
-        ctx.save_for_backward(x, weight, out)
+            if bits is not None:
+                lib.check(N.timed(f"enc_mid_fwd_s{s}", x, lambda: lib.dll.kvae_enc_mid_fwd_bits(
+                    N.ptr(x[a:b]), N.ptr(weight), N.ptr(bias), N.ptr(out[a:b]), N.ptr(bits[a:b]), b - a, Cc, s, N.stream_for(x))),
+                    "kvae_enc_mid_fwd_bits")
+            else:
+                lib.check(N.timed(f"enc_mid_fwd_s{s}", x, lambda: lib.dll.kvae_enc_mid_fwd(
+                    N.ptr(x[a:b]), N.ptr(weight), N.ptr(bias), N.ptr(out[a:b]), b - a, Cc, s, N.stream_for(x))), "kvae_enc_mid_fwd")
+        ctx.save_for_backward(x, weight, out if bits is None else None, bits)
         return out
 
     @staticmethod
     def backward(ctx, g):
-        x, weight, out = ctx.saved_tensors
+        x, weight, out, bits = ctx.saved_tensors
         g = g.contiguous()
         Nb, Cc, s, _ = x.shape
         lib = N.lib_for(x)
@@ -160,9 +235,14 @@
             rows = lib.dll.kvae_enc_mid_partial_rows(b - a, s)
             wp = torch.empty(rows, weight.numel(), device=x.device, dtype=torch.float32)
             bp = torch.empty(rows, Cc, device=x.device, dtype=torch.float32)
-            lib.check(lib.dll.kvae_enc_mid_bwd(N.ptr(x[a:b]), N.ptr(weight), N.ptr(out[a:b]), N.ptr(g[a:b]),
-                                               N.ptr(g_x[a:b]) if g_x is not None else None, N.ptr(wp), N.ptr(bp), b - a, Cc, s,
-                                               N.stream_for(x)), "kvae_enc_mid_bwd")
+            if bits is not None:
+                lib.check(lib.dll.kvae_enc_mid_bwd_bits(N.ptr(x[a:b]), N.ptr(weight), N.ptr(bits[a:b]), N.ptr(g[a:b]),
+                                                        N.ptr(g_x[a:b]) if g_x is not None else None, N.ptr(wp), N.ptr(bp), b - a, Cc, s,
+                                                        N.stream_for(x)), "kvae_enc_mid_bwd_bits")
+            else:
+                lib.check(lib.dll.kvae_enc_mid_bwd(N.ptr(x[a:b]), N.ptr(weight), N.ptr(out[a:b]), N.ptr(g[a:b]),
+                                                   N.ptr(g_x[a:b]) if g_x is not None else None, N.ptr(wp), N.ptr(bp), b - a, Cc, s,
+                                                   N.stream_for(x)), "kvae_enc_mid_bwd")
             cw, cb = colsum_pair(wp, bp)
             gw, gb = _acc(gw, cw), _acc(gb, cb)
         return g_x, gw.view_as(weight), gb
@@ -208,10 +288,6 @@
             cw, cb = colsum_pair(wp, bp)
             gw, gb = _acc(gw, cw), _acc(gb, cb)
         return g_x, gw.view_as(weight), gb
-
-
-def _optr(t):
-    return N.ptr(t) if t is not None else None
 
 
 class EncoderHead(torch.autograd.Function):
diff --git a/kalman-vae_amd/kvae/vae/losses.py b/kalman-vae_amd/kvae/vae/losses.py
--- a/kalman-vae_amd/kvae/vae/losses.py
+++ b/kalman-vae_amd/kvae/vae/losses.py
@@ -27,13 +27,15 @@
 
 
 def vae_loss(x, x_mu, x_var, a, a_mu, a_var, scale_reconstruction: float = 0.3, beta: float = 1.0,
-             mask=None, out_distr: str = "gaussian"):
+             mask=None, out_distr: str = "gaussian", frame_ll=None):
     mk = _frame_mask(mask, x)
     denom = mk.sum().clamp(min=1.0)
     from kvae import _native
     if out_distr.lower() == "bernoulli" and _native.fused_ok(a) and a.dtype == torch.float32 and a_var.dim() == a.dim():
         from kvae.vae.fused import BernoulliFrameLogLik, LatentReg
-        if x_mu.dtype == torch.float32 and x.dtype == torch.float32 and not x.requires_grad:
+        if frame_ll is not None:
+            lpx = frame_ll
+        elif x_mu.dtype == torch.float32 and x.dtype == torch.float32 and not x.requires_grad:
             lpx = BernoulliFrameLogLik.apply(x_mu, x)
         else:
             lpx = -F.binary_cross_entropy_with_logits(x_mu, x, reduction="none").sum(dim=(2, 3, 4))
@@ -41,7 +43,9 @@
         reg = (LatentReg.apply(a, a_mu, a_var) * mk).sum() / denom
         return scale_reconstruction * recon + beta * reg, recon, reg
     if out_distr.lower() == "bernoulli":
-        if _native.fused_ok(x_mu) and x_mu.dtype == torch.float32 and x.dtype == torch.float32 and not x.requires_grad:
+        if frame_ll is not None:
+            lpx = frame_ll
+        elif _native.fused_ok(x_mu) and x_mu.dtype == torch.float32 and x.dtype == torch.float32 and not x.requires_grad:
             from kvae.vae.fused import BernoulliFrameLogLik
             lpx = BernoulliFrameLogLik.apply(x_mu, x)
         else:
diff --git a/kalman-vae_amd/kvae/vae/vae.py b/kalman-vae_amd/kvae/vae/vae.py
--- a/kalman-vae_amd/kvae/vae/vae.py
+++ b/kalman-vae_amd/kvae/vae/vae.py
@@ -6,7 +6,9 @@
 
 from kvae import _native
 from kvae.utils.config import KVAEConfig
-from kvae.vae.fused import DecoderFc, DecoderHead, DecoderUp, EncoderHead, EncoderMid, EncoderStem, conv_block
+from kvae.vae import fused as _fused
+from kvae.vae.fused import (DecoderFc, DecoderHead, DecoderHeadLoss, DecoderUp, EncoderHead, EncoderMid, EncoderStem,
+                            conv_block)
 
 
 def _conv_out(size, k, s, p):
@@ -70,7 +72,7 @@
         up += [nn.Conv2d(chans[-1], 4 * config.img_channels, kernel_size=3, padding=1), nn.PixelShuffle(2)]
         self.deconv_layers = nn.Sequential(*up)
 
-    def forward(self, a: torch.Tensor) -> torch.Tensor:
+    def forward(self, a: torch.Tensor, frames: torch.Tensor = None, want_recon: bool = True):
         fused = _native.fused_ok(a) and a.dtype == torch.float32
         h = DecoderFc.apply(a, self.fc.weight, self.fc.bias) if fused and DecoderFc.supported(a, self.fc) else self.fc(a)
         h = h.unflatten(1, (self.init_channels, self.init_size, self.init_size))
@@ -81,6 +83,9 @@
             if isinstance(layer, nn.Conv2d):
                 relu = i + 2 < len(layers) and isinstance(layers[i + 2], nn.ReLU)
                 if not relu and DecoderHead.supported(h, layer):
+                    if (frames is not None and _fused._FUSED_TAIL and frames.dtype == torch.float32 and not frames.requires_grad
+                            and frames.shape[0] == h.shape[0] and tuple(frames.shape[1:]) == (1, 32, 32)):
+                        return DecoderHeadLoss.apply(h, layer.weight, layer.bias, frames, want_recon)
                     h = DecoderHead.apply(h, layer.weight, layer.bias)
                 elif relu and DecoderUp.supported(h, layer):
                     h = DecoderUp.apply(h, layer.weight, layer.bias)
```
